# richhiey/YourMT3

Measured on AMD Instinct MI355X. Metric: audio-sec transcribed / wall-sec (RTF), higher is better.
Workload: dtype bf16; 1 GPU; BASELINE configs[1]: MT3 base (T5-small dims, 6+6 layers, d512, 8x64 heads, d_ff 2048, vocab 1536), 2.048 s / 16 kHz / 128-mel segments (256 encoder frames), greedy decode forced to 1024 tokens, seeded random weights; segments_per_gpu=64, global_batch=64, decode_len=1024, frames=256, parallelism=dp1 (segments sharded, token ids all-gathered over RCCL)

## Files before the change

include/ymt3.h:

```cpp
#ifndef YMT3_H
#define YMT3_H

#include <stddef.h>
#include <stdint.h>

#ifdef __cplusplus
extern "C" {
#endif

#define YMT3_ABI_VERSION 3

enum { YMT3_OK = 0, YMT3_ERR_ARG = 1, YMT3_ERR_BLOB = 2, YMT3_ERR_HIP = 3, YMT3_ERR_UNSUPPORTED = 4 };
enum { YMT3_ENC_T5 = 0, YMT3_ENC_PERCEIVER_TF = 1 };
enum { YMT3_FFN_DENSE = 0, YMT3_FFN_MOE = 1 };

typedef struct ymt3_config {
    int32_t sample_rate, segment_samples, n_fft, hop, n_mels;
    float   f_min, f_max, log_floor;
    int32_t d_model, d_ff, n_heads, d_kv, n_enc_layers, n_dec_layers;
    int32_t vocab, rel_buckets, rel_max_distance;
    float   ln_eps;
    int32_t max_decode_len, n_channels, eos_id, pad_id;
    int32_t encoder_type, n_latents;
    int32_t dec_ffn, n_experts, moe_top_k, moe_fp8;
// ... 4 lines not shown
typedef struct ymt3_ctx* ymt3_handle;

int         ymt3_abi_version(void);
const char* ymt3_last_error(void);

int  ymt3_create(const ymt3_config* cfg, const void* blob_host, size_t blob_bytes, int device, ymt3_handle* out);
void ymt3_destroy(ymt3_handle h);

size_t ymt3_device_bytes(ymt3_handle h);

#define YMT3_PCM_S16 0
#define YMT3_PCM_F32 1
int ymt3_ingest_plan(ymt3_handle h, int64_t n_frames, int sample_rate_in, int64_t* n_samples_out, int* n_segments);
int ymt3_ingest(ymt3_handle h, const void* pcm_dev, int pcm_format, int64_t n_frames, int n_channels,
                int sample_rate_in, float* segments_dev, int n_segments, void* stream);

int ymt3_logmel(ymt3_handle h, const float* audio_dev, int B, float* mel_dev, void* stream);

int ymt3_encode(ymt3_handle h, const float* mel_dev, int B, void* enc_dev, void* stream);

int ymt3_decode_greedy(ymt3_handle h, const void* enc_dev, int B, int n_steps, int32_t* tokens_dev,
                       const int32_t* forced_dev, float* logits_dev, void* stream);

int ymt3_decode_prompted(ymt3_handle h, const void* enc_dev, int B, int n_steps, const int32_t* prompt_dev, int n_prompt,
                         int32_t* tokens_dev, const int32_t* forced_dev, float* logits_dev, void* stream);
int ymt3_transcribe_segments_prompted(ymt3_handle h, const float* audio_dev, int B, int n_steps, const int32_t* prompt_dev,
                                      int n_prompt, int32_t* tokens_dev, void* stream);
int ymt3_transcribe_stream_prompted(ymt3_handle h, const float* audio_dev, int n_segments, int n_steps, const int32_t* prompt_dev,
                                    int n_prompt, int32_t* tokens_dev, int slots, int interval, void* stream);

int ymt3_decode_scored(ymt3_handle h, const void* enc_dev, int B, int n_steps, const int32_t* prompt_dev, int n_prompt,
                       int32_t* tokens_dev, float* scores_dev, const int32_t* forced_dev, float* logits_dev, void* stream);
int ymt3_transcribe_segments_scored(ymt3_handle h, const float* audio_dev, int B, int n_steps, const int32_t* prompt_dev,
                                    int n_prompt, int32_t* tokens_dev, float* scores_dev, void* stream);
int ymt3_transcribe_stream_scored(ymt3_handle h, const float* audio_dev, int n_segments, int n_steps, const int32_t* prompt_dev,
                                  int n_prompt, int32_t* tokens_dev, float* scores_dev, int slots, int interval, void* stream);

int ymt3_score_tokens(ymt3_handle h, const void* enc_dev, int B, int n_steps, const int32_t* prompt_dev, int n_prompt,
                      const int32_t* tokens_dev, const int32_t* lengths_dev, float* scores_dev, float* logits_dev, void* stream);
int ymt3_transcribe_segments_score(ymt3_handle h, const float* audio_dev, int B, int n_steps, const int32_t* prompt_dev, int n_prompt,
                                   const int32_t* tokens_dev, const int32_t* lengths_dev, float* scores_dev, void* stream);

typedef struct ymt3_constraint_s* ymt3_constraint;
int  ymt3_constraint_create(ymt3_handle h, int n_states, int vocab, const uint32_t* allowed_bits_host, const int32_t* next_host,
                            ymt3_constraint* out);
void ymt3_constraint_destroy(ymt3_constraint c);
int ymt3_decode_constrained(ymt3_handle h, const void* enc_dev, int B, int n_steps, const int32_t* prompt_dev, int n_prompt,
                            int32_t* tokens_dev, float* scores_dev, const int32_t* forced_dev, float* logits_dev,
                            ymt3_constraint constraint, const int32_t* start_state_dev, void* stream);
int ymt3_transcribe_segments_constrained(ymt3_handle h, const float* audio_dev, int B, int n_steps, const int32_t* prompt_dev,
                                         int n_prompt, int32_t* tokens_dev, float* scores_dev, ymt3_constraint constraint,
                                         const int32_t* start_state_dev, void* stream);
int ymt3_transcribe_stream_constrained(ymt3_handle h, const float* audio_dev, int n_segments, int n_steps, const int32_t* prompt_dev,
                                       int n_prompt, int32_t* tokens_dev, float* scores_dev, int slots, int interval,
                                       ymt3_constraint constraint, const int32_t* start_state_dev, void* stream);

typedef struct ymt3_beam_params { int32_t num_beams, num_return; float length_penalty; } ymt3_beam_params;
int ymt3_decode_beam(ymt3_handle h, const void* enc_dev, int B, int n_steps, const int32_t* prompt_dev, int n_prompt,
                     const ymt3_beam_params* params, int32_t* tokens_dev, float* seq_scores_dev, float* token_scores_dev,
                     ymt3_constraint constraint, const int32_t* start_state_dev, void* stream);
int ymt3_transcribe_segments_beam(ymt3_handle h, const float* audio_dev, int B, int n_steps, const int32_t* prompt_dev, int n_prompt,
                                  const ymt3_beam_params* params, int32_t* tokens_dev, float* seq_scores_dev, float* token_scores_dev,
                                  ymt3_constraint constraint, const int32_t* start_state_dev, void* stream);
int ymt3_transcribe_stream_beam(ymt3_handle h, const float* audio_dev, int n_segments, int n_steps, const int32_t* prompt_dev, int n_prompt,
                                const ymt3_beam_params* params, int32_t* tokens_dev, float* seq_scores_dev, float* token_scores_dev,
                                int slots, int interval, ymt3_constraint constraint, const int32_t* start_state_dev, void* stream);
int ymt3_debug_beam_trace(ymt3_handle h, int32_t* trace_dev, float* run_dev, float* logits_dev, int n_steps, int n_groups);

int ymt3_set_early_stop(ymt3_handle h, int interval);

int ymt3_transcribe_segments(ymt3_handle h, const float* audio_dev, int B, int n_steps,
                             int32_t* tokens_dev, void* stream);

int ymt3_transcribe_stream(ymt3_handle h, const float* audio_dev, int n_segments, int n_steps, int32_t* tokens_dev,
                           int slots, int interval, void* stream);

int ymt3_last_decode_steps(ymt3_handle h);

int ymt3_set_abort_recovery(ymt3_handle h, int mode);
int ymt3_merged_fallbacks(ymt3_handle h);

int ymt3_last_decode_chains(ymt3_handle h);

#define YMT3_PROFILE_CLASSES 16
int ymt3_profile_decode(ymt3_handle h, const void* enc_dev, int B, int n_steps, int stride, int32_t* tokens_dev,
                        float* ms_by_class, int32_t* launches_by_class, void* stream);

int ymt3_debug_step_stamps(ymt3_handle h, int32_t* cls, int32_t* grid, uint64_t* stats, int* n_kernels);
int ymt3_debug_kernel_stamps(ymt3_handle h, int kernel, uint64_t* stamps, int capacity_wgs);

int ymt3_debug_decode_start(ymt3_handle h, int step0);

int ymt3_debug_force_stage_abort(ymt3_handle h);

int ymt3_debug_moe_trace(ymt3_handle h, int32_t* trace_dev, int n_steps, int n_rows);

int ymt3_test_gemm(ymt3_handle h, const void* a_dev, const void* w_dev, float* c_dev, int M, int N, int K, void* stream);

#ifdef __cplusplus
}
#endif
#endif
```

yourmt3_amd/_lib.py:

```python
from __future__ import annotations

import ctypes
import os

from .config import CConfig

_HERE = os.path.dirname(os.path.abspath(__file__))
LIB_PATH = os.environ.get("YMT3_LIB", os.path.join(_HERE, "libymt3_hip.so"))

SYMBOLS = [
    "ymt3_abi_version", "ymt3_last_error", "ymt3_create", "ymt3_destroy", "ymt3_device_bytes",
    "ymt3_logmel", "ymt3_encode", "ymt3_decode_greedy", "ymt3_transcribe_segments", "ymt3_test_gemm", "ymt3_profile_decode", "ymt3_debug_decode_start", "ymt3_debug_force_stage_abort", "ymt3_set_early_stop", "ymt3_last_decode_steps",
    "ymt3_ingest_plan", "ymt3_ingest", "ymt3_transcribe_stream", "ymt3_debug_step_stamps", "ymt3_debug_kernel_stamps",
    "ymt3_set_abort_recovery", "ymt3_merged_fallbacks", "ymt3_debug_moe_trace", "ymt3_last_decode_chains",
    "ymt3_decode_prompted", "ymt3_transcribe_segments_prompted", "ymt3_transcribe_stream_prompted",
    "ymt3_decode_scored", "ymt3_transcribe_segments_scored", "ymt3_transcribe_stream_scored",
    "ymt3_constraint_create", "ymt3_constraint_destroy", "ymt3_decode_constrained", "ymt3_transcribe_segments_constrained",
    "ymt3_transcribe_stream_constrained",
    "ymt3_decode_beam", "ymt3_transcribe_segments_beam", "ymt3_debug_beam_trace", "ymt3_transcribe_stream_beam",
    "ymt3_score_tokens", "ymt3_transcribe_segments_score",
]

_lib = None


class BeamParams(ctypes.Structure):
    _fields_ = [("num_beams", ctypes.c_int32), ("num_return", ctypes.c_int32), ("length_penalty", ctypes.c_float)]


class YMT3Error(RuntimeError):
    pass


def load() -> ctypes.CDLL:
    global _lib
    if _lib is not None:
        return _lib
    if not os.path.exists(LIB_PATH):
        raise YMT3Error(
            f"{LIB_PATH} not found: build it with `python -m yourmt3_amd.build` "
            "(hipcc --offload-arch=gfx950).  There is no CPU fallback for the hot path.")
    import torch
    lib = ctypes.CDLL(LIB_PATH)
    vp, i32, sz = ctypes.c_void_p, ctypes.c_int, ctypes.c_size_t
    lib.ymt3_abi_version.restype = i32
    lib.ymt3_last_error.restype = ctypes.c_char_p
    lib.ymt3_create.argtypes = [ctypes.POINTER(CConfig), vp, sz, i32, ctypes.POINTER(vp)]
    lib.ymt3_create.restype = i32
    lib.ymt3_destroy.argtypes = [vp]
    lib.ymt3_destroy.restype = None
    lib.ymt3_device_bytes.argtypes = [vp]
    lib.ymt3_device_bytes.restype = sz
    lib.ymt3_logmel.argtypes = [vp, vp, i32, vp, vp]
    lib.ymt3_encode.argtypes = [vp, vp, i32, vp, vp]
    lib.ymt3_decode_greedy.argtypes = [vp, vp, i32, i32, vp, vp, vp, vp]
    lib.ymt3_transcribe_segments.argtypes = [vp, vp, i32, i32, vp, vp]
    lib.ymt3_test_gemm.argtypes = [vp, vp, vp, vp, i32, i32, i32, vp]
    lib.ymt3_profile_decode.argtypes = [vp, vp, i32, i32, i32, vp, ctypes.POINTER(ctypes.c_float), ctypes.POINTER(ctypes.c_int32), vp]
    lib.ymt3_profile_decode.restype = i32
    lib.ymt3_debug_decode_start.argtypes = [vp, i32]
    lib.ymt3_debug_decode_start.restype = i32
    lib.ymt3_debug_force_stage_abort.argtypes = [vp]
    lib.ymt3_debug_force_stage_abort.restype = i32
    lib.ymt3_last_decode_steps.argtypes = [vp]
    lib.ymt3_last_decode_steps.restype = i32
    lib.ymt3_set_early_stop.argtypes = [vp, i32]
    lib.ymt3_set_early_stop.restype = i32
    lib.ymt3_ingest_plan.argtypes = [vp, ctypes.c_int64, i32, ctypes.POINTER(ctypes.c_int64), ctypes.POINTER(ctypes.c_int)]
    lib.ymt3_ingest_plan.restype = i32
    lib.ymt3_ingest.argtypes = [vp, vp, i32, ctypes.c_int64, i32, i32, vp, i32, vp]
    lib.ymt3_ingest.restype = i32
    lib.ymt3_transcribe_stream.argtypes = [vp, vp, i32, i32, vp, i32, i32, vp]
    lib.ymt3_transcribe_stream.restype = i32
    lib.ymt3_decode_prompted.argtypes = [vp, vp, i32, i32, vp, i32, vp, vp, vp, vp]
    lib.ymt3_decode_prompted.restype = i32
    lib.ymt3_transcribe_segments_prompted.argtypes = [vp, vp, i32, i32, vp, i32, vp, vp]
    lib.ymt3_transcribe_segments_prompted.restype = i32
    lib.ymt3_transcribe_stream_prompted.argtypes = [vp, vp, i32, i32, vp, i32, vp, i32, i32, vp]
    lib.ymt3_transcribe_stream_prompted.restype = i32
    lib.ymt3_decode_scored.argtypes = [vp, vp, i32, i32, vp, i32, vp, vp, vp, vp, vp]
    lib.ymt3_decode_scored.restype = i32
    lib.ymt3_transcribe_segments_scored.argtypes = [vp, vp, i32, i32, vp, i32, vp, vp, vp]
    lib.ymt3_transcribe_segments_scored.restype = i32
    lib.ymt3_transcribe_stream_scored.argtypes = [vp, vp, i32, i32, vp, i32, vp, vp, i32, i32, vp]
    lib.ymt3_transcribe_stream_scored.restype = i32
    lib.ymt3_constraint_create.argtypes = [vp, i32, i32, vp, vp, ctypes.POINTER(vp)]
    lib.ymt3_constraint_create.restype = i32
    lib.ymt3_constraint_destroy.argtypes = [vp]
    lib.ymt3_constraint_destroy.restype = None
    lib.ymt3_decode_constrained.argtypes = [vp, vp, i32, i32, vp, i32, vp, vp, vp, vp, vp, vp, vp]
    lib.ymt3_decode_constrained.restype = i32
    lib.ymt3_transcribe_segments_constrained.argtypes = [vp, vp, i32, i32, vp, i32, vp, vp, vp, vp, vp]
    lib.ymt3_transcribe_segments_constrained.restype = i32
    lib.ymt3_transcribe_stream_constrained.argtypes = [vp, vp, i32, i32, vp, i32, vp, vp, i32, i32, vp, vp, vp]
    lib.ymt3_transcribe_stream_constrained.restype = i32
    lib.ymt3_debug_step_stamps.argtypes = [vp, vp, vp, vp, ctypes.POINTER(ctypes.c_int)]
    lib.ymt3_debug_step_stamps.restype = i32
    lib.ymt3_debug_kernel_stamps.argtypes = [vp, i32, vp, i32]
    lib.ymt3_debug_kernel_stamps.restype = i32
    lib.ymt3_set_abort_recovery.argtypes = [vp, i32]
    lib.ymt3_set_abort_recovery.restype = i32
    lib.ymt3_merged_fallbacks.argtypes = [vp]
    lib.ymt3_merged_fallbacks.restype = i32
    lib.ymt3_last_decode_chains.argtypes = [vp]
    lib.ymt3_last_decode_chains.restype = i32
    lib.ymt3_debug_moe_trace.argtypes = [vp, vp, i32, i32]
    lib.ymt3_debug_moe_trace.restype = i32
    bp = ctypes.POINTER(BeamParams)
    lib.ymt3_decode_beam.argtypes = [vp, vp, i32, i32, vp, i32, bp, vp, vp, vp, vp, vp, vp]
    lib.ymt3_decode_beam.restype = i32
    lib.ymt3_transcribe_segments_beam.argtypes = [vp, vp, i32, i32, vp, i32, bp, vp, vp, vp, vp, vp, vp]
    lib.ymt3_transcribe_segments_beam.restype = i32
    lib.ymt3_transcribe_stream_beam.argtypes = [vp, vp, i32, i32, vp, i32, bp, vp, vp, vp, i32, i32, vp, vp, vp]
    lib.ymt3_transcribe_stream_beam.restype = i32
    lib.ymt3_debug_beam_trace.argtypes = [vp, vp, vp, vp, i32, i32]
    lib.ymt3_debug_beam_trace.restype = i32
    lib.ymt3_score_tokens.argtypes = [vp, vp, i32, i32, vp, i32, vp, vp, vp, vp, vp]
    lib.ymt3_score_tokens.restype = i32
    lib.ymt3_transcribe_segments_score.argtypes = [vp, vp, i32, i32, vp, i32, vp, vp, vp, vp]
    lib.ymt3_transcribe_segments_score.restype = i32
    for n in ("ymt3_logmel", "ymt3_encode", "ymt3_decode_greedy", "ymt3_transcribe_segments", "ymt3_test_gemm"):
        getattr(lib, n).restype = i32
    if lib.ymt3_abi_version() != 3:
        raise YMT3Error("libymt3_hip.so ABI version mismatch")
    _lib = lib
    return lib


def check(rc: int) -> None:
    if rc != 0:
        raise YMT3Error(f"ymt3 error {rc}: {load().ymt3_last_error().decode(errors='replace')}")
```

yourmt3_amd/csrc/decode.hip:

```cpp
#include <cstdlib>
#include <type_traits>

#include "common.h"
#include "kernels.h"

namespace {

constexpr int DKV = 64;
constexpr int WO_LDS_BYTES = 8 * 64 * 128;
typedef unsigned u32x4 __attribute__((ext_vector_type(4)));

#ifndef YMT3_STAMP_PHASE
#define YMT3_STAMP_PHASE 0
#endif
#define STAMP_IN(a) do { if ((a).stamp && threadIdx.x == 0) (a).stamp[2 * blockIdx.x] = wall_clock64(); } while (0)
#define PAIR_MARK(a, k, v) do { if ((a).stamp && threadIdx.x == 0) (a).stamp[1024 + 8 * blockIdx.x + (k)] = (v); } while (0)
#define STAMP_OUT(a) do { if ((a).stamp && (threadIdx.x & 63) == 0) atomicMax((a).stamp + 2 * blockIdx.x + 1, (unsigned long long)wall_clock64()); } while (0)

template <int MODE, int K, int NT, bool PEND = false>
__global__ __launch_bounds__(512) void dec_gemm_kernel(const bf16_t* __restrict__ pW, const void* __restrict__ pX, const float* __restrict__ pGain,
                                                       float* pSsq, float* pOut, int row0, int R, int N, int ssq_stride, DecGemmArgs a) {
    constexpr bool NORM = (MODE != DG_RESID);
    constexpr int KW = K / 8;
    constexpr int KS = KW / 32;
// ... 111 lines not shown
                }
                __syncthreads();
            }
#pragma unroll
            for (int i = 0; i < NIX; ++i) {
                const int row = i * RPIX + lane / LPRX;
                const float sc = sscale[row];
                *reinterpret_cast<uint2*>(sA + row * PITCH + (lane % LPRX) * 8) =
                    make_uint2(pack_bf16x2(xv[i][0] * sc * gv[0], xv[i][1] * sc * gv[1]),
                               pack_bf16x2(xv[i][2] * sc * gv[2], xv[i][3] * sc * gv[3]));
            }
        } else {
            u32x4 av[NIA];
#pragma unroll
            for (int i = 0; i < NIA; ++i) {
                int mm = m0 + i * RPIW + lane / LPRW;
                mm = mm < m_end ? mm : m_end - 1;
                av[i] = *reinterpret_cast<const u32x4*>(reinterpret_cast<const bf16_t*>(pX) + (size_t)mm * K + wave * KW + (lane % LPRW) * 8);
            }
            __builtin_amdgcn_sched_barrier(0);
            STAMP_IN(a);
#pragma unroll
            for (int i = 0; i < NIW; ++i) {
                const int off = (i * RPIW + lane / LPRW) * PITCH + (lane % LPRW) * 16;
                *reinterpret_cast<u32x4*>(sW + off) = wv[i];
                if (i < NIA) *reinterpret_cast<u32x4*>(sA + off) = av[i];
            }
        }
#pragma unroll
        for (int ks = 0; ks < KS; ++ks) {
            const int off = li * PITCH + (ks * 32 + g * 8) * 2;
            const bf16x8 af = *reinterpret_cast<const bf16x8*>(sA + off);
#pragma unroll
            for (int c = 0; c < NT; ++c) {
                const bf16x8 wf = *reinterpret_cast<const bf16x8*>(sW + c * STRIP + off);
                acc[c] = __builtin_amdgcn_mfma_f32_16x16x32_bf16(wf, af, acc[c], 0, 0, 0);
            }
        }
    }

#if YMT3_STAMP_PHASE == 1
    STAMP_IN(a);
#endif
#pragma unroll
    for (int c = 0; c < NT; ++c)
        *reinterpret_cast<float4*>(red + ((wave * ROWS + li) * COLS + c * 16 + g * 4)) =
            make_float4(acc[c][0], acc[c][1], acc[c][2], acc[c][3]);
    __syncthreads();
#if YMT3_STAMP_PHASE == 2
    STAMP_IN(a);
#endif
    float2 s = make_float2(0.f, 0.f);
    if (epi) {
        s = *reinterpret_cast<const float2*>(red + (mr * COLS + nq));
#pragma unroll
        for (int w = 1; w < 8; ++w) {
            const float2 t = *reinterpret_cast<const float2*>(red + ((w * ROWS + mr) * COLS + nq));
            s.x += t.x; s.y += t.y;
        }
    }

    if constexpr (MODE == DG_RESID) {
        float2 o = make_float2(0.f, 0.f);
        if (live) {
            if (a.part) {
                float2 sp = hp[0];
#pragma unroll
                for (int w = 1; w < 8; ++w) { sp.x += hp[w].x; sp.y += hp[w].y; }
                hold.x += sp.x; hold.y += sp.y;
            }
            o = make_float2(hold.x + s.x, hold.y + s.y);
            *reinterpret_cast<float2*>(pOut + (size_t)m * N + n) = o;
        }
        float q = o.x * o.x + o.y * o.y;
        q = sum8(q);
        if (live && (tid & 7) == 0) pSsq[(size_t)nt_idx * ssq_stride + m] = q;
    } else if constexpr (MODE == DG_NORM_LOGITS) {
        if (live) *reinterpret_cast<float2*>(pOut + (size_t)m * N + n) = s;
    } else if (live) {
        if constexpr (MODE == DG_NORM_BF16_RELU) { s.x = fmaxf(s.x, 0.f); s.y = fmaxf(s.y, 0.f); }
        const uint32_t pk = pack_bf16x2(s.x, s.y);
        if constexpr (MODE == DG_NORM_QKV_CACHE) {
            const int inner = a.H * DKV;
            if (n < inner) {
                *reinterpret_cast<uint32_t*>(a.out_bf16 + (size_t)m * inner + n) = pk;
            } else {
                const int nn = n - inner, kv = nn / inner, hh = (nn % inner) >> 6, dd = nn & 63;
                bf16_t* cache = kv ? a.vcache : a.kcache;
                *reinterpret_cast<uint32_t*>(cache + (((size_t)m * a.H + hh) * a.L + step) * DKV + dd) = pk;
            }
        } else {
            *reinterpret_cast<uint32_t*>(a.out_bf16 + (size_t)m * N + n) = pk;
        }
    }
    STAMP_OUT(a);
}

template <int MODE, int K, int BM, int PF, int NTH>
__global__ __launch_bounds__(NTH) void dec_gemm_mid_kernel(const bf16_t* __restrict__ pW, const void* __restrict__ pX, const float* __restrict__ pGain,
                                                           float* pSsq, float* pOut, int row0, int R, int N, int ssq_stride, DecGemmArgs a) {
    constexpr bool NORM = (MODE != DG_RESID);
    constexpr int BN = 64, BK = 64, MT = BM / 16, PITCH = BK * 2 + 16, NKT = K / BK;
    constexpr int RG = NTH / 256, MTW = MT / RG;
    static_assert(NTH == 256 || NTH == 512, "");
    static_assert(MT % RG == 0, "row tiles split between the two wave groups");
    constexpr int A_STAGE = BM * PITCH, W_STAGE = BN * PITCH;
    __shared__ __attribute__((aligned(16))) char sA[2][A_STAGE];
    __shared__ __attribute__((aligned(16))) char sW[2][W_STAGE];
    __shared__ float sscale[BM];
    __shared__ __attribute__((aligned(16))) float sgain[NORM ? K : 4];
    const int tid = threadIdx.x, lane = tid & 63, wave = tid >> 6, li = lane & 15, g = lane >> 4;
    const int wc = wave & 3, rg = wave >> 2;
    const int n_mt = (R + BM - 1) / BM, n_nt = N / BN;
    int nt_idx, mt_idx;
    if ((n_nt & 7) == 0) {
        const int xcd = blockIdx.x & 7, slot = blockIdx.x >> 3;
        mt_idx = slot % n_mt;
        nt_idx = (slot / n_mt) * 8 + xcd;
    } else {
        mt_idx = blockIdx.x % n_mt;
        nt_idx = blockIdx.x / n_mt;
    }
    const int n0 = nt_idx * BN, m0 = row0 + mt_idx * BM, m_end = row0 + R;

    constexpr int NWV = 512 / NTH, NAB = (BM * 8 + NTH - 1) / NTH, NAF = BM * 16 / NTH;
    static_assert(BM * 16 % NTH == 0, "");
    static_assert(NKT % PF == 0, "the K loop is unrolled by the prefetch depth");
    u32x4 wvr[PF][NWV];
    u32x4 abr[PF][NORM ? 1 : NAB];
    f32x4 afr[PF][NORM ? NAF : 1];
    auto load_regs = [&](int kt, u32x4 (&wv)[NWV], u32x4 (&ab)[NORM ? 1 : NAB], f32x4 (&af)[NORM ? NAF : 1]) {
#pragma unroll
        for (int i = 0; i < NWV; ++i) {
            const int idx = tid + i * NTH, row = idx >> 3, ch = idx & 7;
            wv[i] = *reinterpret_cast<const u32x4*>(pW + (size_t)(n0 + row) * K + kt * BK + ch * 8);
        }
        if constexpr (NORM) {
#pragma unroll
            for (int i = 0; i < NAF; ++i) {
                const int idx = tid + i * NTH, row = idx >> 4, ch = idx & 15;
                int mm = m0 + row;
                mm = mm < m_end ? mm : m_end - 1;
                af[i] = *reinterpret_cast<const f32x4*>(reinterpret_cast<const float*>(pX) + (size_t)mm * K + kt * BK + ch * 4);
            }
        } else {
#pragma unroll
            for (int i = 0; i < NAB; ++i) {
                const int idx = tid + i * NTH, row = idx >> 3, ch = idx & 7;
                int mm = m0 + row;
                mm = mm < m_end ? mm : m_end - 1;
                if (BM * 8 % NTH == 0 || idx < BM * 8)
                    ab[i] = *reinterpret_cast<const u32x4*>(reinterpret_cast<const bf16_t*>(pX) + (size_t)mm * K + kt * BK + ch * 8);
            }
        }
    };
    auto store_lds = [&](int kt, int buf, const u32x4 (&wv)[NWV], const u32x4 (&ab)[NORM ? 1 : NAB], const f32x4 (&af)[NORM ? NAF : 1]) {
#pragma unroll
        for (int i = 0; i < NWV; ++i) {
            const int idx = tid + i * NTH, row = idx >> 3, ch = idx & 7;
            *reinterpret_cast<u32x4*>(sW[buf] + row * PITCH + ch * 16) = wv[i];
        }
        if constexpr (NORM) {
#pragma unroll
            for (int i = 0; i < NAF; ++i) {
                const int idx = tid + i * NTH, row = idx >> 4, ch = idx & 15;
                const float sc = sscale[row];
                const f32x4 gv = *reinterpret_cast<const f32x4*>(sgain + kt * BK + ch * 4);
// ... 454 lines not shown
        }
        if constexpr (OP && SELF) qs[tid] = f2bf(o / L);
        else a.out[((size_t)r * H + h) * DKV + tid] = f2bf(o / L);
    }
    if constexpr (OP && SELF) {
        __syncthreads();
        asm volatile("s_waitcnt vmcnt(0)" ::: "memory");
        const int li = lane & 15, g = lane >> 4;
        const char* strip = wo_lds + wave * 8192;
        f32x4 pa[4];
#pragma unroll
        for (int c = 0; c < 4; ++c) pa[c] = (f32x4){0.f, 0.f, 0.f, 0.f};
#pragma unroll
        for (int ks = 0; ks < 2; ++ks) {
            bf16x8 af = *reinterpret_cast<const bf16x8*>(qs + ks * 32 + g * 8);
            if (li != 0) af = (bf16x8){0, 0, 0, 0, 0, 0, 0, 0};
#pragma unroll
            for (int c = 0; c < 4; ++c) {
                const int row = c * 16 + li;
                const bf16x8 wf = *reinterpret_cast<const bf16x8*>(strip + row * 128 + (((ks * 4 + g) ^ (row & 7)) * 16));
                pa[c] = __builtin_amdgcn_mfma_f32_16x16x32_bf16(wf, af, pa[c], 0, 0, 0);
            }
        }
        if (li == 0) {
            float* dst = a.opart + ((size_t)r * H + h) * 512 + wave * 64 + g * 4;
            if constexpr (PAIR == 1) {
                const __amdgpu_buffer_rsrc_t ro = __builtin_amdgcn_make_buffer_rsrc(a.opart, 0, 0x7fffffff, 0x00020000);
                const int off = (((r * H + h) * 512) + wave * 64 + g * 4) * 4;
#pragma unroll
                for (int c = 0; c < 4; ++c) __builtin_amdgcn_raw_buffer_store_b128(__builtin_bit_cast(u32x4, pa[c]), ro, off + c * 64, 0, 16);
            } else {
#pragma unroll
                for (int c = 0; c < 4; ++c) *reinterpret_cast<float4*>(dst + c * 16) = make_float4(pa[c][0], pa[c][1], pa[c][2], pa[c][3]);
            }
        }
    }
    if constexpr (FUSEQ) {
        if (a.chain_sync && blockIdx.x == 0 && tid < CHAIN_COUNTERS) a.chain_sync[tid * CHAIN_LINE] = 0u;
    }
    if constexpr (PAIR == 1) PAIR_MARK(a, 2, wall_clock64());
    if constexpr (PAIR == 2) pair_leave(ps, r, left_before);
    if constexpr (PAIR != 1) STAMP_OUT(a);
}

template <bool SELF, bool FUSEQ, int NW, bool OP = false>
__global__ __launch_bounds__(64 * NW, 4) void dec_attn_kernel(const bf16_t* __restrict__ pK, const bf16_t* __restrict__ pV, const bf16_t* __restrict__ pQ,
                                                              const float* __restrict__ pF, const void* __restrict__ p4, const void* __restrict__ p5,
                                                              unsigned geom0, unsigned geom1, DecAttnArgs a) {
    attn_body<SELF, FUSEQ, NW, OP, 0>(pK, pV, pQ, pF, p4, p5, geom0, geom1, a, PairSync{});
}

template <int NW>
__global__ __launch_bounds__(64 * NW, 4) void dec_attn_beam_kernel(const bf16_t* __restrict__ pK, const bf16_t* __restrict__ pV, const bf16_t* __restrict__ pQ,
                                                                   const float* __restrict__ pF, const void* __restrict__ p4, const void* __restrict__ p5,
                                                                   unsigned geom0, unsigned geom1, DecAttnArgs a, BeamAttn ba) {
    attn_body<true, false, NW, false, 0, true>(pK, pV, pQ, pF, p4, p5, geom0, geom1, a, PairSync{}, ba);
}

__global__ __launch_bounds__(512, 4) void dec_attn_pair_kernel(const bf16_t* __restrict__ pK, const bf16_t* __restrict__ pV, const bf16_t* __restrict__ pQ,
                                                               const float* __restrict__ pF, const void* __restrict__ p4, const void* __restrict__ p5,
                                                               unsigned geom0, unsigned geom1, DecAttnArgs a, DecAttnArgs b, unsigned gb0, unsigned gb1,
                                                               PairSync ps) {
    attn_body<true, false, 8, true, 1>(pK, pV, pQ, pF, p4, p5, geom0, geom1, a, ps);
    asm volatile("" ::: "memory");
    __builtin_amdgcn_sched_barrier(0);
    attn_body<false, true, 8, true, 2>(b.k, b.v, b.wq, b.x_f32, b.gain, b.ipart, gb0, gb1, b, ps);
}

__device__ __forceinline__ void embed_row(const ArgmaxArgs& a, int r, const bf16_t* e, const bf16_t* c, float* scratch4) {
    const int tid = threadIdx.x;
    float q = 0.f;
    for (int i = tid; i < a.d; i += 256) {
        const float v = bf2f(e[i]) + (c ? bf2f(c[i]) : 0.f);
        a.h[(size_t)r * a.d + i] = v;
        q += v * v;
    }
    q = wave_sum(q);
    __syncthreads();
    if ((tid & 63) == 0) scratch4[tid >> 6] = q;
    __syncthreads();
    if (tid < SSQ_TILES) a.ssq[(size_t)tid * a.ssq_stride + r] = tid == 0 ? (scratch4[0] + scratch4[1]) + (scratch4[2] + scratch4[3]) : 0.f;
}

__global__ __launch_bounds__(256) void argmax_embed_kernel(const float* __restrict__ pLogits, DecodeShared* pShared, int* pFinished, int* pRowPos,
                                                           const long long* __restrict__ pRowOut, const bf16_t* __restrict__ pEmbed, int row0, int V,
                                                           ArgmaxArgs a) {
    __shared__ float sv[4];
    __shared__ int si[4];
    __shared__ int s_feed;
    __shared__ float s_sum[4];
    const int tid = threadIdx.x, lane = tid & 63, wave = tid >> 6;
    const int r = row0 + blockIdx.x;
    DecodeShared* sh = pShared;
    const int t = sh->step, n_steps = sh->n_steps, n_prompt = sh->n_prompt, col = t - sh->step0 - n_prompt;
    const float* row = pLogits + (size_t)r * V;
    int32_t* const tokens_out = sh->tokens_out;
    const int32_t* const forced = sh->forced;
    float* const logits_out = sh->logits_out;
    const int32_t* const prompt = sh->prompt;
    float* const scores_out = sh->scores_out;
    const uint32_t* const c_allowed = sh->c_allowed;
    const int was_finished = pFinished[r];
    const int forced_tok = forced && col >= 0 ? forced[(size_t)r * n_steps + col] : 0;
    const int pos0 = pRowPos ? pRowPos[r] : 0;
    const long long out0 = pRowPos ? pRowOut[r] : 0;

    STAMP_IN(a);
    float bv = -3.4e38f;
    int bi = 0;
    for (int i = tid; i < V; i += 256) {
        const float v = row[i];
        if (v > bv) { bv = v; bi = i; }
    }
    int state = 0;
    const uint32_t* mrow = nullptr;
    if (c_allowed) {
        state = a.row_state[r];
        asm volatile("" : "+v"(state));
        mrow = c_allowed + (size_t)state * sh->c_words;
        bv = -3.4e38f;
        bi = 0x7fffffff;
        for (int i = tid; i < V; i += 256) {
            const float v = row[i];
            if ((mrow[i >> 5] >> (i & 31)) & 1u) {
                if (v > bv) { bv = v; bi = i; }
                else bi = min(bi, i);
            }
        }
    }
#define ARGMAX_TAKE(ctrl, rows, cond)                                                                                      \
    do {                                                                                                                  \
        const float ov = __builtin_bit_cast(float, __builtin_amdgcn_update_dpp(0, __builtin_bit_cast(int, bv), (ctrl), (rows), 0xF, false)); \
        const int oi = __builtin_amdgcn_update_dpp(0, bi, (ctrl), (rows), 0xF, false);                                    \
        if ((cond) && (ov > bv || (ov == bv && oi < bi))) { bv = ov; bi = oi; }                                           \
    } while (0)
    ARGMAX_TAKE(0x128, 0xF, true);
    ARGMAX_TAKE(0x124, 0xF, true);
    ARGMAX_TAKE(0x122, 0xF, true);
    ARGMAX_TAKE(0x121, 0xF, true);
    ARGMAX_TAKE(0x142, 0xA, (lane & 16) != 0);
    ARGMAX_TAKE(0x143, 0xC, lane >= 32);
#undef ARGMAX_TAKE
    if (lane == 63) { sv[wave] = bv; si[wave] = bi; }
    __syncthreads();
    const float row_max = scores_out ? fmaxf(fmaxf(sv[0], sv[1]), fmaxf(sv[2], sv[3])) : 0.f;
    long long score_at = -1;
    int score_id = -1;
    if (tid == 0) { bv = sv[0]; bi = si[0]; }
    if (tid == 0 && pRowPos) {
#pragma unroll
        for (int w = 1; w < 4; ++w)
            if (sv[w] > bv || (sv[w] == bv && si[w] < bi)) { bv = sv[w]; bi = si[w]; }
        bi = min(bi, V - 1);
        int feed = a.pad_id;
        if (!was_finished && pos0 < n_prompt) {
            pRowPos[r] = pos0 + 1;
            feed = prompt[a.row_prompt[r] + pos0];
        } else if (!was_finished) {
            const int p = pos0 - n_prompt;
            tokens_out[out0 + p] = bi;
            if ((a.eos_id >= 0 && bi == a.eos_id) || p + 1 >= n_steps) pFinished[r] = 1;
            else pRowPos[r] = pos0 + 1;
            feed = bi;
            score_at = out0 + p;
            score_id = bi;
            if (mrow) a.row_state[r] = sh->c_next[(size_t)state * V + bi];
        }
        s_feed = feed < 0 ? 0 : (feed >= V ? V - 1 : feed);
    } else if (tid == 0 && col < 0) {
        const int p = prompt[(size_t)r * n_prompt + (t - sh->step0)];
        s_feed = p < 0 ? 0 : (p >= V ? V - 1 : p);
    } else if (tid == 0) {
#pragma unroll
        for (int w = 1; w < 4; ++w)
            if (sv[w] > bv || (sv[w] == bv && si[w] < bi)) { bv = sv[w]; bi = si[w]; }
        int tok = min(bi, V - 1);
        if (a.eos_id >= 0) {
            if (was_finished) tok = a.pad_id;
            else if (tok == a.eos_id) pFinished[r] = 1;
        }
        tokens_out[(size_t)r * n_steps + col] = tok;
        int feed = forced ? forced_tok : tok;
        feed = feed < 0 ? 0 : (feed >= V ? V - 1 : feed);
        s_feed = feed;
        score_at = (long long)r * n_steps + col;
        score_id = !forced && a.eos_id >= 0 && was_finished ? -1 : feed;
        if (mrow && !(a.eos_id >= 0 && was_finished)) a.row_state[r] = sh->c_next[(size_t)state * V + feed];
    }
    __syncthreads();
    const int feed = s_feed;
    const bf16_t* e = pEmbed + (size_t)feed * a.d;
    const bf16_t* c = a.chan_embed ? a.chan_embed + (size_t)(r % a.n_channels) * a.d : nullptr;
    embed_row(a, r, e, c, sv);
    if (logits_out && !pRowPos && col >= 0) {
        float* dst = logits_out + ((size_t)r * n_steps + col) * V;
        for (int i = tid; i < V; i += 256) dst[i] = row[i];
    }
    if (scores_out) {
        float q = 0.f;
        if (mrow) {
            for (int i = tid; i < V; i += 256)
                if ((mrow[i >> 5] >> (i & 31)) & 1u) q += __expf(row[i] - row_max);
        } else {
            for (int i = tid; i < V; i += 256) q += __expf(row[i] - row_max);
        }
        q = wave_sum(q);
        if (lane == 0) s_sum[wave] = q;
    }
    if (a.zero_sync)
        for (int i = blockIdx.x * 256 + tid; i < a.zero_lines; i += gridDim.x * 256) a.zero_sync[(size_t)i * CHAIN_LINE] = 0u;
    __syncthreads();
    if (tid == 0) {
        if (scores_out && score_at >= 0)
            scores_out[score_at] = score_id < 0 ? 0.f
                                 : mrow && !((mrow[score_id >> 5] >> (score_id & 31)) & 1u) ? -__builtin_inff()
                                 : (row[score_id] - row_max) - __logf((s_sum[0] + s_sum[1]) + (s_sum[2] + s_sum[3]));
        if (a.eos_id >= 0) __threadfence();
        bool last;
        if (a.ticket && gridDim.x > 64) {
            const int grp = blockIdx.x >> 5, n_grp = ((int)gridDim.x + 31) >> 5, in_grp = min(32, (int)gridDim.x - 32 * grp);
            last = false;
            if (atomicAdd(a.ticket + (size_t)grp * CHAIN_LINE, 1u) == (unsigned)(in_grp - 1)) {
                a.ticket[(size_t)grp * CHAIN_LINE] = 0u;
                if (a.eos_id >= 0) __threadfence();
                last = atomicAdd(&sh->done_count, 1) == n_grp - 1;
            }
        } else {
            last = atomicAdd(&sh->done_count, 1) == (int)gridDim.x - 1;
        }
        if (last) {
            sh->done_count = 0;
            sh->step = t + 1;
            if (a.eos_id >= 0) {
                int n = 0;
                for (int i = 0; i < (int)gridDim.x; ++i) n += pFinished[row0 + i] ? 0 : 1;
                sh->n_unfinished = n;
            }
        }
    }
    STAMP_OUT(a);
}

__global__ __launch_bounds__(256) void decode_init_kernel(ArgmaxArgs a, int n_chains, int n_steps, int step0, int32_t* tokens_out,
                                                          const int32_t* forced, float* logits_out, const int32_t* prompt, int n_prompt,
                                                          float* scores_out, ConstraintView cv) {
    const int r = blockIdx.x, tid = threadIdx.x;
    const bf16_t* e = a.embed + (size_t)a.pad_id * a.d;
    const bf16_t* c = a.chan_embed ? a.chan_embed + (size_t)(r % a.n_channels) * a.d : nullptr;
    __shared__ float sv[4];
    embed_row(a, r, e, c, sv);
    if (tid == 0) {
        a.finished[r] = 0;
        if (a.row_state) a.row_state[r] = cv.start ? min(max(cv.start[r], 0), cv.n_states - 1) : 0;
    }
    if (r == 0 && tid < n_chains) {
        DecodeShared* sh = a.shared + tid;
        sh->step = step0;
        sh->step0 = step0;
        sh->done_count = 0;
        sh->n_unfinished = a.R;
        sh->n_steps = n_steps;
        sh->tokens_out = tokens_out;
        sh->forced = forced;
        sh->logits_out = logits_out;
        sh->prompt = prompt;
        sh->n_prompt = n_prompt;
        sh->scores_out = scores_out;
        sh->c_allowed = cv.allowed;
        sh->c_next = cv.next;
        sh->c_words = cv.words;
    }
}

__global__ __launch_bounds__(256) void slot_start_kernel(ArgmaxArgs a, int row0, long long first_out, int n_steps, long long* row_out,
                                                         long long first_prompt, int n_prompt, long long* row_prompt, ConstraintView cv) {
    const int r = row0 + blockIdx.x, tid = threadIdx.x;
    const bf16_t* e = a.embed + (size_t)a.pad_id * a.d;
    const bf16_t* c = a.chan_embed ? a.chan_embed + (size_t)(r % a.n_channels) * a.d : nullptr;
    __shared__ float sv[4];
    embed_row(a, r, e, c, sv);
    if (tid == 0) {
        a.finished[r] = 0;
        a.row_pos[r] = 0;
        row_out[r] = first_out + (long long)blockIdx.x * n_steps;
        row_prompt[r] = first_prompt + (long long)blockIdx.x * n_prompt;
        if (a.row_state) a.row_state[r] = cv.start ? min(max(cv.start[blockIdx.x], 0), cv.n_states - 1) : 0;
    }
}

__global__ void slot_retire_kernel(ArgmaxArgs a, int row0, int n_steps, int n_prompt, int32_t* tokens_out, float* scores_out) {
    const int r = row0 + blockIdx.x;
    const long long o = a.row_out[r];
    for (int i = max(a.row_pos[r] + 1 - n_prompt, 0) + threadIdx.x; i < n_steps; i += blockDim.x) {
        tokens_out[o + i] = a.pad_id;
        if (scores_out) scores_out[o + i] = 0.f;
    }
}

__global__ void pad_tail_kernel(int32_t* tokens_out, float* scores_out, int row0, int n_steps, int from, int pad_id) {
    const size_t o = (size_t)(row0 + blockIdx.x) * n_steps;
    for (int i = from + threadIdx.x; i < n_steps; i += blockDim.x) {
        tokens_out[o + i] = pad_id;
        if (scores_out) scores_out[o + i] = 0.f;
    }
}

template <int MODE, int K, int NT, bool PEND = false>
constexpr size_t dg_lds_bytes() {
    return (size_t)(8 * 16 * 16 * NT + 16 + (PEND ? 8 * 16 : 0)) * 4 + (size_t)8 * (1 + NT) * 16 * (K / 8 * 2 + 16);
}

template <int MODE, int K, int NT = 1, bool PEND = false>
int launch_dg(const DecGemmArgs& a, hipStream_t stream) {
    if (a.W == nullptr)
        return hipFuncSetAttribute(reinterpret_cast<const void*>(dec_gemm_kernel<MODE, K, NT, PEND>),
                                   hipFuncAttributeMaxDynamicSharedMemorySize, (int)dg_lds_bytes<MODE, K, NT, PEND>()) == hipSuccess ? 0 : -2;
    if (MODE == DG_RESID && a.N != 16 * SSQ_TILES) return -3;
    if (PEND && (!a.pend_y || (MODE == DG_NORM_QKV_CACHE && !a.h_out))) return -4;
    dec_gemm_kernel<MODE, K, NT, PEND><<<(a.N / (16 * NT)) * ((a.R + 15) / 16), 512, dg_lds_bytes<MODE, K, NT, PEND>(), stream>>>(
        a.W, MODE == DG_RESID ? static_cast<const void*>(a.a_bf16) : static_cast<const void*>(a.x_f32), a.gain, a.ssq, a.out_f32, a.row0, a.R, a.N,
        a.ssq_stride, a);
    return 0;
}

template <int MODE, bool PEND = false>
int launch_dg_wide(const DecGemmArgs& a, hipStream_t stream) {
    static const bool narrow = getenv("YMT3_DEC_GEMM_NARROW") != nullptr;
    const int wgs16 = (a.N / 16) * ((a.R + 15) / 16);
    if (!narrow && a.N % 32 == 0 && wgs16 > 320) return launch_dg<MODE, 512, 2, PEND>(a, stream);
    return launch_dg<MODE, 512, 1, PEND>(a, stream);
}

}

int init_decode_kernels() {
    DecGemmArgs z{};
    int rc = 0;
    rc |= launch_dg<DG_RESID, 512>(z, nullptr);
    rc |= launch_dg<DG_RESID, 1024>(z, nullptr);
    rc |= launch_dg<DG_RESID, 2048>(z, nullptr);
    rc |= launch_dg<DG_NORM_QKV_CACHE, 512>(z, nullptr);
    rc |= launch_dg<DG_NORM_BF16, 512>(z, nullptr);
    rc |= launch_dg<DG_NORM_BF16_RELU, 512>(z, nullptr);
    rc |= launch_dg<DG_NORM_LOGITS, 512>(z, nullptr);
    rc |= launch_dg<DG_NORM_QKV_CACHE, 512, 2>(z, nullptr);
    rc |= launch_dg<DG_NORM_BF16, 512, 2>(z, nullptr);
    rc |= launch_dg<DG_NORM_BF16_RELU, 512, 2>(z, nullptr);
    rc |= launch_dg<DG_NORM_LOGITS, 512, 2>(z, nullptr);
    rc |= launch_dg<DG_NORM_QKV_CACHE, 512, 1, true>(z, nullptr);
    rc |= launch_dg<DG_NORM_QKV_CACHE, 512, 2, true>(z, nullptr);
    rc |= launch_dg<DG_NORM_LOGITS, 512, 1, true>(z, nullptr);
    rc |= launch_dg<DG_NORM_LOGITS, 512, 2, true>(z, nullptr);
    if (hipFuncSetAttribute(reinterpret_cast<const void*>(dec_attn_pair_kernel), hipFuncAttributeMaxDynamicSharedMemorySize, WO_LDS_BYTES) != hipSuccess) rc |= -2;
    if (hipFuncSetAttribute(reinterpret_cast<const void*>(dec_attn_kernel<true, false, 8, true>), hipFuncAttributeMaxDynamicSharedMemorySize,
                            WO_LDS_BYTES) != hipSuccess) rc |= -2;
    return rc;
}

template <int MODE, int K, int BM>
int launch_dg_mid(const DecGemmArgs& a, hipStream_t stream) {
    if (MODE == DG_RESID && a.N != 16 * SSQ_TILES) return -3;
    constexpr int PF = 4;
    constexpr int NTH = 256;
    dec_gemm_mid_kernel<MODE, K, BM, PF, NTH><<<(a.N / 64) * ((a.R + BM - 1) / BM), NTH, 0, stream>>>(
        a.W, MODE == DG_RESID ? static_cast<const void*>(a.a_bf16) : static_cast<const void*>(a.x_f32), a.gain, a.ssq, a.out_f32, a.row0, a.R, a.N,
        a.ssq_stride, a);
    return 0;
}

static int launch_dec_gemm_mid(int mode, const DecGemmArgs& a, hipStream_t stream) {
    if (a.N % 64 || a.part) return -1;
    switch (mode) {
        case DG_RESID:
            if (a.K == 512) return launch_dg_mid<DG_RESID, 512, 32>(a, stream);
            if (a.K == 2048) return launch_dg_mid<DG_RESID, 2048, 32>(a, stream);
            return -1;
        case DG_NORM_QKV_CACHE: return a.K == 512 ? launch_dg_mid<DG_NORM_QKV_CACHE, 512, 64>(a, stream) : -1;
        case DG_NORM_BF16: return a.K == 512 ? launch_dg_mid<DG_NORM_BF16, 512, 32>(a, stream) : -1;
        case DG_NORM_BF16_RELU: return a.K == 512 ? launch_dg_mid<DG_NORM_BF16_RELU, 512, 64>(a, stream) : -1;
        case DG_NORM_LOGITS: return a.K == 512 ? launch_dg_mid<DG_NORM_LOGITS, 512, 64>(a, stream) : -1;
        default: return -1;
    }
}

int launch_dec_gemm(int mode, const DecGemmArgs& a, hipStream_t stream) {
    if (a.R <= 0) return 0;
    if (a.N % 16) return -1;
    const int mid_rows = a.mid_rows >= 0 ? a.mid_rows : DEC_GEMM_MID_ROWS;
    if (mid_rows > 0 && a.R >= mid_rows && a.N % 64 == 0 && !a.part && !a.pend_y && (a.K == 512 || (a.K == 2048 && mode == DG_RESID)))
        return launch_dec_gemm_mid(mode, a, stream);
    if (mode == DG_RESID) {
        if (a.K == 512) return launch_dg<DG_RESID, 512>(a, stream);
        if (a.K == 2048) return launch_dg<DG_RESID, 2048>(a, stream);
        if (a.K == 1024) return launch_dg<DG_RESID, 1024>(a, stream);
        return -1;
    }
    if (a.K != 512) return -1;
    if (a.pend_y) {
        if (mode == DG_NORM_QKV_CACHE) return launch_dg_wide<DG_NORM_QKV_CACHE, true>(a, stream);
        if (mode == DG_NORM_LOGITS) return launch_dg_wide<DG_NORM_LOGITS, true>(a, stream);
        return -1;
    }
    switch (mode) {
        case DG_NORM_QKV_CACHE: return launch_dg_wide<DG_NORM_QKV_CACHE>(a, stream);
        case DG_NORM_BF16: return launch_dg_wide<DG_NORM_BF16>(a, stream);
        case DG_NORM_BF16_RELU: return launch_dg_wide<DG_NORM_BF16_RELU>(a, stream);
        case DG_NORM_LOGITS: return launch_dg_wide<DG_NORM_LOGITS>(a, stream);
        default: return -1;
    }
}

int launch_dec_attention(bool self_attn, const DecAttnArgs& a, hipStream_t stream) {
    if (a.R <= 0) return 0;
    const bool many = a.force_many || a.R * a.H > 2048;
    if (a.chain_sync && (self_attn || !a.wq)) return -1;
    if ((a.wo || a.ipart) && (many || a.H != 8 || (a.wo && !a.opart) || (a.ipart && !a.wq))) return -1;
    if (a.row0 < 0 || a.row0 > 0xffff || a.rows_per_kv < 1 || a.rows_per_kv > 0xff || a.H < 1 || a.H > 0xff || a.slab_keys < 1 || a.slab_keys > 0xfffff ||
        a.n_keys_const < 0 || a.n_keys_const > 0xfff || (self_attn && a.bias_stride != a.slab_keys))
        return -1;
    const unsigned g0 = (unsigned)a.row0 | (unsigned)a.rows_per_kv << 16 | (unsigned)a.H << 24, g1 = (unsigned)a.slab_keys | (unsigned)a.n_keys_const << 20;
    const int grid = a.R * a.H;
#define ATTN(S, F, W, O, THREADS, LDS, PQ, PF, P4, P5) dec_attn_kernel<S, F, W, O><<<grid, THREADS, LDS, stream>>>(a.k, a.v, PQ, PF, P4, P5, g0, g1, a)
    if (self_attn) {
        if (a.wo) ATTN(true, false, 8, true, 512, WO_LDS_BYTES, a.q, a.bias, a.shared, a.row_pos);
        else if (many) ATTN(true, false, 2, false, 128, 0, a.q, a.bias, a.shared, a.row_pos);
        else ATTN(true, false, 8, false, 512, 0, a.q, a.bias, a.shared, a.row_pos);
    } else if (a.wq) {
        if (a.ipart) ATTN(false, true, 8, true, 512, 0, a.wq, a.x_f32, a.gain, a.ipart);
        else ATTN(false, true, 8, false, 512, 0, a.wq, a.x_f32, a.gain, a.ssq);
    } else {
        if (many) ATTN(false, false, 2, false, 128, 0, a.q, nullptr, nullptr, nullptr);
        else ATTN(false, false, 8, false, 512, 0, a.q, nullptr, nullptr, nullptr);
    }
#undef ATTN
    return 0;
}

int launch_dec_attention_beam(const DecAttnArgs& a, const BeamAttn& ba, hipStream_t stream) {
    if (a.R <= 0) return 0;
    if (!ba.anc || ba.W < 1 || ba.W > BEAM_MAX || a.R % ba.W || a.row0 % ba.W || ba.anc_pitch % 16 || ba.anc_pitch <= a.slab_keys || ba.anc_pitch > 48 * 1024 ||
        a.row0 + a.R > ba.anc_rows || a.wo || a.ipart || a.wq || a.chain_sync || a.rows_per_kv != 1)
        return -1;
    if (a.row0 < 0 || a.row0 > 0xffff || a.H < 1 || a.H > 0xff || a.slab_keys < 1 || a.slab_keys > 0xfffff || a.bias_stride != a.slab_keys) return -1;
    const bool many = a.force_many || a.R * a.H > 2048;
    const unsigned g0 = (unsigned)a.row0 | 1u << 16 | (unsigned)a.H << 24, g1 = (unsigned)a.slab_keys;
    const int grid = a.R * a.H;
    if (many) dec_attn_beam_kernel<2><<<grid, 128, ba.anc_pitch, stream>>>(a.k, a.v, a.q, a.bias, a.shared, a.row_pos, g0, g1, a, ba);
    else dec_attn_beam_kernel<8><<<grid, 512, ba.anc_pitch, stream>>>(a.k, a.v, a.q, a.bias, a.shared, a.row_pos, g0, g1, a, ba);
    return 0;
}

bool dec_attention_pair_fits(int n_cus) {
    int n = 0;
    if (hipOccupancyMaxActiveBlocksPerMultiprocessor(&n, dec_attn_pair_kernel, 512, WO_LDS_BYTES) != hipSuccess) return false;
    return (long long)n * n_cus >= 512;
}

int launch_dec_attention_pair(const DecAttnArgs& a, const DecAttnArgs& b, unsigned* pair_rows, unsigned* abort_word, unsigned* host_abort,
                              hipStream_t stream) {
    if (a.R <= 0) return 0;
    if (a.R > 16 * CHAIN_TILES_MAX || a.R != b.R || a.row0 != b.row0 || a.H != 8 || b.H != 8 || !a.wo || !a.opart || !b.wq || b.ipart != a.opart || !pair_rows || !abort_word ||
        a.rows_per_kv != 1 || b.rows_per_kv < 1 || b.rows_per_kv > 0xff || a.row0 < 0 || a.row0 > 0xffff || a.slab_keys < 1 || a.slab_keys > 0xfffff ||
        b.slab_keys < 1 || b.slab_keys > 0xfffff || b.n_keys_const < 1 || b.n_keys_const > 0xfff || a.bias_stride != a.slab_keys)
        return -1;
    const unsigned g0 = (unsigned)a.row0 | 1u << 16 | 8u << 24, g1 = (unsigned)a.slab_keys;
    const unsigned h0 = (unsigned)b.row0 | (unsigned)b.rows_per_kv << 16 | 8u << 24, h1 = (unsigned)b.slab_keys | (unsigned)b.n_keys_const << 20;
    dec_attn_pair_kernel<<<a.R * 8, 512, WO_LDS_BYTES, stream>>>(a.k, a.v, a.q, a.bias, a.shared, a.row_pos, g0, g1, a, b, h0, h1,
                                                                 PairSync{pair_rows, abort_word, host_abort});
    return 0;
}

int launch_argmax_embed(const ArgmaxArgs& a, hipStream_t stream) {
    if (a.R <= 0) return 0;
    argmax_embed_kernel<<<a.R, 256, 0, stream>>>(a.logits, a.shared, a.finished, a.row_pos, a.row_out, a.embed, a.row0, a.V, a);
    return 0;
}

int launch_decode_init(const ArgmaxArgs& a, int n_chains, int n_steps, int step0, int32_t* tokens_out, const int32_t* forced,
                       float* logits_out, const int32_t* prompt, int n_prompt, float* scores_out, const ConstraintView& cv,
                       hipStream_t stream) {
    if (a.R <= 0) return 0;
    if (n_prompt < 0 || (n_prompt > 0 && !prompt)) return -1;
    if (cv.allowed && (!cv.next || !a.row_state || cv.n_states < 1 || cv.words * 32 < a.V)) return -1;
    decode_init_kernel<<<a.R, 256, 0, stream>>>(a, n_chains, n_steps, step0, tokens_out, forced, logits_out, prompt, n_prompt, scores_out, cv);
    return 0;
}

int launch_slot_start(const ArgmaxArgs& a, int row0, long long first_out, int n_steps, long long* row_out, long long first_prompt,
                      int n_prompt, long long* row_prompt, const ConstraintView& cv, hipStream_t stream) {
    if (!a.row_pos || !row_out || !row_prompt || a.n_channels <= 0) return -1;
    if (cv.start && cv.n_states < 1) return -1;
    slot_start_kernel<<<a.n_channels, 256, 0, stream>>>(a, row0, first_out, n_steps, row_out, first_prompt, n_prompt, row_prompt, cv);
    return 0;
}

int launch_slot_retire(const ArgmaxArgs& a, int row0, int n_rows, int n_steps, int n_prompt, int32_t* tokens_out, float* scores_out,
                       hipStream_t stream) {
    if (!a.row_pos || !a.row_out || n_rows <= 0) return -1;
    slot_retire_kernel<<<n_rows, 256, 0, stream>>>(a, row0, n_steps, n_prompt, tokens_out, scores_out);
    return 0;
}

int launch_pad_tail(int32_t* tokens_out, float* scores_out, int row0, int R, int n_steps, int from, int pad_id, hipStream_t stream) {
    if (R <= 0 || from >= n_steps) return 0;
    pad_tail_kernel<<<R, 256, 0, stream>>>(tokens_out, scores_out, row0, n_steps, from, pad_id);
    return 0;
}
```

yourmt3_amd/csrc/kernels.h:

```cpp
#pragma once
#include <hip/hip_runtime.h>
#include <stdint.h>
#include "common.h"

struct FrontendTables {
    const float* window;
    const float2* tw;
    const float2* untw;
    const int* mel_start;
    const int* mel_len;
    const int* mel_off;
    const float* mel_w;
    int n_fft, hop, n_mels, n_samples, n_frames, n_mel_w;
    float log_floor;
};
int launch_logmel(const FrontendTables& t, const float* audio, float* mel, int B, hipStream_t stream);

struct IngestArgs {
    const void* pcm;
    const float* taps;
    float* out;
    long long n_in, n_out, n_total, r;
    int up, down, J, Jp, n_channels, s16, window;
};
int launch_ingest(const IngestArgs& a, hipStream_t stream);

enum GemmEpilogue {
    EPI_F32 = 0,
    EPI_BF16 = 1,
    EPI_BF16_RELU = 2,
    EPI_RESID = 3,
    EPI_KV_HEADMAJOR = 4,
};
struct GemmArgs {
    const bf16_t* A; const bf16_t* W; void* out; const float* bias;
    int M, N, K, lda, ldw, ldc;
    int T, H, n_seg;
};
int launch_gemm(int epilogue, const GemmArgs& a, hipStream_t stream);
int init_gemm_kernels();

int launch_rmsnorm(const float* x, const float* gain, bf16_t* out, int M, int d, float eps, hipStream_t stream);
int launch_f32_to_bf16(const float* x, bf16_t* out, size_t n, hipStream_t stream);
int launch_broadcast_bf16(const bf16_t* src, float* out, int B, size_t n, hipStream_t stream);

int init_enc_attn_kernels();
int launch_enc_attention_qkv(const bf16_t* q, int ldq, const bf16_t* k, const bf16_t* v, int ldkv, const float* bias_off,
                             bf16_t* out, int B, int T, int H, hipStream_t stream);
int launch_enc_attention(const bf16_t* qkv, const float* bias_off, bf16_t* out, int B, int T, int H, hipStream_t stream);

struct SeqAttnArgs {
    const bf16_t* q; const bf16_t* k; const bf16_t* v; bf16_t* out;
    const float* bias_off;
    int n_seq, H, Tq, Tk, inner_n;
    long long q_outer, q_inner, q_step, kv_outer, kv_inner, kv_step, o_outer, o_inner, o_step;
};
int launch_seq_attention(const SeqAttnArgs& a, hipStream_t stream);
int launch_spec_embed(const float* mel, const float* w, const bf16_t* pos, const float* gain, bf16_t* out, long long n_rows, int F, int d,
                      float eps, hipStream_t stream);

struct DecodeShared {
    int step;
    int done_count;
    int n_steps;
    int step0;
    int n_unfinished;
    int n_prompt;
    int32_t* tokens_out;
    const int32_t* forced;
    float* logits_out;
    const int32_t* prompt;
    float* scores_out;
    const uint32_t* c_allowed;
    const int32_t* c_next;
    int c_words;
};

struct ConstraintView {
    const uint32_t* allowed;
    const int32_t* next;
    int words, n_states;
    const int32_t* start;
};

constexpr int SSQ_TILES = 32;

struct DecGemmArgs {
    const float* x_f32;
    const float* gain;
    const bf16_t* a_bf16;
    const bf16_t* W;
    int row0, R, N, K;
    float eps;
    bf16_t* out_bf16;
    float* out_f32;
    bf16_t* kcache;
    bf16_t* vcache;
    int H, L;
    const DecodeShared* shared;
    const int* row_pos;
    unsigned long long* stamp;
    float* ssq;
    int ssq_stride;
    const float* part;
    const float* pend_y;
    float* h_out;
    int mid_rows;
};
constexpr int DEC_GEMM_MID_ROWS = 512;
struct ChainArgs {
    const bf16_t *w0, *w1, *w2, *w3;
    const bf16_t* attn;
    const float* part;
    float* h;
    float* ssq; int ssq_stride;
    const float *gain1, *gain3;
    bf16_t* dff;
    int d_ff;
    int mode3, N3;
    bf16_t* out_q; bf16_t* kcache; bf16_t* vcache;
    float* logits;
    int H, L;
    const DecodeShared* shared; const int* row_pos;
    int row0, R;
    float eps;
    unsigned* sync;
    unsigned* host_abort;
    unsigned long long* stamp;
    unsigned* sync_abort;
    int nsub;
};
constexpr int CHAIN_LINE = 32;
constexpr int CHAIN_TILES_MAX = 16;
constexpr int CHAIN_COUNTERS = 3 * CHAIN_TILES_MAX * 8;
constexpr int CHAIN_ABORT_WORD = CHAIN_COUNTERS * CHAIN_LINE;
constexpr int CHAIN_SYNC_WORDS = (CHAIN_COUNTERS + 1) * CHAIN_LINE;
int init_chain_kernels();
bool dec_chain_fits(int n_cus);
bool dec_attention_pair_fits(int n_cus);
int launch_dec_chain(const ChainArgs& c, hipStream_t stream);
int launch_chain_poison(const unsigned* sync, int32_t* tokens, float* scores, long long n, hipStream_t stream);

struct StepLayer {
    const bf16_t *wo, *wq_c, *wo_c, *wi, *wo2, *w3;
    const float *ln2, *ln3, *gain3;
    const bf16_t *kself, *vself;
    const bf16_t *kcross, *vcross;
    bf16_t *knext, *vnext;
    int N3, last;
};
struct StepArgs {
    int n_layers, R, T, L, ssq_stride;
    float eps;
    int tiles_free, pad_;
    bf16_t* q; bf16_t* attn; float* opart; float* h; float* ssq; bf16_t* dff; float* logits;
    const float* bias;
    const DecodeShared* shared; const int* row_pos;
    unsigned* sync;
    unsigned* pair_rows;
    unsigned* abort_word; unsigned* host_abort;
    unsigned long long* stamp;
    StepLayer layer[8];
};
constexpr int STEP_SYNC_LINES_PER_LAYER = CHAIN_COUNTERS + 32 + 32;
constexpr int STEP_SYNC_LINES = 9 * STEP_SYNC_LINES_PER_LAYER;
int init_step_kernel();
bool dec_step_fits(int n_cus);
int launch_dec_step(const StepArgs& s, hipStream_t stream);

enum DecGemmMode { DG_NORM_QKV_CACHE = 0, DG_NORM_BF16 = 1, DG_NORM_BF16_RELU = 2, DG_NORM_LOGITS = 3, DG_RESID = 4 };
int init_decode_kernels();
int launch_dec_gemm(int mode, const DecGemmArgs& a, hipStream_t stream);

struct DecAttnArgs {
    const bf16_t* q;
    const bf16_t* k;
    const bf16_t* v;
    bf16_t* out;
    const float* bias;
    const DecodeShared* shared;
    const int* row_pos;
    unsigned long long* stamp;
    int n_keys_const;
    int slab_keys;
    int rows_per_kv;
    int row0, R, H, bias_stride;
    const bf16_t* wq;
    const float* x_f32;
    const float* gain;
    const float* ssq; int ssq_stride;
    float eps;
    const bf16_t* wo;
    float* opart;
    const float* ipart;
    unsigned* chain_sync;
    int force_many;
};
int launch_dec_attention(bool self_attn, const DecAttnArgs& a, hipStream_t stream);
int launch_dec_attention_pair(const DecAttnArgs& self_args, const DecAttnArgs& cross_args, unsigned* pair_rows, unsigned* abort_word,
                              unsigned* host_abort, hipStream_t stream);

struct McCrossArgs {
    const float* x_f32;
    const float* gain;
    const float* ssq; int ssq_stride;
    const bf16_t* wq;
    const bf16_t* k;
    const bf16_t* v;
    bf16_t* out;
    int row0, n_seg, n_channels, H, T;
    float eps;
};
int init_mc_cross_kernels();
int launch_mc_cross_attention(const McCrossArgs& a, hipStream_t stream);

struct ArgmaxArgs {
    const float* logits;
    float* h;
    const bf16_t* embed;
    const bf16_t* chan_embed;
    DecodeShared* shared;
    int* finished;
    float* ssq;
    int ssq_stride;
    int row0, R, V, d, n_channels, eos_id, pad_id;
    int* row_pos;
    const long long* row_out;
    unsigned long long* stamp;
    unsigned* ticket;
    unsigned* zero_sync;
    int zero_lines;
    const long long* row_prompt;
    int* row_state;
};
int launch_argmax_embed(const ArgmaxArgs& a, hipStream_t stream);
int launch_pad_tail(int32_t* tokens_out, float* scores_out, int row0, int R, int n_steps, int from, int pad_id, hipStream_t stream);
int launch_slot_start(const ArgmaxArgs& a, int row0, long long first_out, int n_steps, long long* row_out, long long first_prompt,
                      int n_prompt, long long* row_prompt, const ConstraintView& cv, hipStream_t stream);
int launch_slot_retire(const ArgmaxArgs& a, int row0, int n_rows, int n_steps, int n_prompt, int32_t* tokens_out, float* scores_out,
                       hipStream_t stream);
int launch_decode_init(const ArgmaxArgs& a, int n_chains, int n_steps, int step0, int32_t* tokens_out, const int32_t* forced,
                       float* logits_out, const int32_t* prompt, int n_prompt, float* scores_out, const ConstraintView& cv,
                       hipStream_t stream);

constexpr int BEAM_MAX = 8;
struct BeamAttn {
    const uint8_t* anc;
    int anc_rows, anc_pitch, W;
};
int launch_dec_attention_beam(const DecAttnArgs& a, const BeamAttn& ba, hipStream_t stream);

struct BeamShared {
    float alpha;
    int32_t* tokens_out;
    float* seq_out;
    float* tok_out;
    int32_t* trace;
    float* trace_run;
    float* trace_logits;
    int trace_steps, trace_groups;
};
struct BeamArgs {
    const float* logits;
    float* h;
    const bf16_t* embed; const bf16_t* chan_embed;
    DecodeShared* shared; BeamShared* beam;
    int* finished;
    float* ssq; int ssq_stride;
    int R, V, d, n_channels, eos_id, pad_id, W;
    int* row_state;
    uint8_t* anc; int anc_rows, anc_pitch;
    int32_t* fed_tok; float* fed_lp; int fed_pitch;
    float* run;
    float* fin_score; int* fin_len; int* fin_store; int32_t* fin_tok; float* fin_lp;
    int* n_fin;
    uint8_t* slot_anc;
    unsigned long long* stamp;
    int* row_pos;
    long long* row_out;
    long long* row_prompt;
};
int launch_beam_select(const BeamArgs& a, hipStream_t stream);
int launch_beam_init(const BeamArgs& a, int n_steps, const int32_t* prompt, int n_prompt, const ConstraintView& cv, const BeamShared& params,
                     hipStream_t stream);
int launch_beam_finalize(const BeamArgs& a, int N, hipStream_t stream);
int launch_beam_slot_start(const BeamArgs& a, int row0, long long first_group, int n_prompt, const ConstraintView& cv, hipStream_t stream);
int launch_beam_slot_finalize(const BeamArgs& a, int row0, int N, hipStream_t stream);

struct SeqEmbedArgs {
    float* h;
    const bf16_t* embed;
    const bf16_t* chan_embed;
    const int32_t* prompt;
    const int32_t* tokens;
    int row0, n_rows, L, n_prompt, n_steps, V, d, n_channels, pad_id;
};
int launch_seq_embed(const SeqEmbedArgs& a, hipStream_t stream);
struct SeqAttnDecArgs {
    const bf16_t* q; const bf16_t* k; const bf16_t* v; bf16_t* out;
    const float* bias;
    long long q_seq, kv_seq, o_seq;
    int ldq, ldkv, ldo, kv_head;
    int row0, n_rows, L, n_keys, rows_per_kv, H, bias_stride;
};
int launch_dec_seq_attention(bool causal, const SeqAttnDecArgs& a, hipStream_t stream);
struct SeqLmHeadArgs {
    const bf16_t* xn;
    const bf16_t* W;
    const int32_t* tokens;
    const int32_t* lengths;
    float* scores;
    float* logits;
    int M, L, n_prompt, n_steps, V, d, row0;
};
int launch_seq_lm_head_score(const SeqLmHeadArgs& a, hipStream_t stream);

struct MoeArgs {
    float* h;
// ... 39 lines not shown
```

yourmt3_amd/csrc/runtime.hip:

```cpp
#include <hip/hip_runtime.h>

#include <cmath>
#include <cstdarg>
#include <cstdio>
#include <cstdlib>
#include <algorithm>
#include <cstring>
#include <map>
#include <atomic>
#include <string>
#include <thread>
#include <vector>

#include "../../include/ymt3.h"
#include "common.h"
#include "kernels.h"

static thread_local char g_err[512] = "";
void ymt3_set_error(const char* fmt, ...) {
    va_list ap;
    va_start(ap, fmt);
    vsnprintf(g_err, sizeof(g_err), fmt, ap);
    va_end(ap);
}
// ... 4 lines not shown
    } while (0)
#define LAUNCH(expr)                                                             \
    do {                                                                         \
        int _rc = (expr);                                                        \
        if (_rc != 0) FAIL(YMT3_ERR_UNSUPPORTED, "%s rejected its shape (rc=%d)", #expr, _rc); \
    } while (0)

struct Tensor {
    void* dev = nullptr;
    uint32_t dtype = 0, ndim = 0, shape[4] = {1, 1, 1, 1};
    size_t nbytes = 0;
};

struct StepGraph {
    hipGraph_t graph = nullptr;
    hipGraphExec_t exec = nullptr;
    bool merged = false;
};

struct ymt3_ctx {
    ymt3_config cfg{};
    int device = 0;
    int T = 0, inner = 0, maxB = 0, maxR = 0;
    char* blob_dev = nullptr;
    size_t blob_bytes = 0;
    std::map<std::string, Tensor> tensors;
    std::vector<void*> allocs;
    size_t dev_bytes = 0;
    FrontendTables fe{};
    float* mel = nullptr;
    bf16_t* mel_bf = nullptr;
    float* h_enc = nullptr;
    bf16_t *xn = nullptr, *qkv = nullptr, *attn = nullptr, *ff = nullptr, *enc_out = nullptr;
    size_t act_rows = 0;
    bf16_t *p_xs = nullptr, *p_kvs = nullptr;
    float* p_z = nullptr;
    bf16_t *p_zn = nullptr, *p_qkv = nullptr, *p_att = nullptr, *p_ff = nullptr;
    bf16_t* wkv_all = nullptr;
    bf16_t* ckv = nullptr;
    bf16_t *kcache = nullptr, *vcache = nullptr;
    float* h_dec = nullptr;
    float* h_dec2 = nullptr;
    bf16_t *dq = nullptr, *dattn = nullptr, *dff = nullptr;
    float* logits = nullptr;
    float* ssq = nullptr;
    float* opart = nullptr;
    MoeArgs moe{};
    int* finished = nullptr;
    int* row_pos = nullptr;
    long long* row_out = nullptr;
    long long* row_prompt = nullptr;
    int* row_state = nullptr;
    int* host_rows = nullptr;
    bool slot_mode = false;
    DecodeShared* shared = nullptr;
    hipStream_t cap_stream = nullptr;
    int n_chains = 1;
    bool auto_chains = true;
    int last_chains = 1;
    bool chain_threads = true;
    hipStream_t chain_stream[8] = {};
    hipEvent_t fork_ev = nullptr, join_ev[8] = {};
    std::map<long, StepGraph> step_graphs;
    bool use_graph = true;
    int graph_steps = 16;
    bool fuse_q = true;
    bool moe_fold_combine = true;
    bool fold_o = true;
    bool gemm_chain = true;
    unsigned* chain_sync = nullptr;
    unsigned* chain_host_abort = nullptr;
    bool step_merged = false;
    bool forced_abort = false;
    int abort_recovery = 1;
    int fallback_count = 0;
    int mid_rows = -1;
    bool force_2wave = false;
    bool attn_pair = true;
    unsigned* pair_rows = nullptr;
    bool step_kernel = false;
    bool moe_chain = false;
    int merged_max_rows = 64;
    bool step_tiles_free = false;
    unsigned* ticket = nullptr;
    unsigned* step_sync = nullptr;
    bool prof_on = false;
    size_t prof_span_idx = 0;
    bool prof_span_open = false;
    int last_steps = 0;
    int early_stop_interval = 0;
    int* host_flag = nullptr;
    bool debug_hooks = false;
    int prof_step0 = 0;
    int32_t* moe_trace = nullptr;
    int moe_trace_steps = 0, moe_trace_rows = 0;
    int beam_W = 0;
    BeamArgs beam{};
    BeamShared* beam_shared = nullptr;
    BeamShared beam_trace{};
    std::vector<hipEvent_t> prof_ev;
    std::vector<int> prof_cls;
    unsigned long long* stamp_buf = nullptr;
    int stamp_n = 0, stamp_cls[64] = {}, stamp_grid[64] = {};
    struct Resampler { float* taps = nullptr; int up = 1, down = 1, J = 1, Jp = 4, window = 0; long long r = 0; };
    std::map<std::pair<int, int>, Resampler> resamplers;
};

constexpr int STAMP_NODES = 64, STAMP_WGS = 8192;
static unsigned long long* next_stamp(ymt3_ctx* c, int cls, int grid) {
    if (!c->stamp_buf || c->stamp_n >= STAMP_NODES || grid > STAMP_WGS) return nullptr;
    const int i = c->stamp_n++;
    c->stamp_cls[i] = cls;
    c->stamp_grid[i] = grid;
    return c->stamp_buf + (size_t)i * STAMP_WGS * 2;
}

enum { PC_QKV = 0, PC_SELF_ATTN, PC_SELF_O, PC_CROSS_Q, PC_CROSS_ATTN, PC_CROSS_O, PC_FFN_WI, PC_FFN_WO, PC_LM_HEAD, PC_ARGMAX, PC_SPAN, PC_CHAIN, PC_ATTN_PAIR, PC_STEP, PC_COUNT };

struct ProfScope {
    ymt3_ctx* c; hipStream_t s; bool on;
    ProfScope(ymt3_ctx* c_, int cls, hipStream_t s_) : c(c_), s(s_), on(c_->prof_on) {
        if (!on) return;
        hipEvent_t a, b;
        if (hipEventCreate(&a) != hipSuccess || hipEventCreate(&b) != hipSuccess) { on = false; return; }
        c->prof_ev.push_back(a); c->prof_ev.push_back(b); c->prof_cls.push_back(cls);
        (void)hipEventRecord(a, s);
    }
    ~ProfScope() { if (on) (void)hipEventRecord(c->prof_ev.back(), s); }
};
#define PLAUNCH(cls, expr) do { ProfScope _ps(h, cls, s); LAUNCH(expr); } while (0)

static int dev_alloc(ymt3_ctx* c, void** p, size_t bytes) {
    HIP_TRY(hipMalloc(p, bytes ? bytes : 16));
    c->allocs.push_back(*p);
    c->dev_bytes += bytes;
    return 0;
}

template <typename T>
static int get(ymt3_ctx* c, const std::string& name, uint32_t dtype, T** out, size_t min_elems = 0) {
    auto it = c->tensors.find(name);
    if (it == c->tensors.end()) FAIL(YMT3_ERR_BLOB, "weight blob has no tensor '%s'", name.c_str());
    if (it->second.dtype != dtype) FAIL(YMT3_ERR_BLOB, "tensor '%s' has dtype %u, expected %u", name.c_str(), it->second.dtype, dtype);
    const size_t esz = dtype == 1 ? 2 : (dtype == 3 ? 1 : 4);
    if (it->second.nbytes < min_elems * esz)
        FAIL(YMT3_ERR_BLOB, "tensor '%s' holds %zu bytes, expected at least %zu", name.c_str(), it->second.nbytes, min_elems * esz);
    *out = reinterpret_cast<T*>(it->second.dev);
    return 0;
}
#define GET(...)                     \
    do {                             \
        int _rc = get(__VA_ARGS__);  \
        if (_rc) return _rc;         \
    } while (0)

#pragma pack(push, 1)
struct BlobEntry {
    char name[48];
    uint32_t dtype, ndim, shape[4];
    uint64_t offset, nbytes;
};
#pragma pack(pop)
static_assert(sizeof(BlobEntry) == 88, "blob entry layout");

static int parse_blob(ymt3_ctx* c, const void* blob, size_t nbytes) {
    const char* b = static_cast<const char*>(blob);
    if (nbytes < 16 || memcmp(b, "YMT3BLOB", 8) != 0) FAIL(YMT3_ERR_BLOB, "bad weight blob magic");
    uint32_t ver, n;
    memcpy(&ver, b + 8, 4);
    memcpy(&n, b + 12, 4);
    if (ver != 1) FAIL(YMT3_ERR_BLOB, "unsupported blob version %u", ver);
    if (16 + (size_t)n * sizeof(BlobEntry) > nbytes) FAIL(YMT3_ERR_BLOB, "truncated blob header");
    HIP_TRY(hipMalloc(reinterpret_cast<void**>(&c->blob_dev), nbytes));
    c->allocs.push_back(c->blob_dev);
    c->dev_bytes += nbytes;
    c->blob_bytes = nbytes;
    HIP_TRY(hipMemcpy(c->blob_dev, blob, nbytes, hipMemcpyHostToDevice));
    for (uint32_t i = 0; i < n; ++i) {
        BlobEntry e;
        memcpy(&e, b + 16 + (size_t)i * sizeof(BlobEntry), sizeof(e));
        const size_t header_end = 16 + (size_t)n * sizeof(BlobEntry);
        if (e.offset % 16 || e.offset < header_end || e.offset > nbytes || e.nbytes > nbytes - e.offset)
            FAIL(YMT3_ERR_BLOB, "tensor %u out of bounds / misaligned", i);
        e.name[47] = 0;
        Tensor t;
        t.dev = c->blob_dev + e.offset;
        t.dtype = e.dtype;
        t.ndim = e.ndim;
        memcpy(t.shape, e.shape, sizeof(t.shape));
        t.nbytes = e.nbytes;
        c->tensors[e.name] = t;
    }
    return 0;
}

extern "C" int ymt3_abi_version(void) { return YMT3_ABI_VERSION; }
extern "C" const char* ymt3_last_error(void) { return g_err; }

extern "C" void ymt3_destroy(ymt3_handle h) {
    if (!h) return;
    (void)hipSetDevice(h->device);
    for (auto& kv : h->step_graphs) {
        if (kv.second.exec) (void)hipGraphExecDestroy(kv.second.exec);
        if (kv.second.graph) (void)hipGraphDestroy(kv.second.graph);
    }
    if (h->cap_stream) (void)hipStreamDestroy(h->cap_stream);
    if (h->host_flag) (void)hipHostFree(h->host_flag);
    if (h->chain_host_abort) (void)hipHostFree(h->chain_host_abort);
    if (h->host_rows) (void)hipHostFree(h->host_rows);
    for (int i = 0; i < 8; ++i) {
        if (h->chain_stream[i]) (void)hipStreamDestroy(h->chain_stream[i]);
        if (h->join_ev[i]) (void)hipEventDestroy(h->join_ev[i]);
    }
    if (h->fork_ev) (void)hipEventDestroy(h->fork_ev);
    for (void* p : h->allocs) (void)hipFree(p);
    delete h;
}

extern "C" size_t ymt3_device_bytes(ymt3_handle h) { return h ? h->dev_bytes : 0; }

static int create_impl(ymt3_ctx* c, const ymt3_config* cfg, const void* blob, size_t nbytes) {
    const ymt3_config& k = c->cfg;
    if (k.d_kv != 64) FAIL(YMT3_ERR_UNSUPPORTED, "d_kv must be 64 (got %d)", k.d_kv);
    if (k.d_model != 16 * SSQ_TILES) FAIL(YMT3_ERR_UNSUPPORTED, "d_model must be 512 (got %d)", k.d_model);
    if (k.n_heads * k.d_kv != 512) FAIL(YMT3_ERR_UNSUPPORTED, "n_heads*d_kv must be 512");
    if (k.encoder_type != YMT3_ENC_T5 && k.encoder_type != YMT3_ENC_PERCEIVER_TF) FAIL(YMT3_ERR_UNSUPPORTED, "unknown encoder_type %d", k.encoder_type);
    if (k.dec_ffn == YMT3_FFN_MOE && (k.moe_top_k != 2 || k.n_experts < 2 || k.n_experts > 16 || k.d_ff != 2048))
        FAIL(YMT3_ERR_UNSUPPORTED, "MoE FFN needs top_k = 2, 2..16 experts, d_ff = 2048");
    if (k.max_batch <= 0 || k.n_channels <= 0 || k.max_decode_len <= 0) FAIL(YMT3_ERR_ARG, "bad max_batch / n_channels / max_decode_len");
    if (k.hop <= 0 || k.sample_rate <= 0 || k.segment_samples <= 0 || k.n_fft <= 0 || k.n_mels <= 0 || k.vocab <= 0 || k.d_ff <= 0 ||
        k.n_enc_layers < 0 || k.n_dec_layers <= 0 || k.n_enc_layers > 64 || k.n_dec_layers > 64 || k.n_channels > 64 ||
        k.max_decode_len > 65536 || (long long)k.max_batch * k.n_channels > 65536)
        FAIL(YMT3_ERR_ARG, "a size field of the config is zero, negative or absurd");
    c->T = 1 + k.segment_samples / k.hop;
    c->inner = k.n_heads * k.d_kv;
    c->maxB = k.max_batch;
    c->maxR = k.max_batch * k.n_channels;
    if (c->T % 64) FAIL(YMT3_ERR_UNSUPPORTED, "n_frames must be a multiple of 64 (got %d)", c->T);
    if (k.segment_samples <= k.n_fft / 2) FAIL(YMT3_ERR_UNSUPPORTED, "segment_samples must exceed n_fft/2 (reflect padding)");
    if (k.pad_id < 0 || k.pad_id >= k.vocab || k.eos_id >= k.vocab) FAIL(YMT3_ERR_ARG, "pad_id / eos_id outside the vocabulary");
    if (k.vocab % 16 || k.d_ff % 128) FAIL(YMT3_ERR_UNSUPPORTED, "vocab %% 16 and d_ff %% 128 must be 0");
    if (k.n_fft != 2048 && k.n_fft != 512) FAIL(YMT3_ERR_UNSUPPORTED, "n_fft must be 2048 or 512 (got %d)", k.n_fft);
    if (k.n_mels % 64) FAIL(YMT3_ERR_UNSUPPORTED, "n_mels must be a multiple of 64 (got %d)", k.n_mels);
    if (k.hop > 256 || k.hop % 2)
        FAIL(YMT3_ERR_UNSUPPORTED, "hop must be even and at most 256 (got %d): the log-mel kernel stages 8 frames in LDS and reads sample pairs", k.hop);
    if (k.encoder_type == YMT3_ENC_T5 && c->T != 64 && c->T != 128 && c->T != 256 && c->T != 512)
        FAIL(YMT3_ERR_UNSUPPORTED, "n_frames must be 64, 128, 256 or 512 for the T5 encoder's self-attention (got %d)", c->T);
    if (k.encoder_type == YMT3_ENC_PERCEIVER_TF && c->T != 64 && c->T != 128 && c->T != 256)
        FAIL(YMT3_ERR_UNSUPPORTED, "n_frames must be 64, 128 or 256 for the Perceiver-TF temporal attention (got %d)", c->T);
    if (k.dec_ffn == YMT3_FFN_DENSE && k.d_ff != 512 && k.d_ff != 1024 && k.d_ff != 2048)
        FAIL(YMT3_ERR_UNSUPPORTED, "a dense d_ff must be 512, 1024 or 2048 (got %d): the decoder's FFN-out kernel is instantiated at those K", k.d_ff);
    if (k.dec_ffn != YMT3_FFN_DENSE && k.dec_ffn != YMT3_FFN_MOE) FAIL(YMT3_ERR_UNSUPPORTED, "unknown dec_ffn %d", k.dec_ffn);

    HIP_TRY(hipSetDevice(c->device));
    int rc = parse_blob(c, blob, nbytes);
    if (rc) return rc;
    if (init_gemm_kernels() || init_enc_attn_kernels() || init_decode_kernels() || init_moe_kernels() || init_mc_cross_kernels()) FAIL(YMT3_ERR_HIP, "hipFuncSetAttribute(max dynamic LDS) failed");

    const int nfft = k.n_fft;
    FrontendTables& fe = c->fe;
    GET(c, "fe.window", 0u, const_cast<float**>(&fe.window), (size_t)nfft);
    GET(c, "fe.tw", 0u, reinterpret_cast<float**>(const_cast<float2**>(&fe.tw)), (size_t)nfft);
    GET(c, "fe.untw", 0u, reinterpret_cast<float**>(const_cast<float2**>(&fe.untw)), (size_t)nfft + 2);
    GET(c, "fe.mel_start", 2u, const_cast<int**>(&fe.mel_start), (size_t)k.n_mels);
    GET(c, "fe.mel_len", 2u, const_cast<int**>(&fe.mel_len), (size_t)k.n_mels);
    GET(c, "fe.mel_off", 2u, const_cast<int**>(&fe.mel_off), (size_t)k.n_mels);
    GET(c, "fe.mel_w", 0u, const_cast<float**>(&fe.mel_w), 1);
    fe.n_mel_w = (int)(c->tensors["fe.mel_w"].nbytes / 4);
    fe.n_fft = nfft; fe.hop = k.hop; fe.n_mels = k.n_mels; fe.n_samples = k.segment_samples;
    fe.n_frames = c->T; fe.log_floor = k.log_floor;
    if (fe.n_mel_w > 2304) FAIL(YMT3_ERR_UNSUPPORTED, "fe.mel_w holds %d filterbank weights; the log-mel kernel stages at most 2304", fe.n_mel_w);

    const size_t BT = (size_t)c->maxB * c->T, d = k.d_model, R = c->maxR;
    if (dev_alloc(c, (void**)&c->mel, BT * k.n_mels * 4)) return YMT3_ERR_HIP;
    if (dev_alloc(c, (void**)&c->mel_bf, BT * k.n_mels * 2)) return YMT3_ERR_HIP;
    const size_t AR = c->act_rows = std::max(BT, (size_t)k.max_decode_len);
    if (dev_alloc(c, (void**)&c->h_enc, AR * d * 4)) return YMT3_ERR_HIP;
    if (dev_alloc(c, (void**)&c->xn, AR * d * 2)) return YMT3_ERR_HIP;
    if (dev_alloc(c, (void**)&c->qkv, AR * 3 * c->inner * 2)) return YMT3_ERR_HIP;
    if (dev_alloc(c, (void**)&c->attn, AR * c->inner * 2)) return YMT3_ERR_HIP;
    if (dev_alloc(c, (void**)&c->ff, AR * k.d_ff * 2)) return YMT3_ERR_HIP;
    if (dev_alloc(c, (void**)&c->enc_out, BT * d * 2)) return YMT3_ERR_HIP;
    if (k.encoder_type == YMT3_ENC_PERCEIVER_TF) {
        const int D = k.ptf_d, K = k.n_latents;
        if (D <= 0 || D % 64 || D > 256) FAIL(YMT3_ERR_UNSUPPORTED, "ptf_d must be 64, 128, 192 or 256 (got %d)", D);
        if (K < 16 || K > 64 || K % 16) FAIL(YMT3_ERR_UNSUPPORTED, "n_latents must be 16, 32, 48 or 64 latents per frame (got %d)", K);
        if (k.ptf_blocks < 1 || k.ptf_blocks > 16 || k.ptf_dff <= 0 || k.ptf_dff % 128) FAIL(YMT3_ERR_UNSUPPORTED, "ptf_blocks must be 1..16 and ptf_dff a multiple of 128");
        if (D % 128 || (3 * D) % 128) FAIL(YMT3_ERR_UNSUPPORTED, "ptf_d must be a multiple of 128 (GEMM column tiles)");
        if (c->T > 256 || (k.n_mels != 64 && k.n_mels != 128 && k.n_mels != 256)) FAIL(YMT3_ERR_UNSUPPORTED, "the Perceiver-TF encoder needs n_frames <= 256 and n_mels in {64, 128, 256}");
        if (K != 32 && K != 64) FAIL(YMT3_ERR_UNSUPPORTED, "n_latents must be 32 or 64 (latent self-attention key tiles)");
        const size_t N1 = (size_t)c->maxB * c->T * k.n_mels, N2 = (size_t)c->maxB * c->T * K;
        if (N1 > 0x7fffffffULL / 2) FAIL(YMT3_ERR_UNSUPPORTED, "max_batch too large for the Perceiver-TF encoder workspace");
        if (dev_alloc(c, (void**)&c->p_xs, N1 * D * 2) || dev_alloc(c, (void**)&c->p_kvs, N1 * 2 * D * 2) || dev_alloc(c, (void**)&c->p_z, N2 * D * 4) ||
            dev_alloc(c, (void**)&c->p_zn, N2 * D * 2) || dev_alloc(c, (void**)&c->p_qkv, N2 * 3 * D * 2) || dev_alloc(c, (void**)&c->p_att, N2 * D * 2) ||
            dev_alloc(c, (void**)&c->p_ff, N2 * k.ptf_dff * 2))
            return YMT3_ERR_HIP;
        std::vector<std::string> names = {"spec_w", "spec_pos", "ln_x", "latents", "bias_off", "ln_out", "out_w"};
        for (int b = 0; b < k.ptf_blocks; ++b) {
            const std::string p = std::to_string(b) + ".";
            for (const char* n : {"s.ln_q", "s.wq", "s.wkv", "s.wo", "l.ln1", "l.wqkv", "l.wo", "t.ln1", "t.wqkv", "t.wo"}) names.push_back(p + n);
            for (const char* sub : {"s.", "l.", "t."})
                for (const char* n : {"ln_ff", "wi", "wo2"}) names.push_back(p + sub + n);
// ... 45 lines not shown
            HIP_TRY(hipMemset(c->step_sync, 0, (size_t)STEP_SYNC_LINES * CHAIN_LINE * sizeof(unsigned)));
        }
        if (c->gemm_chain || c->attn_pair || c->moe_chain) {
            if (dev_alloc(c, (void**)&c->chain_sync, CHAIN_SYNC_WORDS * sizeof(unsigned))) return YMT3_ERR_HIP;
            HIP_TRY(hipMemset(c->chain_sync, 0, CHAIN_SYNC_WORDS * sizeof(unsigned)));
            HIP_TRY(hipHostMalloc(reinterpret_cast<void**>(&c->chain_host_abort), sizeof(unsigned), hipHostMallocDefault));
            *c->chain_host_abort = 0u;
            if (dev_alloc(c, (void**)&c->pair_rows, (size_t)16 * CHAIN_TILES_MAX * 2 * CHAIN_LINE * sizeof(unsigned))) return YMT3_ERR_HIP;
            HIP_TRY(hipMemset(c->pair_rows, 0, (size_t)16 * CHAIN_TILES_MAX * 2 * CHAIN_LINE * sizeof(unsigned)));
        }
    }
    if (k.dec_ffn == YMT3_FFN_MOE) {
        MoeArgs& m = c->moe;
        const size_t P = 2 * R;
        if (R > 1536) FAIL(YMT3_ERR_UNSUPPORTED, "the MoE FFN holds its pair list in LDS: at most 1536 decoder rows (got %zu)", R);
        if (dev_alloc(c, (void**)&m.xn, R * d * 2) || dev_alloc(c, (void**)&m.sel, P * 4) || dev_alloc(c, (void**)&m.gate, P * 4) ||
            dev_alloc(c, (void**)&m.hidden, P * k.d_ff * 2) || dev_alloc(c, (void**)&m.y, P * d * 4))
            return YMT3_ERR_HIP;
        m.E = k.n_experts; m.top_k = k.moe_top_k; m.d_model = d; m.d_ff = k.d_ff; m.eps = k.ln_eps;
    }
    {
        BeamArgs& b = c->beam;
        b.anc_rows = (int)R;
        b.anc_pitch = (k.max_decode_len + 1 + 15) / 16 * 16;
        b.fed_pitch = k.max_decode_len + 1;
        if (dev_alloc(c, (void**)&b.anc, (size_t)2 * R * b.anc_pitch) || dev_alloc(c, (void**)&b.slot_anc, R * b.anc_pitch) ||
            dev_alloc(c, (void**)&b.fed_tok, R * b.fed_pitch * 4) || dev_alloc(c, (void**)&b.fed_lp, R * b.fed_pitch * 4) ||
            dev_alloc(c, (void**)&b.run, R * 4) || dev_alloc(c, (void**)&b.fin_score, R * 4) || dev_alloc(c, (void**)&b.fin_len, R * 4) ||
            dev_alloc(c, (void**)&b.fin_store, R * 4) || dev_alloc(c, (void**)&b.fin_tok, R * 4) || dev_alloc(c, (void**)&b.fin_lp, R * 4) ||
            dev_alloc(c, (void**)&b.n_fin, R * 4) || dev_alloc(c, (void**)&c->beam_shared, sizeof(BeamShared)))
            return YMT3_ERR_HIP;
        HIP_TRY(hipMemset(b.anc, 0, (size_t)2 * R * b.anc_pitch));
        HIP_TRY(hipMemset(b.slot_anc, 0, R * b.anc_pitch));
        HIP_TRY(hipMemset(b.fed_tok, 0, R * b.fed_pitch * 4));
        HIP_TRY(hipMemset(b.fed_lp, 0, R * b.fed_pitch * 4));
        HIP_TRY(hipMemset(c->beam_shared, 0, sizeof(BeamShared)));
    }
    if (dev_alloc(c, (void**)&c->shared, 8 * sizeof(DecodeShared))) return YMT3_ERR_HIP;
    HIP_TRY(hipMemset(c->shared, 0, 8 * sizeof(DecodeShared)));
    if (getenv("YMT3_STAMP")) {
        if (dev_alloc(c, (void**)&c->stamp_buf, (size_t)STAMP_NODES * STAMP_WGS * 2 * sizeof(unsigned long long))) return YMT3_ERR_HIP;
        HIP_TRY(hipMemset(c->stamp_buf, 0, (size_t)STAMP_NODES * STAMP_WGS * 2 * sizeof(unsigned long long)));
    }
    HIP_TRY(hipStreamCreateWithFlags(&c->cap_stream, hipStreamNonBlocking));
    const char* dh = getenv("YMT3_DEBUG_HOOKS");
    c->debug_hooks = dh && dh[0] == '1';
    const char* ng = getenv("YMT3_NO_GRAPH");
    c->use_graph = !(ng && ng[0] == '1');
    if (const char* gs = getenv("YMT3_GRAPH_STEPS")) { const int v = atoi(gs); if (v >= 1 && v <= 64) c->graph_steps = v; }
    const char* nf = getenv("YMT3_NO_FUSEQ");
    c->fuse_q = !(nf && nf[0] == '1');
    const char* mcl = getenv("YMT3_MOE_COMBINE_LAUNCH");
    c->moe_fold_combine = !(mcl && mcl[0] == '1');
    const char* nfo = getenv("YMT3_NO_FOLD_O");
    c->fold_o = !(nfo && nfo[0] == '1');
    if (const char* mr = getenv("YMT3_DEC_GEMM_MID_ROWS")) c->mid_rows = atoi(mr) < 0 ? -1 : atoi(mr);
    const char* f2 = getenv("YMT3_SELF_ATTN_2WAVE");
    c->force_2wave = f2 && f2[0] == '1';
    if (const char* mm = getenv("YMT3_MERGED_MAX_ROWS")) { const int v = atoi(mm); if (v >= 16 && v <= 16 * CHAIN_TILES_MAX) c->merged_max_rows = v; }
    { const char* tf = getenv("YMT3_STEP_TILES_FREE"); c->step_tiles_free = tf && tf[0] == '1'; }
    if (const char* ar = getenv("YMT3_ABORT_RECOVERY")) c->abort_recovery = ar[0] == '0' ? 0 : 1;
    const char* nc = getenv("YMT3_CHAINS");
    if (nc && atoi(nc) >= 1) { c->n_chains = atoi(nc) > 8 ? 8 : atoi(nc); c->auto_chains = false; }
    const char* ct = getenv("YMT3_CHAIN_THREADS");
    c->chain_threads = !(ct && ct[0] == '0');
    for (int i = 0; i < std::max(c->n_chains, 2); ++i) {
        HIP_TRY(hipStreamCreateWithFlags(&c->chain_stream[i], hipStreamNonBlocking));
        HIP_TRY(hipEventCreateWithFlags(&c->join_ev[i], hipEventDisableTiming));
    }
    HIP_TRY(hipEventCreateWithFlags(&c->fork_ev, hipEventDisableTiming));

    const char* enc_names[] = {"ln1", "wqkv", "wo", "ln2", "wi", "wo2"};
    for (int l = 0; l < k.n_enc_layers; ++l)
        for (const char* n : enc_names)
            if (!c->tensors.count("enc." + std::to_string(l) + "." + n)) FAIL(YMT3_ERR_BLOB, "missing enc.%d.%s", l, n);
    const bool fp8_experts = k.dec_ffn == YMT3_FFN_MOE && k.moe_fp8;
    std::vector<const char*> dec_names = {"ln1", "wqkv", "wo", "ln2", "wq_c", "wo_c", "ln3"};
    if (fp8_experts) { dec_names.push_back("wi_q8"); dec_names.push_back("wo2_q8"); dec_names.push_back("wi_s"); dec_names.push_back("wo2_s"); }
    else { dec_names.push_back("wi"); dec_names.push_back("wo2"); }
    if (k.dec_ffn == YMT3_FFN_MOE) dec_names.push_back("router");
    for (int l = 0; l < nd; ++l)
        for (const char* n : dec_names)
            if (!c->tensors.count("dec." + std::to_string(l) + "." + n)) FAIL(YMT3_ERR_BLOB, "missing dec.%d.%s", l, n);
    HIP_TRY(hipDeviceSynchronize());
    return YMT3_OK;
}

extern "C" int ymt3_create(const ymt3_config* cfg, const void* blob, size_t nbytes, int device, ymt3_handle* out) {
    if (!cfg || !blob || !out) FAIL(YMT3_ERR_ARG, "null argument to ymt3_create");
    int ndev = 0;
    if (hipGetDeviceCount(&ndev) != hipSuccess || ndev <= 0) FAIL(YMT3_ERR_HIP, "no HIP device visible: the HIP path cannot run (there is no CPU fallback)");
    if (device < 0 || device >= ndev) FAIL(YMT3_ERR_ARG, "device %d out of range (%d visible)", device, ndev);
    ymt3_ctx* c = new ymt3_ctx();
    c->cfg = *cfg;
    c->device = device;
    int rc = create_impl(c, cfg, blob, nbytes);
    if (rc != YMT3_OK) {
        ymt3_destroy(c);
        return rc;
    }
    *out = c;
    return YMT3_OK;
}

static int merged_fallback(ymt3_ctx* h) {
    h->gemm_chain = h->attn_pair = h->step_kernel = h->moe_chain = false;
    ++h->fallback_count;
    h->forced_abort = false;
    for (auto& kv : h->step_graphs) {
        if (kv.second.exec) (void)hipGraphExecDestroy(kv.second.exec);
        if (kv.second.graph) (void)hipGraphDestroy(kv.second.graph);
    }
    h->step_graphs.clear();
    if (h->chain_sync) HIP_TRY(hipMemset(h->chain_sync, 0, CHAIN_SYNC_WORDS * sizeof(unsigned)));
    if (h->pair_rows) HIP_TRY(hipMemset(h->pair_rows, 0, (size_t)16 * CHAIN_TILES_MAX * 2 * CHAIN_LINE * sizeof(unsigned)));
    if (h->step_sync) HIP_TRY(hipMemset(h->step_sync, 0, (size_t)STEP_SYNC_LINES * CHAIN_LINE * sizeof(unsigned)));
    HIP_TRY(hipDeviceSynchronize());
    if (h->chain_host_abort) *h->chain_host_abort = 0u;
    return YMT3_OK;
}

static int check_call(ymt3_handle h, int B) {
    if (!h) FAIL(YMT3_ERR_ARG, "null handle");
    if (B < 0 || B > h->maxB) FAIL(YMT3_ERR_ARG, "B=%d outside [0, max_batch=%d]", B, h->maxB);
    HIP_TRY(hipSetDevice(h->device));
    if (h->chain_host_abort && *static_cast<volatile unsigned*>(h->chain_host_abort)) {
        HIP_TRY(hipDeviceSynchronize());
        int rc = merged_fallback(h);
        if (rc) return rc;
    }
    return 0;
}

struct ymt3_constraint_s {
    ymt3_ctx* owner;
    int device, n_states, vocab, words;
    uint32_t* allowed = nullptr;
    int32_t* next = nullptr;
};

extern "C" void ymt3_constraint_destroy(ymt3_constraint c) {
    if (!c) return;
    (void)hipSetDevice(c->device);
    if (c->allowed) (void)hipFree(c->allowed);
    if (c->next) (void)hipFree(c->next);
    delete c;
}

extern "C" int ymt3_constraint_create(ymt3_handle h, int n_states, int vocab, const uint32_t* allowed_bits_host, const int32_t* next_host,
                                      ymt3_constraint* out) {
    if (!out) FAIL(YMT3_ERR_ARG, "null output pointer");
    *out = nullptr;
    if (!h) FAIL(YMT3_ERR_ARG, "null handle");
    if (!allowed_bits_host || !next_host) FAIL(YMT3_ERR_ARG, "null automaton table");
    if (vocab != h->cfg.vocab) FAIL(YMT3_ERR_ARG, "constraint vocab=%d != the model's vocab=%d", vocab, h->cfg.vocab);
    if (n_states < 1 || n_states > 1024) FAIL(YMT3_ERR_ARG, "n_states=%d outside [1, 1024]", n_states);
    const int words = (vocab + 31) / 32;
    for (int st = 0; st < n_states; ++st) {
        bool any = false;
        for (int i = 0; i < vocab && !any; ++i) any = (allowed_bits_host[(size_t)st * words + i / 32] >> (i % 32)) & 1u;
        if (!any) FAIL(YMT3_ERR_ARG, "state %d allows no token", st);
        for (int i = 0; i < vocab; ++i) {
            const int32_t nx = next_host[(size_t)st * vocab + i];
            if (nx < 0 || nx >= n_states) FAIL(YMT3_ERR_ARG, "next[%d][%d]=%d outside [0, %d)", st, i, nx, n_states);
        }
    }
// ... 103 lines not shown
        if ((rc = gemm(EPI_BF16, h->p_zn, w, h->p_qkv, N2, 3 * D, D))) return rc;
        {
            SeqAttnArgs a{};
            a.q = h->p_qkv; a.k = h->p_qkv + D; a.v = h->p_qkv + 2 * D; a.out = h->p_att; a.bias_off = tbias;
            a.n_seq = B * K; a.H = Hs; a.Tq = T; a.Tk = T; a.inner_n = K;
            a.q_outer = a.kv_outer = (long long)T * K * 3 * D; a.q_inner = a.kv_inner = 3 * D; a.q_step = a.kv_step = (long long)K * 3 * D;
            a.o_outer = (long long)T * K * D; a.o_inner = D; a.o_step = (long long)K * D;
            LAUNCH(launch_seq_attention(a, s));
        }
        GET(h, p + "t.wo", 1u, &w, (size_t)D * D);
        if ((rc = gemm(EPI_RESID, h->p_att, w, h->p_z, N2, D, D))) return rc;
        if ((rc = ffn(p + "t."))) return rc;
    }
    GET(h, "ptf.ln_out", 0u, &f, (size_t)D);
    LAUNCH(launch_rmsnorm(h->p_z, f, h->p_zn, N2, D, k.ln_eps, s));
    GET(h, "ptf.out_w", 1u, &w, (size_t)d * K * D);
    int rc = gemm(EPI_F32, h->p_zn, w, h->h_enc, B * T, d, K * D);
    if (rc) return rc;
    GET(h, "enc.ln_f", 0u, &f, (size_t)d);
    LAUNCH(launch_rmsnorm(h->h_enc, f, enc_out, B * T, d, k.ln_eps, s));
    HIP_TRY(hipGetLastError());
    return YMT3_OK;
}

static int encode_impl(ymt3_handle h, const float* mel, int B, bf16_t* enc_out, hipStream_t s) {
    const ymt3_config& k = h->cfg;
    if (k.encoder_type == YMT3_ENC_PERCEIVER_TF) return encode_ptf(h, mel, B, enc_out, s);
    const int M = B * h->T, d = k.d_model, inner = h->inner;
    LAUNCH(launch_f32_to_bf16(mel, h->mel_bf, (size_t)M * k.n_mels, s));
    bf16_t* w;
    float* f;
    {
        float* bias;
        GET(h, "in_proj.w", 1u, &w, (size_t)d * k.n_mels);
        GET(h, "in_proj.b", 0u, &bias, (size_t)d);
        GemmArgs g{h->mel_bf, w, h->h_enc, bias, M, d, k.n_mels, k.n_mels, k.n_mels, d, 0, 0, 0};
        LAUNCH(launch_gemm(EPI_F32, g, s));
    }
    const float* bias_off;
    GET(h, "enc.bias_off", 0u, const_cast<float**>(&bias_off), (size_t)k.n_heads * (2 * h->T - 1));
    for (int l = 0; l < k.n_enc_layers; ++l) {
        const std::string p = "enc." + std::to_string(l) + ".";
        GET(h, p + "ln1", 0u, &f, (size_t)d);
        LAUNCH(launch_rmsnorm(h->h_enc, f, h->xn, M, d, k.ln_eps, s));
        GET(h, p + "wqkv", 1u, &w, (size_t)3 * inner * d);
        { GemmArgs g{h->xn, w, h->qkv, nullptr, M, 3 * inner, d, d, d, 3 * inner, 0, 0, 0}; LAUNCH(launch_gemm(EPI_BF16, g, s)); }
        LAUNCH(launch_enc_attention(h->qkv, bias_off, h->attn, B, h->T, k.n_heads, s));
        GET(h, p + "wo", 1u, &w, (size_t)d * inner);
        { GemmArgs g{h->attn, w, h->h_enc, nullptr, M, d, inner, inner, inner, d, 0, 0, 0}; LAUNCH(launch_gemm(EPI_RESID, g, s)); }
        GET(h, p + "ln2", 0u, &f, (size_t)d);
        LAUNCH(launch_rmsnorm(h->h_enc, f, h->xn, M, d, k.ln_eps, s));
        GET(h, p + "wi", 1u, &w, (size_t)k.d_ff * d);
        { GemmArgs g{h->xn, w, h->ff, nullptr, M, k.d_ff, d, d, d, k.d_ff, 0, 0, 0}; LAUNCH(launch_gemm(EPI_BF16_RELU, g, s)); }
        GET(h, p + "wo2", 1u, &w, (size_t)d * k.d_ff);
        { GemmArgs g{h->ff, w, h->h_enc, nullptr, M, d, k.d_ff, k.d_ff, k.d_ff, d, 0, 0, 0}; LAUNCH(launch_gemm(EPI_RESID, g, s)); }
    }
    GET(h, "enc.ln_f", 0u, &f, (size_t)d);
    LAUNCH(launch_rmsnorm(h->h_enc, f, enc_out, M, d, k.ln_eps, s));
    HIP_TRY(hipGetLastError());
    return YMT3_OK;
}

extern "C" int ymt3_encode(ymt3_handle h, const float* mel_dev, int B, void* enc_dev, void* stream) {
    int rc = check_call(h, B);
    if (rc) return rc;
    if (B == 0) return YMT3_OK;
    if (!mel_dev || !enc_dev) FAIL(YMT3_ERR_ARG, "null buffer");
    return encode_impl(h, mel_dev, B, static_cast<bf16_t*>(enc_dev), (hipStream_t)stream);
}

static int beam_args(ymt3_handle h, int R, int W, DecodeShared* shared, BeamArgs* out) {
    const ymt3_config& k = h->cfg;
    const int d = k.d_model;
    BeamArgs b = h->beam;
    b.logits = h->logits; b.h = h->h_dec; b.shared = shared; b.beam = h->beam_shared; b.finished = h->finished; b.ssq = h->ssq; b.ssq_stride = h->maxR;
    b.R = R; b.V = k.vocab; b.d = d; b.n_channels = k.n_channels; b.eos_id = k.eos_id; b.pad_id = k.pad_id; b.W = W; b.row_state = h->row_state;
    if (h->slot_mode) { b.row_pos = h->row_pos; b.row_out = h->row_out; b.row_prompt = h->row_prompt; }
    GET(h, "dec.embed", 1u, const_cast<bf16_t**>(&b.embed), (size_t)k.vocab * d);
    if (k.n_channels > 1) GET(h, "dec.chan_embed", 1u, const_cast<bf16_t**>(&b.chan_embed), (size_t)k.n_channels * d);
    *out = b;
    return 0;
}

static int launch_step(ymt3_handle h, int B, int row0, int R, DecodeShared* shared, hipStream_t s, bool solo = true) {
    const ymt3_config& k = h->cfg;
    const int d = k.d_model, inner = h->inner, H = k.n_heads, L = k.max_decode_len;
    const size_t layer_cache = (size_t)h->maxR * H * L * 64;
    const size_t slab = (size_t)B * H * h->T * 64;
    const float* bias_dist;
    GET(h, "dec.bias_dist", 0u, const_cast<float**>(&bias_dist), (size_t)H * L);
    bf16_t* w;
    float* f;
    struct LayerW { float *ln1, *ln2, *ln3; bf16_t *wqkv, *wo, *wq_c, *wo_c, *wi, *wo2, *router; uint8_t *wi_q8, *wo_q8; float *wi_s, *wo_s; };
    std::vector<LayerW> LW(k.n_dec_layers);
    for (int l = 0; l < k.n_dec_layers; ++l) {
        const std::string p = "dec." + std::to_string(l) + ".";
        GET(h, p + "ln1", 0u, &LW[l].ln1, (size_t)d);
        GET(h, p + "ln2", 0u, &LW[l].ln2, (size_t)d);
        GET(h, p + "ln3", 0u, &LW[l].ln3, (size_t)d);
        GET(h, p + "wqkv", 1u, &LW[l].wqkv, (size_t)3 * inner * d);
        GET(h, p + "wo", 1u, &LW[l].wo, (size_t)d * inner);
        GET(h, p + "wq_c", 1u, &LW[l].wq_c, (size_t)inner * d);
        GET(h, p + "wo_c", 1u, &LW[l].wo_c, (size_t)d * inner);
        const size_t ne = k.dec_ffn == YMT3_FFN_MOE ? (size_t)k.n_experts : 1;
        LW[l].wi = LW[l].wo2 = nullptr; LW[l].wi_q8 = LW[l].wo_q8 = nullptr; LW[l].wi_s = LW[l].wo_s = nullptr;
        if (k.dec_ffn == YMT3_FFN_MOE && k.moe_fp8) {
            GET(h, p + "wi_q8", 3u, &LW[l].wi_q8, ne * k.d_ff * d);
            GET(h, p + "wo2_q8", 3u, &LW[l].wo_q8, ne * d * k.d_ff);
            GET(h, p + "wi_s", 0u, &LW[l].wi_s, ne);
            GET(h, p + "wo2_s", 0u, &LW[l].wo_s, ne);
        } else {
            GET(h, p + "wi", 1u, &LW[l].wi, ne * k.d_ff * d);
            GET(h, p + "wo2", 1u, &LW[l].wo2, ne * d * k.d_ff);
        }
        LW[l].router = nullptr;
        if (k.dec_ffn == YMT3_FFN_MOE) GET(h, p + "router", 1u, &LW[l].router, (size_t)k.n_experts * d);
    }
    bf16_t* lm_head;
    GET(h, "dec.lm_head", 1u, &lm_head, (size_t)k.vocab * d);
    (void)w;
    h->stamp_n = 0;
    const int mtiles = (R + 15) / 16;
    const bool fold_combine = k.dec_ffn == YMT3_FFN_MOE && h->moe_fold_combine && R < (h->mid_rows > 0 ? h->mid_rows : (h->mid_rows < 0 ? DEC_GEMM_MID_ROWS : 1 << 30));
    float* hcur = h->h_dec;
    const float* pend = nullptr;
    const int bW = h->beam_W, rows_kv = k.n_channels * (bW > 0 ? bW : 1);
    const bool mc = h->fuse_q && rows_kv >= 2 && rows_kv <= 16 && (h->T == 128 || h->T == 256 || h->T == 512) &&
                    row0 % rows_kv == 0 && R % rows_kv == 0;
    const bool merged_rows = solo && k.n_channels == 1 && row0 == 0 && R <= h->merged_max_rows && h->attn_pair && h->pair_rows;
    const bool fold = bW == 0 && h->fold_o && h->fuse_q && !mc && !h->force_2wave && H == 8 && d == 512 && ((R <= 96 && solo) || merged_rows);
    const bool merged_regime = fold && solo && k.n_channels == 1 && R <= h->merged_max_rows && row0 == 0;
    const bool chain = h->gemm_chain && h->chain_sync && merged_regime && k.dec_ffn != YMT3_FFN_MOE && inner == 512 && k.d_ff == 2048 &&
                       k.vocab % 32 == 0 && k.vocab / 32 >= 32 && k.vocab / 32 <= 64;
    const bool pair_ok = h->attn_pair && h->pair_rows && merged_regime;
    const bool moe_chain = h->moe_chain && h->chain_sync && pair_ok && fold_combine && k.dec_ffn == YMT3_FFN_MOE && k.n_experts == 8 && inner == 512 && k.d_ff == 2048 &&
                           k.vocab % 32 == 0 && k.vocab / 32 >= 32 && k.vocab / 32 <= 64 && h->h_dec2;
    const bool stepk = h->step_kernel && h->step_sync && chain && pair_ok && R <= 64 && k.n_dec_layers <= 8 && h->T <= 0xfff;
    h->step_merged = chain || pair_ok || moe_chain;
    bool qkv_done = false, lm_done = false;
    for (int l = 0; l < k.n_dec_layers; ++l) {
        const LayerW& W = LW[l];
        DecGemmArgs a{};
        a.row0 = row0; a.R = R; a.eps = k.ln_eps; a.H = H; a.L = L; a.shared = shared; a.ssq = h->ssq; a.ssq_stride = h->maxR;
        a.row_pos = h->slot_mode ? h->row_pos : nullptr;
        a.mid_rows = h->mid_rows;
        a.x_f32 = hcur; a.gain = W.ln1; a.W = W.wqkv; a.N = 3 * inner; a.K = d; a.out_bf16 = h->dq;
        if (pend) {
            a.pend_y = pend;
            a.h_out = hcur == h->h_dec ? h->h_dec2 : h->h_dec;
        }
        a.kcache = h->kcache + l * layer_cache; a.vcache = h->vcache + l * layer_cache;
        if (!qkv_done) {
            a.stamp = next_stamp(h, PC_QKV, a.N / 16 * mtiles);
            PLAUNCH(PC_QKV, launch_dec_gemm(DG_NORM_QKV_CACHE, a, s));
        }
        qkv_done = false;
        if (pend) { hcur = a.h_out; pend = nullptr; a.pend_y = nullptr; a.h_out = nullptr; }
        if (stepk) {
            StepArgs sa{};
            sa.n_layers = k.n_dec_layers; sa.R = R; sa.T = h->T; sa.L = L; sa.ssq_stride = h->maxR; sa.eps = k.ln_eps;
            sa.tiles_free = h->step_tiles_free ? 1 : 0;
            sa.q = h->dq; sa.attn = h->dattn; sa.opart = h->opart; sa.h = hcur; sa.ssq = h->ssq; sa.dff = h->dff; sa.logits = h->logits;
            sa.bias = bias_dist; sa.shared = shared; sa.row_pos = a.row_pos;
            sa.sync = h->step_sync; sa.pair_rows = h->pair_rows; sa.abort_word = h->chain_sync + CHAIN_ABORT_WORD; sa.host_abort = h->chain_host_abort;
            const float* ln_f;
            GET(h, "dec.ln_f", 0u, const_cast<float**>(&ln_f), (size_t)d);
            for (int j = 0; j < k.n_dec_layers; ++j) {
                const bool last = j + 1 == k.n_dec_layers;
                StepLayer& SL = sa.layer[j];
                SL.wo = LW[j].wo; SL.wq_c = LW[j].wq_c; SL.wo_c = LW[j].wo_c; SL.wi = LW[j].wi; SL.wo2 = LW[j].wo2;
                SL.w3 = last ? lm_head : LW[j + 1].wqkv;
                SL.ln2 = LW[j].ln2; SL.ln3 = LW[j].ln3; SL.gain3 = last ? ln_f : LW[j + 1].ln1;
                SL.kself = h->kcache + (size_t)j * layer_cache; SL.vself = h->vcache + (size_t)j * layer_cache;
                SL.kcross = h->ckv + (size_t)(2 * j) * slab; SL.vcross = h->ckv + (size_t)(2 * j + 1) * slab;
                SL.knext = last ? nullptr : h->kcache + (size_t)(j + 1) * layer_cache; SL.vnext = last ? nullptr : h->vcache + (size_t)(j + 1) * layer_cache;
                SL.N3 = last ? k.vocab : 3 * inner; SL.last = last ? 1 : 0;
            }
            sa.stamp = next_stamp(h, PC_STEP, ((R + 15) / 16) * 128);
            PLAUNCH(PC_STEP, launch_dec_step(sa, s));
            lm_done = true;
            break;
        }
        DecAttnArgs t{};
        t.q = h->dq; t.k = a.kcache; t.v = a.vcache; t.out = h->dattn; t.bias = bias_dist; t.shared = shared; t.row0 = row0;
        t.n_keys_const = 0; t.slab_keys = L; t.rows_per_kv = 1; t.R = R; t.H = H; t.bias_stride = L;
        t.row_pos = a.row_pos; t.force_many = h->force_2wave ? 1 : 0;
        if (fold) { t.wo = W.wo; t.opart = h->opart; }
        const bool pair = pair_ok && fold;
        DecAttnArgs ts = t;
        if (bW > 0) {
            const BeamAttn ba{h->beam.anc, h->beam.anc_rows, h->beam.anc_pitch, bW};
            t.stamp = next_stamp(h, PC_SELF_ATTN, R * H);
            PLAUNCH(PC_SELF_ATTN, launch_dec_attention_beam(t, ba, s));
        } else if (!pair) {
            t.stamp = next_stamp(h, PC_SELF_ATTN, R * H);
            PLAUNCH(PC_SELF_ATTN, launch_dec_attention(true, t, s));
        }
        t.wo = nullptr; t.opart = nullptr;
        a.a_bf16 = h->dattn; a.W = W.wo; a.N = d; a.K = inner; a.out_f32 = hcur;
        if (!fold) {
            a.stamp = next_stamp(h, PC_SELF_O, a.N / 16 * mtiles);
            PLAUNCH(PC_SELF_O, launch_dec_gemm(DG_RESID, a, s));
        }
        t.k = h->ckv + (size_t)(2 * l) * slab; t.v = h->ckv + (size_t)(2 * l + 1) * slab; t.bias = nullptr;
        t.n_keys_const = h->T; t.slab_keys = h->T; t.rows_per_kv = rows_kv;
        if (fold) t.ipart = h->opart;
        if (mc) {
            McCrossArgs mcx{};
            mcx.x_f32 = hcur; mcx.gain = W.ln2; mcx.ssq = h->ssq; mcx.ssq_stride = h->maxR; mcx.eps = k.ln_eps;
            mcx.wq = W.wq_c; mcx.k = t.k + (size_t)(row0 / rows_kv) * H * h->T * 64; mcx.v = t.v + (size_t)(row0 / rows_kv) * H * h->T * 64;
            mcx.out = h->dattn; mcx.row0 = row0; mcx.n_seg = R / rows_kv; mcx.n_channels = rows_kv; mcx.H = H; mcx.T = h->T;
            PLAUNCH(PC_CROSS_ATTN, launch_mc_cross_attention(mcx, s));
        } else if (h->fuse_q) {
            t.wq = W.wq_c; t.x_f32 = hcur; t.gain = W.ln2; t.ssq = h->ssq; t.ssq_stride = h->maxR; t.eps = k.ln_eps;
        } else {
            a.gain = W.ln2; a.W = W.wq_c; a.N = inner; a.K = d; a.out_bf16 = h->dq;
            a.stamp = next_stamp(h, PC_CROSS_Q, a.N / 16 * mtiles);
            PLAUNCH(PC_CROSS_Q, launch_dec_gemm(DG_NORM_BF16, a, s));
        }
        if (pair) {
            if (chain || moe_chain) t.chain_sync = h->chain_sync;
            ts.stamp = t.stamp = next_stamp(h, PC_ATTN_PAIR, R * H);
            PLAUNCH(PC_ATTN_PAIR, launch_dec_attention_pair(ts, t, h->pair_rows, h->chain_sync + CHAIN_ABORT_WORD, h->chain_host_abort, s));
        } else if (!mc) {
            if (chain) t.chain_sync = h->chain_sync;
            t.stamp = next_stamp(h, PC_CROSS_ATTN, R * H);
            PLAUNCH(PC_CROSS_ATTN, launch_dec_attention(false, t, s));
        }
        if (chain) {
            const bool last = l + 1 == k.n_dec_layers;
            ChainArgs cg{};
            cg.w0 = W.wo_c; cg.w1 = W.wi; cg.w2 = W.wo2; cg.w3 = last ? lm_head : LW[l + 1].wqkv;
            cg.attn = h->dattn; cg.part = h->opart; cg.h = hcur; cg.ssq = h->ssq; cg.ssq_stride = h->maxR;
            cg.gain1 = W.ln3;
            if (last) GET(h, "dec.ln_f", 0u, const_cast<float**>(&cg.gain3), (size_t)d);
// ... 2 lines not shown
            cg.mode3 = last ? DG_NORM_LOGITS : DG_NORM_QKV_CACHE; cg.N3 = last ? k.vocab : 3 * inner;
            cg.out_q = h->dq; cg.kcache = h->kcache + (size_t)(l + 1) * layer_cache; cg.vcache = h->vcache + (size_t)(l + 1) * layer_cache;
            cg.logits = h->logits; cg.H = H; cg.L = L; cg.shared = shared; cg.row_pos = a.row_pos; cg.row0 = row0; cg.R = R; cg.eps = k.ln_eps;
            cg.sync = h->chain_sync; cg.host_abort = h->chain_host_abort;
            { static const int nsub_env = [] { const char* e = getenv("YMT3_CHAIN_NSUB"); return e ? (int)strtol(e, nullptr, 16) : 0; }(); cg.nsub = nsub_env; }
            cg.stamp = next_stamp(h, PC_CHAIN, 256);
            PLAUNCH(PC_CHAIN, launch_dec_chain(cg, s));
            if (last) lm_done = true; else qkv_done = true;
            continue;
        }
        if (moe_chain) {
            const bool last = l + 1 == k.n_dec_layers;
            MoeChainArgs mc2{};
            mc2.wo_c = W.wo_c; mc2.w3 = last ? lm_head : LW[l + 1].wqkv;
            if (k.moe_fp8) { mc2.wi = W.wi_q8; mc2.wo = W.wo_q8; mc2.wi_s = W.wi_s; mc2.wo_s = W.wo_s; }
            else { mc2.wi = W.wi; mc2.wo = W.wo2; }
            mc2.attn = h->dattn; mc2.h = hcur; mc2.part = h->opart; mc2.ssq = h->ssq; mc2.ssq_stride = h->maxR;
            mc2.gain_r = W.ln3; mc2.router = W.router; mc2.xn = h->moe.xn; mc2.sel = h->moe.sel; mc2.gate = h->moe.gate; mc2.hidden = h->moe.hidden; mc2.y = h->moe.y;
            if (last) GET(h, "dec.ln_f", 0u, const_cast<float**>(&mc2.gain3), (size_t)d);
            else mc2.gain3 = LW[l + 1].ln1;
            mc2.mode3 = last ? DG_NORM_LOGITS : DG_NORM_QKV_CACHE; mc2.N3 = last ? k.vocab : 3 * inner;
            mc2.h_out = last ? nullptr : (hcur == h->h_dec ? h->h_dec2 : h->h_dec);
            mc2.out_q = h->dq; mc2.kcache = h->kcache + (size_t)(l + 1) * layer_cache; mc2.vcache = h->vcache + (size_t)(l + 1) * layer_cache;
            mc2.logits = h->logits; mc2.H = H; mc2.L = L; mc2.shared = shared; mc2.row_pos = a.row_pos;
            mc2.R = R; mc2.E = k.n_experts; mc2.fp8 = k.moe_fp8; mc2.eps = k.ln_eps;
            mc2.sync = h->chain_sync; mc2.host_abort = h->chain_host_abort;
            mc2.sel_trace = h->slot_mode ? nullptr : h->moe_trace; mc2.layer = l; mc2.n_layers = k.n_dec_layers;
            mc2.trace_rows = h->moe_trace_rows; mc2.trace_steps = h->moe_trace_steps;
            mc2.stamp = next_stamp(h, PC_CHAIN, 256);
            PLAUNCH(PC_CHAIN, launch_moe_chain(mc2, s));
            if (last) lm_done = true;
            else { qkv_done = true; hcur = mc2.h_out; }
            continue;
        }
        a.a_bf16 = h->dattn; a.W = W.wo_c; a.N = d; a.K = inner;
        a.part = fold ? h->opart : nullptr;
        a.stamp = next_stamp(h, PC_CROSS_O, a.N / 16 * mtiles);
        PLAUNCH(PC_CROSS_O, launch_dec_gemm(DG_RESID, a, s));
        a.part = nullptr;
        if (k.dec_ffn == YMT3_FFN_MOE) {
            MoeArgs mo = h->moe;
            mo.h = hcur; mo.gain = W.ln3; mo.ssq = h->ssq; mo.ssq_stride = h->maxR;
            mo.router = W.router; mo.wi = W.wi; mo.wo = W.wo2; mo.row0 = row0; mo.R = R;
            mo.wi_q8 = W.wi_q8; mo.wo_q8 = W.wo_q8; mo.wi_s = W.wi_s; mo.wo_s = W.wo_s; mo.fp8 = k.moe_fp8;
            mo.sel_trace = h->slot_mode ? nullptr : h->moe_trace; mo.shared = shared; mo.layer = l; mo.n_layers = k.n_dec_layers;
            mo.trace_rows = h->moe_trace_rows; mo.trace_steps = h->moe_trace_steps;
            { ProfScope _ps(h, PC_FFN_WI, s); LAUNCH(launch_moe_stage(0, mo, s)); LAUNCH(launch_moe_stage(1, mo, s)); }
            { ProfScope _ps(h, PC_FFN_WO, s); LAUNCH(launch_moe_stage(2, mo, s)); if (!fold_combine) LAUNCH(launch_moe_stage(3, mo, s)); }
            if (fold_combine) pend = mo.y;
        } else {
            a.gain = W.ln3; a.W = W.wi; a.N = k.d_ff; a.K = d; a.out_bf16 = h->dff;
            a.stamp = next_stamp(h, PC_FFN_WI, a.N / 16 * mtiles);
            PLAUNCH(PC_FFN_WI, launch_dec_gemm(DG_NORM_BF16_RELU, a, s));
            a.a_bf16 = h->dff; a.W = W.wo2; a.N = d; a.K = k.d_ff;
            a.stamp = next_stamp(h, PC_FFN_WO, a.N / 16 * mtiles);
            PLAUNCH(PC_FFN_WO, launch_dec_gemm(DG_RESID, a, s));
        }
    }
    DecGemmArgs a{};
    a.row0 = row0; a.R = R; a.eps = k.ln_eps; a.H = H; a.L = L; a.shared = shared; a.ssq = h->ssq; a.ssq_stride = h->maxR;
    a.mid_rows = h->mid_rows;
    GET(h, "dec.ln_f", 0u, &f, (size_t)d);
    a.x_f32 = hcur; a.gain = f; a.W = lm_head; a.N = k.vocab; a.K = d; a.out_f32 = h->logits;
    a.pend_y = pend;
    if (!lm_done) {
        a.stamp = next_stamp(h, PC_LM_HEAD, a.N / 16 * mtiles);
        PLAUNCH(PC_LM_HEAD, launch_dec_gemm(DG_NORM_LOGITS, a, s));
    }
    if (bW > 0) {
        BeamArgs b{};
        int rcb = beam_args(h, R, bW, shared, &b);
        if (rcb) return rcb;
        b.stamp = next_stamp(h, PC_ARGMAX, R / bW);
        PLAUNCH(PC_ARGMAX, launch_beam_select(b, s));
        return YMT3_OK;
    }
    ArgmaxArgs g{};
    g.logits = h->logits; g.h = h->h_dec; g.shared = shared; g.finished = h->finished; g.ssq = h->ssq; g.ssq_stride = h->maxR; g.row0 = row0;
    g.R = R; g.V = k.vocab; g.d = d; g.n_channels = k.n_channels; g.eos_id = k.eos_id; g.pad_id = k.pad_id;
    GET(h, "dec.embed", 1u, const_cast<bf16_t**>(&g.embed), (size_t)k.vocab * d);
    if (k.n_channels > 1) GET(h, "dec.chan_embed", 1u, const_cast<bf16_t**>(&g.chan_embed), (size_t)k.n_channels * d);
    if (h->slot_mode) { g.row_pos = h->row_pos; g.row_out = h->row_out; g.row_prompt = h->row_prompt; }
    g.row_state = h->row_state;
    if (solo) g.ticket = h->ticket;
    if (stepk) { g.zero_sync = h->step_sync; g.zero_lines = k.n_dec_layers * STEP_SYNC_LINES_PER_LAYER; }
    g.stamp = next_stamp(h, PC_ARGMAX, R);
    PLAUNCH(PC_ARGMAX, launch_argmax_embed(g, s));
    return YMT3_OK;
}

static int decode_run(ymt3_handle h, const bf16_t* enc, int B, int n_steps, const int32_t* prompt, int n_prompt, int32_t* tokens,
                      float* scores, const int32_t* forced, float* logits_out, const ConstraintView& cv, hipStream_t s, int prof_stride,
                      int step0);

static int decode_impl(ymt3_handle h, const bf16_t* enc, int B, int n_steps, const int32_t* prompt, int n_prompt, int32_t* tokens,
                       float* scores, const int32_t* forced, float* logits_out, const ConstraintView& cv, hipStream_t s,
                       int prof_stride = 0) {
    const int step0 = h->prof_step0;
    h->prof_step0 = 0;
    if (n_prompt < 0) FAIL(YMT3_ERR_ARG, "n_prompt=%d < 0", n_prompt);
    if (n_prompt > 0 && !prompt) FAIL(YMT3_ERR_ARG, "n_prompt=%d with a null prompt", n_prompt);
    if (n_prompt > 0 && step0 > 0) FAIL(YMT3_ERR_ARG, "ymt3_debug_decode_start does not combine with a prompt (n_prompt=%d)", n_prompt);
    return decode_run(h, enc, B, n_steps, prompt, n_prompt, tokens, scores, forced, logits_out, cv, s, prof_stride, step0);
}

static int decode_run(ymt3_handle h, const bf16_t* enc, int B, int n_steps, const int32_t* prompt, int n_prompt, int32_t* tokens,
                      float* scores, const int32_t* forced, float* logits_out, const ConstraintView& cv, hipStream_t s, int prof_stride,
                      int step0) {
    const ymt3_config& k = h->cfg;
    bool merged = false;
    if (n_steps <= 0 || step0 + n_prompt + n_steps > k.max_decode_len)
        FAIL(YMT3_ERR_ARG, "n_steps=%d outside [1, max_decode_len - n_prompt=%d]", n_steps, k.max_decode_len - step0 - n_prompt);
    const int n_total = n_prompt + n_steps;
    const int d = k.d_model, R = B * k.n_channels;
    GemmArgs g{enc, h->wkv_all, h->ckv, nullptr, B * h->T, k.n_dec_layers * 2 * h->inner, d, d, d, 0, h->T, k.n_heads, B};
    LAUNCH(launch_gemm(EPI_KV_HEADMAJOR, g, s));

    ArgmaxArgs a{};
    a.h = h->h_dec; a.shared = h->shared; a.finished = h->finished; a.ssq = h->ssq; a.ssq_stride = h->maxR;
    a.R = R; a.V = k.vocab; a.d = d; a.n_channels = k.n_channels; a.eos_id = k.eos_id; a.pad_id = k.pad_id;
    GET(h, "dec.embed", 1u, const_cast<bf16_t**>(&a.embed), (size_t)k.vocab * d);
    if (k.n_channels > 1) GET(h, "dec.chan_embed", 1u, const_cast<bf16_t**>(&a.chan_embed), (size_t)k.n_channels * d);
    int n_chains = (!h->use_graph || prof_stride > 0 || k.dec_ffn == YMT3_FFN_MOE) ? 1 : h->n_chains;
    if (h->auto_chains && n_chains == 1 && h->use_graph && prof_stride == 0 && k.dec_ffn != YMT3_FFN_MOE && k.n_channels == 1 && R >= 168 && R <= 256 &&
        !(h->early_stop_interval > 0 && k.eos_id >= 0 && !forced))
        n_chains = 2;
    if (n_chains > R) n_chains = R;
    h->last_chains = n_chains;
    if (h->step_kernel && h->step_sync) HIP_TRY(hipMemsetAsync(h->step_sync, 0, (size_t)STEP_SYNC_LINES * CHAIN_LINE * sizeof(unsigned), s));
    a.row_state = h->row_state;
    LAUNCH(launch_decode_init(a, n_chains, n_steps, step0, tokens, forced, logits_out, prompt, n_prompt, scores, cv, s));
    h->last_steps = n_total;
    int row0[9];
    row0[0] = 0;
    for (int c = 0; c < n_chains; ++c) row0[c + 1] = row0[c] + R / n_chains + (c < R % n_chains ? 1 : 0);

    if (!h->use_graph || prof_stride > 0) {
        for (int t = 0; t < n_total; ++t) {
            const bool sampled = prof_stride > 0 && (t % prof_stride) == prof_stride / 2;
            const bool span_begin = prof_stride > 1 && (t % prof_stride) == prof_stride / 2 + 1 && t + prof_stride - 1 <= n_total;
            const bool span_end = prof_stride > 1 && t >= prof_stride && (t % prof_stride) == prof_stride / 2 && !h->prof_ev.empty() && h->prof_span_open;
            if (span_end) { (void)hipEventRecord(h->prof_ev[h->prof_span_idx], s); h->prof_span_open = false; }
            if (span_begin) {
                hipEvent_t ea, eb;
                if (hipEventCreate(&ea) == hipSuccess && hipEventCreate(&eb) == hipSuccess) {
                    h->prof_ev.push_back(ea); h->prof_ev.push_back(eb); h->prof_cls.push_back(PC_SPAN);
                    h->prof_span_idx = h->prof_ev.size() - 1; h->prof_span_open = true;
                    (void)hipEventRecord(ea, s);
                }
            }
            h->prof_on = sampled;
            int rc = launch_step(h, B, 0, R, h->shared, s);
            h->prof_on = false;
            if (rc) return rc;
            merged = merged || h->step_merged;
        }
        if (h->prof_span_open) {
            (void)hipEventRecord(h->prof_ev[h->prof_span_idx], s);
            h->prof_cls[h->prof_span_idx / 2] = -1;
            h->prof_span_open = false;
        }
    } else {
        hipGraphExec_t exec[8];
        for (int c = 0; c < n_chains; ++c) {
            StepGraph& sg = h->step_graphs[((long)B * 16 + n_chains) * 16 + c];
            if (!sg.exec) {
                HIP_TRY(hipStreamBeginCapture(h->cap_stream, hipStreamCaptureModeThreadLocal));
                int rc = launch_step(h, B, row0[c], row0[c + 1] - row0[c], h->shared + c, h->cap_stream, n_chains == 1);
                hipError_t e = hipStreamEndCapture(h->cap_stream, &sg.graph);
                if (rc) return rc;
                if (e != hipSuccess) FAIL(YMT3_ERR_HIP, "hipStreamEndCapture: %s", hipGetErrorString(e));
                HIP_TRY(hipGraphInstantiate(&sg.exec, sg.graph, nullptr, nullptr, 0));
                sg.merged = h->step_merged;
            }
            exec[c] = sg.exec;
            merged = merged || sg.merged;
        }
        if (n_chains == 1 && h->early_stop_interval > 0 && k.eos_id >= 0 && !forced) {
            for (int i = 0; i < n_prompt; ++i) HIP_TRY(hipGraphLaunch(exec[0], s));
            int t = 0;
            while (t < n_steps) {
                const int chunk = std::min(h->early_stop_interval, n_steps - t);
                for (int i = 0; i < chunk; ++i) HIP_TRY(hipGraphLaunch(exec[0], s));
                t += chunk;
                if (t >= n_steps) break;
                HIP_TRY(hipMemcpyAsync(h->host_flag, &h->shared->n_unfinished, sizeof(int), hipMemcpyDeviceToHost, s));
                HIP_TRY(hipStreamSynchronize(s));
                if (*h->host_flag == 0) break;
            }
            h->last_steps = n_prompt + t;
            LAUNCH(launch_pad_tail(tokens, scores, 0, R, n_steps, t, k.pad_id, s));
        } else if (n_chains == 1) {
            const int G = h->graph_steps;
            int t = 0;
            if (G > 1 && n_total >= G) {
                StepGraph& mg = h->step_graphs[(((long)B * 16 + 1) * 16) | (1L << 40) | ((long)G << 32)];
                if (!mg.exec) {
                    HIP_TRY(hipStreamBeginCapture(h->cap_stream, hipStreamCaptureModeThreadLocal));
                    int rc = 0;
                    for (int i = 0; i < G && !rc; ++i) rc = launch_step(h, B, 0, R, h->shared, h->cap_stream);
                    hipError_t e = hipStreamEndCapture(h->cap_stream, &mg.graph);
                    if (rc) return rc;
                    if (e != hipSuccess) FAIL(YMT3_ERR_HIP, "hipStreamEndCapture: %s", hipGetErrorString(e));
                    HIP_TRY(hipGraphInstantiate(&mg.exec, mg.graph, nullptr, nullptr, 0));
                    mg.merged = h->step_merged;
                }
                merged = merged || mg.merged;
                for (; t + G <= n_total; t += G) HIP_TRY(hipGraphLaunch(mg.exec, s));
            }
            for (; t < n_total; ++t) HIP_TRY(hipGraphLaunch(exec[0], s));
        } else {
// ... 191 lines not shown
            SeqAttnDecArgs ca{};
            ca.q = h->qkv; ca.k = h->ckv + (size_t)(2 * l) * slab; ca.v = h->ckv + (size_t)(2 * l + 1) * slab; ca.out = h->attn;
            ca.q_seq = ca.o_seq = (long long)L * inner; ca.kv_seq = (long long)H * T * 64;
            ca.ldq = ca.ldo = inner; ca.ldkv = 64; ca.kv_head = T * 64;
            ca.row0 = row0; ca.n_rows = nr; ca.L = L; ca.n_keys = T; ca.rows_per_kv = k.n_channels; ca.H = H;
            LAUNCH(launch_dec_seq_attention(false, ca, s));
            GET(h, p + "wo_c", 1u, &w, (size_t)d * inner);
            { GemmArgs q{h->attn, w, h->h_enc, nullptr, M, d, inner, inner, inner, d, 0, 0, 0}; LAUNCH(launch_gemm(EPI_RESID, q, s)); }
            GET(h, p + "ln3", 0u, &f, (size_t)d);
            LAUNCH(launch_rmsnorm(h->h_enc, f, h->xn, M, d, k.ln_eps, s));
            GET(h, p + "wi", 1u, &w, (size_t)k.d_ff * d);
            { GemmArgs q{h->xn, w, h->ff, nullptr, M, k.d_ff, d, d, d, k.d_ff, 0, 0, 0}; LAUNCH(launch_gemm(EPI_BF16_RELU, q, s)); }
            GET(h, p + "wo2", 1u, &w, (size_t)d * k.d_ff);
            { GemmArgs q{h->ff, w, h->h_enc, nullptr, M, d, k.d_ff, k.d_ff, k.d_ff, d, 0, 0, 0}; LAUNCH(launch_gemm(EPI_RESID, q, s)); }
        }
        LAUNCH(launch_rmsnorm(h->h_enc, ln_f, h->xn, M, d, k.ln_eps, s));
        SeqLmHeadArgs lm{};
        lm.xn = h->xn; lm.W = lm_head; lm.tokens = tokens; lm.lengths = lengths; lm.scores = scores; lm.logits = logits_out;
        lm.M = M; lm.L = L; lm.n_prompt = n_prompt; lm.n_steps = n_steps; lm.V = k.vocab; lm.d = d; lm.row0 = row0;
        LAUNCH(launch_seq_lm_head_score(lm, s));
    }
    HIP_TRY(hipGetLastError());
    return YMT3_OK;
}

extern "C" int ymt3_score_tokens(ymt3_handle h, const void* enc_dev, int B, int n_steps, const int32_t* prompt_dev, int n_prompt,
                                 const int32_t* tokens_dev, const int32_t* lengths_dev, float* scores_dev, float* logits_dev, void* stream) {
    int rc = check_call(h, B);
    if (rc) return rc;
    rc = score_check(h, n_steps, prompt_dev, n_prompt, tokens_dev, scores_dev);
    if (rc) return rc;
    if (B == 0) return YMT3_OK;
    if (!enc_dev) FAIL(YMT3_ERR_ARG, "null buffer");
    return score_impl(h, static_cast<const bf16_t*>(enc_dev), B, n_steps, prompt_dev, n_prompt, tokens_dev, lengths_dev, scores_dev, logits_dev,
                      (hipStream_t)stream);
}

extern "C" int ymt3_transcribe_segments_score(ymt3_handle h, const float* audio_dev, int B, int n_steps, const int32_t* prompt_dev, int n_prompt,
                                              const int32_t* tokens_dev, const int32_t* lengths_dev, float* scores_dev, void* stream) {
    int rc = check_call(h, B);
    if (rc) return rc;
    rc = score_check(h, n_steps, prompt_dev, n_prompt, tokens_dev, scores_dev);
    if (rc) return rc;
    if (B == 0) return YMT3_OK;
    if (!audio_dev) FAIL(YMT3_ERR_ARG, "null buffer");
    hipStream_t s = (hipStream_t)stream;
    LAUNCH(launch_logmel(h->fe, audio_dev, h->mel, B, s));
    rc = encode_impl(h, h->mel, B, h->enc_out, s);
    if (rc) return rc;
    return score_impl(h, h->enc_out, B, n_steps, prompt_dev, n_prompt, tokens_dev, lengths_dev, scores_dev, nullptr, s);
}

static int beam_check(ymt3_handle h, int B, int n_steps, const int32_t* prompt, int n_prompt, const ymt3_beam_params* p, const int32_t* tokens) {
    const ymt3_config& k = h->cfg;
    if (!p) FAIL(YMT3_ERR_ARG, "null beam parameters");
    if (p->num_beams < 1 || p->num_beams > BEAM_MAX) FAIL(YMT3_ERR_ARG, "num_beams=%d outside [1, %d]", p->num_beams, BEAM_MAX);
    if (p->num_return < 1 || p->num_return > p->num_beams) FAIL(YMT3_ERR_ARG, "num_return=%d outside [1, num_beams=%d]", p->num_return, p->num_beams);
    if (!(p->length_penalty >= 0.f) || p->length_penalty > 3.0e38f) FAIL(YMT3_ERR_ARG, "length_penalty=%g must be finite and >= 0", (double)p->length_penalty);
    if ((long long)B * k.n_channels * p->num_beams > h->maxR)
        FAIL(YMT3_ERR_ARG, "B * n_channels * num_beams = %lld rows exceed the max_batch * n_channels = %d rows the handle was created for",
             (long long)B * k.n_channels * p->num_beams, h->maxR);
    if (k.n_channels * p->num_beams > 255) FAIL(YMT3_ERR_ARG, "n_channels * num_beams = %d exceeds 255 rows per segment", k.n_channels * p->num_beams);
    if (h->beam.anc_pitch > 48 * 1024) FAIL(YMT3_ERR_ARG, "beam search needs max_decode_len < %d (the staged ancestry table)", 48 * 1024 - 16);
    if (n_prompt < 0 || (n_prompt > 0 && !prompt)) FAIL(YMT3_ERR_ARG, "n_prompt=%d with prompt %s", n_prompt, prompt ? "set" : "null");
    if (n_steps <= 0 || n_prompt + n_steps > k.max_decode_len)
        FAIL(YMT3_ERR_ARG, "n_steps=%d outside [1, max_decode_len - n_prompt=%d]", n_steps, k.max_decode_len - n_prompt);
    if (h->prof_step0) FAIL(YMT3_ERR_ARG, "ymt3_debug_decode_start is pending: it does not combine with beams");
    if (B > 0 && !tokens) FAIL(YMT3_ERR_ARG, "null buffer");
    return 0;
}

static int decode_beam_impl(ymt3_handle h, const bf16_t* enc, int B, int n_steps, const int32_t* prompt, int n_prompt, const ymt3_beam_params* p,
                            int32_t* tokens, float* seq_scores, float* token_scores, const ConstraintView& cv, hipStream_t s) {
    const ymt3_config& k = h->cfg;
    const int W = p->num_beams, d = k.d_model, R = B * k.n_channels * W, n_total = n_prompt + n_steps;
    GemmArgs g{enc, h->wkv_all, h->ckv, nullptr, B * h->T, k.n_dec_layers * 2 * h->inner, d, d, d, 0, h->T, k.n_heads, B};
    LAUNCH(launch_gemm(EPI_KV_HEADMAJOR, g, s));
    BeamArgs b{};
    int rcb = beam_args(h, R, W, h->shared, &b);
    if (rcb) return rcb;
    BeamShared params = h->beam_trace;
    params.alpha = p->length_penalty; params.tokens_out = tokens; params.seq_out = seq_scores; params.tok_out = token_scores;
    h->last_chains = 1;
    LAUNCH(launch_beam_init(b, n_steps, prompt, n_prompt, cv, params, s));
    h->last_steps = n_total;
    struct BeamGuard { ymt3_ctx* c; ~BeamGuard() { c->beam_W = 0; } } guard{h};
    h->beam_W = W;
    auto graph_of = [&](int G, hipGraphExec_t* out) -> int {
        StepGraph& sg = h->step_graphs[(((long)B * 16 + 14) * 16 + W) | (1L << 41) | ((long)G << 32)];
        if (!sg.exec) {
            HIP_TRY(hipStreamBeginCapture(h->cap_stream, hipStreamCaptureModeThreadLocal));
            int rc = 0;
            for (int i = 0; i < G && !rc; ++i) rc = launch_step(h, B, 0, R, h->shared, h->cap_stream);
            hipError_t e = hipStreamEndCapture(h->cap_stream, &sg.graph);
            if (rc) return rc;
            if (e != hipSuccess) FAIL(YMT3_ERR_HIP, "hipStreamEndCapture: %s", hipGetErrorString(e));
            HIP_TRY(hipGraphInstantiate(&sg.exec, sg.graph, nullptr, nullptr, 0));
        }
        *out = sg.exec;
        return 0;
    };
    if (!h->use_graph) {
        for (int t = 0; t < n_total; ++t) { int rc = launch_step(h, B, 0, R, h->shared, s); if (rc) return rc; }
    } else if (h->early_stop_interval > 0) {
        hipGraphExec_t one;
        int rc = graph_of(1, &one);
        if (rc) return rc;
        for (int i = 0; i < n_prompt; ++i) HIP_TRY(hipGraphLaunch(one, s));
        int t = 0;
        while (t < n_steps) {
            const int chunk = std::min(h->early_stop_interval, n_steps - t);
            for (int i = 0; i < chunk; ++i) HIP_TRY(hipGraphLaunch(one, s));
            t += chunk;
            if (t >= n_steps) break;
            HIP_TRY(hipMemcpyAsync(h->host_flag, &h->shared->n_unfinished, sizeof(int), hipMemcpyDeviceToHost, s));
            HIP_TRY(hipStreamSynchronize(s));
            if (*h->host_flag == 0) break;
        }
        h->last_steps = n_prompt + t;
    } else {
        const int G = h->graph_steps;
        int t = 0;
        if (G > 1 && n_total >= G) {
            hipGraphExec_t many;
            int rc = graph_of(G, &many);
            if (rc) return rc;
            for (; t + G <= n_total; t += G) HIP_TRY(hipGraphLaunch(many, s));
        }
        if (t < n_total) {
            hipGraphExec_t one;
            int rc = graph_of(1, &one);
            if (rc) return rc;
            for (; t < n_total; ++t) HIP_TRY(hipGraphLaunch(one, s));
        }
    }
    LAUNCH(launch_beam_finalize(b, p->num_return, s));
    HIP_TRY(hipGetLastError());
    return YMT3_OK;
}

extern "C" int ymt3_decode_beam(ymt3_handle h, const void* enc_dev, int B, int n_steps, const int32_t* prompt_dev, int n_prompt,
                                const ymt3_beam_params* params, int32_t* tokens_dev, float* seq_scores_dev, float* token_scores_dev,
                                ymt3_constraint constraint, const int32_t* start_state_dev, void* stream) {
    int rc = check_call(h, B);
    if (rc) return rc;
    ConstraintView cv{};
    rc = constraint_view(h, constraint, start_state_dev, &cv);
    if (rc) return rc;
    rc = beam_check(h, B, n_steps, prompt_dev, n_prompt, params, tokens_dev);
    if (rc) return rc;
    if (B == 0) return YMT3_OK;
    if (!enc_dev) FAIL(YMT3_ERR_ARG, "null buffer");
    return decode_beam_impl(h, static_cast<const bf16_t*>(enc_dev), B, n_steps, prompt_dev, n_prompt, params, tokens_dev, seq_scores_dev,
                            token_scores_dev, cv, (hipStream_t)stream);
}

extern "C" int ymt3_transcribe_segments_beam(ymt3_handle h, const float* audio_dev, int B, int n_steps, const int32_t* prompt_dev, int n_prompt,
                                             const ymt3_beam_params* params, int32_t* tokens_dev, float* seq_scores_dev,
                                             float* token_scores_dev, ymt3_constraint constraint, const int32_t* start_state_dev, void* stream) {
    int rc = check_call(h, B);
    if (rc) return rc;
    ConstraintView cv{};
    rc = constraint_view(h, constraint, start_state_dev, &cv);
    if (rc) return rc;
    rc = beam_check(h, B, n_steps, prompt_dev, n_prompt, params, tokens_dev);
    if (rc) return rc;
// ... 56 lines not shown
            LAUNCH(launch_gemm(EPI_KV_HEADMAJOR, g, s));
            rce = start(slot, first_seg + i);
            if (rce) return rce;
            slot_seg[(size_t)slot] = first_seg + i;
        }
        return YMT3_OK;
    };
    for (int i = 0; i < slots; ++i) free_slots.push_back(i);
    rc = admit(0, slots);
    if (rc) return rc;
    int next = slots, live = slots;
    const long max_rounds = ((long)n_segments / slots + 2) * ((n_total + interval - 1) / interval + 1);
    h->last_steps = 0;
    for (long round = 0; live > 0; ++round) {
        h->last_steps += interval;
        if (round > max_rounds) FAIL(YMT3_ERR_HIP, "slot scheduler made no progress (%d live, %d admitted of %d)", live, next, n_segments);
        for (int i = 0; i < interval; i += exec ? per_graph : 1) {
            if (exec) HIP_TRY(hipGraphLaunch(exec, s));
            else { int rcs = launch_step(h, slots, 0, R, h->shared, s); if (rcs) return rcs; }
        }
        HIP_TRY(hipMemcpyAsync(h->host_rows, h->finished, (size_t)R * sizeof(int), hipMemcpyDeviceToHost, s));
        HIP_TRY(hipStreamSynchronize(s));
        if (watch_abort) {
            if (h->forced_abort && h->chain_host_abort) *h->chain_host_abort = 1u;
            if (h->chain_host_abort && *static_cast<volatile unsigned*>(h->chain_host_abort)) return restart();
        }
        free_slots.clear();
        for (int slot = 0; slot < slots; ++slot) {
            if (slot_seg[(size_t)slot] < 0) continue;
            bool all = true;
            for (int c = 0; c < rows; ++c) all = all && h->host_rows[slot * rows + c] != 0;
            if (!all) continue;
            rc = retire(slot);
            if (rc) return rc;
            slot_seg[(size_t)slot] = -1;
            --live;
            free_slots.push_back(slot);
        }
        const int nb = std::min((int)free_slots.size(), n_segments - next);
        if (nb > 0) {
            rc = admit(next, nb);
            if (rc) return rc;
            next += nb;
            live += nb;
        }
    }
    HIP_TRY(hipGetLastError());
    return YMT3_OK;
}

extern "C" int ymt3_transcribe_stream_constrained(ymt3_handle h, const float* audio_dev, int n_segments, int n_steps,
                                                  const int32_t* prompt_dev, int n_prompt, int32_t* tokens_dev, float* scores_dev, int slots,
                                                  int interval, ymt3_constraint constraint, const int32_t* start_state_dev, void* stream) {
    int rc = check_call(h, 0);
    if (rc) return rc;
    ConstraintView cv{};
    rc = constraint_view(h, constraint, start_state_dev, &cv);
    if (rc) return rc;
    if (n_segments < 0) FAIL(YMT3_ERR_ARG, "n_segments=%d", n_segments);
    if (n_segments == 0) return YMT3_OK;
    if (!audio_dev || !tokens_dev) FAIL(YMT3_ERR_ARG, "null buffer");
    const ymt3_config& k = h->cfg;
    if (n_prompt < 0 || (n_prompt > 0 && !prompt_dev)) FAIL(YMT3_ERR_ARG, "n_prompt=%d with prompt %s", n_prompt, prompt_dev ? "set" : "null");
    if (n_steps <= 0 || n_prompt + n_steps > k.max_decode_len)
        FAIL(YMT3_ERR_ARG, "n_steps=%d outside [1, max_decode_len - n_prompt=%d]", n_steps, k.max_decode_len - n_prompt);
    if (interval < 0) FAIL(YMT3_ERR_ARG, "interval=%d", interval);
    if (h->prof_step0) FAIL(YMT3_ERR_UNSUPPORTED, "ymt3_debug_decode_start is pending: it applies to lock-step decode calls only");
    if (interval == 0) interval = 8;
    if (slots <= 0 || slots > h->maxB) slots = h->maxB;
    if (slots > n_segments) slots = n_segments;
    hipStream_t s = (hipStream_t)stream;
    if (!h->host_rows) HIP_TRY(hipHostMalloc(reinterpret_cast<void**>(&h->host_rows), (size_t)h->maxR * sizeof(int), hipHostMallocDefault));
    const int K = k.n_channels, R = slots * K, d = k.d_model;

    ArgmaxArgs a{};
    a.h = h->h_dec; a.shared = h->shared; a.finished = h->finished; a.ssq = h->ssq; a.ssq_stride = h->maxR;
    a.R = R; a.V = k.vocab; a.d = d; a.n_channels = K; a.eos_id = k.eos_id; a.pad_id = k.pad_id;
    a.row_pos = h->row_pos; a.row_out = h->row_out; a.row_prompt = h->row_prompt; a.row_state = h->row_state;
    GET(h, "dec.embed", 1u, const_cast<bf16_t**>(&a.embed), (size_t)k.vocab * d);
    if (K > 1) GET(h, "dec.chan_embed", 1u, const_cast<bf16_t**>(&a.chan_embed), (size_t)K * d);

    struct ModeGuard { ymt3_ctx* c; ~ModeGuard() { c->slot_mode = false; } } guard{h};
    h->slot_mode = true;
    if (h->step_kernel && h->step_sync) HIP_TRY(hipMemsetAsync(h->step_sync, 0, (size_t)STEP_SYNC_LINES * CHAIN_LINE * sizeof(unsigned), s));
    ConstraintView cv_init = cv;
    cv_init.start = nullptr;
    LAUNCH(launch_decode_init(a, 1, n_steps, 0, tokens_dev, nullptr, nullptr, prompt_dev, n_prompt, scores_dev, cv_init, s));
    HIP_TRY(hipMemsetD32Async(reinterpret_cast<hipDeviceptr_t>(h->finished), 1, (size_t)R, s));
    HIP_TRY(hipMemsetAsync(h->row_pos, 0, (size_t)R * sizeof(int), s));
    HIP_TRY(hipMemsetAsync(h->row_out, 0, (size_t)R * sizeof(long long), s));
    HIP_TRY(hipMemsetAsync(h->row_prompt, 0, (size_t)R * sizeof(long long), s));

    const long key = ((long)slots * 16 + 15) * 16;
    auto start = [&](int slot, int seg) -> int {
        ConstraintView cv_seg = cv;
        if (cv.start) cv_seg.start = cv.start + (size_t)seg * K;
        LAUNCH(launch_slot_start(a, slot * K, (long long)seg * K * n_steps, n_steps, h->row_out, (long long)seg * K * n_prompt, n_prompt,
                                 h->row_prompt, cv_seg, s));
        return YMT3_OK;
    };
    auto retire = [&](int slot) -> int {
        LAUNCH(launch_slot_retire(a, slot * K, K, n_steps, n_prompt, tokens_dev, scores_dev, s));
        return YMT3_OK;
    };
    auto restart = [&]() -> int {
        int rcf = merged_fallback(h);
        if (rcf) return rcf;
        return ymt3_transcribe_stream_constrained(h, audio_dev, n_segments, n_steps, prompt_dev, n_prompt, tokens_dev, scores_dev, slots, interval,
                                                  constraint, start_state_dev, stream);
    };
    return run_slot_queue(h, audio_dev, n_segments, slots, K, interval, n_prompt + n_steps, key, true, start, retire, restart, s);
}

extern "C" int ymt3_transcribe_stream_scored(ymt3_handle h, const float* audio_dev, int n_segments, int n_steps, const int32_t* prompt_dev,
                                             int n_prompt, int32_t* tokens_dev, float* scores_dev, int slots, int interval, void* stream) {
    return ymt3_transcribe_stream_constrained(h, audio_dev, n_segments, n_steps, prompt_dev, n_prompt, tokens_dev, scores_dev, slots, interval,
                                              nullptr, nullptr, stream);
}

extern "C" int ymt3_transcribe_stream_prompted(ymt3_handle h, const float* audio_dev, int n_segments, int n_steps, const int32_t* prompt_dev,
                                               int n_prompt, int32_t* tokens_dev, int slots, int interval, void* stream) {
    return ymt3_transcribe_stream_scored(h, audio_dev, n_segments, n_steps, prompt_dev, n_prompt, tokens_dev, nullptr, slots, interval, stream);
}

extern "C" int ymt3_transcribe_stream(ymt3_handle h, const float* audio_dev, int n_segments, int n_steps, int32_t* tokens_dev,
                                      int slots, int interval, void* stream) {
    return ymt3_transcribe_stream_prompted(h, audio_dev, n_segments, n_steps, nullptr, 0, tokens_dev, slots, interval, stream);
}

extern "C" int ymt3_transcribe_stream_beam(ymt3_handle h, const float* audio_dev, int n_segments, int n_steps, const int32_t* prompt_dev,
                                           int n_prompt, const ymt3_beam_params* params, int32_t* tokens_dev, float* seq_scores_dev,
                                           float* token_scores_dev, int slots, int interval, ymt3_constraint constraint,
                                           const int32_t* start_state_dev, void* stream) {
    int rc = check_call(h, 0);
    if (rc) return rc;
    ConstraintView cv{};
    rc = constraint_view(h, constraint, start_state_dev, &cv);
    if (rc) return rc;
    if (n_segments < 0) FAIL(YMT3_ERR_ARG, "n_segments=%d", n_segments);
    rc = beam_check(h, 0, n_steps, prompt_dev, n_prompt, params, tokens_dev);
    if (rc) return rc;
    if (interval < 0) FAIL(YMT3_ERR_ARG, "interval=%d", interval);
    const ymt3_config& k = h->cfg;
    const int W = params->num_beams, K = k.n_channels;
    if (h->maxB / W < 1) FAIL(YMT3_ERR_ARG, "num_beams=%d exceeds max_batch=%d: not one slot of n_channels * num_beams rows fits", W, h->maxB);
    if (n_segments == 0) return YMT3_OK;
    if (!audio_dev || !tokens_dev) FAIL(YMT3_ERR_ARG, "null buffer");
    if (interval == 0) interval = 8;
    if (slots <= 0 || slots > h->maxB / W) slots = h->maxB / W;
    if (slots > n_segments) slots = n_segments;
    hipStream_t s = (hipStream_t)stream;
    if (!h->host_rows) HIP_TRY(hipHostMalloc(reinterpret_cast<void**>(&h->host_rows), (size_t)h->maxR * sizeof(int), hipHostMallocDefault));
    const int rows = K * W, R = slots * rows;

    struct ModeGuard { ymt3_ctx* c; ~ModeGuard() { c->slot_mode = false; c->beam_W = 0; } } guard{h};
    h->slot_mode = true;
    h->beam_W = W;
    BeamArgs b{};
    rc = beam_args(h, R, W, h->shared, &b);
    if (rc) return rc;
    BeamShared bp = h->beam_trace;
    bp.alpha = params->length_penalty; bp.tokens_out = tokens_dev; bp.seq_out = seq_scores_dev; bp.tok_out = token_scores_dev;
    h->last_chains = 1;
    ConstraintView cv_init = cv;
    cv_init.start = nullptr;
    LAUNCH(launch_beam_init(b, n_steps, prompt_dev, n_prompt, cv_init, bp, s));
    HIP_TRY(hipMemsetD32Async(reinterpret_cast<hipDeviceptr_t>(h->finished), 1, (size_t)R, s));
    HIP_TRY(hipMemsetAsync(h->row_pos, 0, (size_t)R * sizeof(int), s));
    HIP_TRY(hipMemsetAsync(h->row_out, 0, (size_t)R * sizeof(long long), s));
    HIP_TRY(hipMemsetAsync(h->row_prompt, 0, (size_t)R * sizeof(long long), s));

    const long key = (((long)slots * 16 + 13) * 16 + W) | (1L << 42);
    const int N = params->num_return;
    auto start = [&](int slot, int seg) -> int {
        ConstraintView cv_seg = cv;
        if (cv.start) cv_seg.start = cv.start + (size_t)seg * K;
        LAUNCH(launch_beam_slot_start(b, slot * rows, (long long)seg * K, n_prompt, cv_seg, s));
        return YMT3_OK;
    };
    auto retire = [&](int slot) -> int {
        LAUNCH(launch_beam_slot_finalize(b, slot * rows, N, s));
        return YMT3_OK;
    };
    auto restart = []() -> int { return YMT3_OK; };
    return run_slot_queue(h, audio_dev, n_segments, slots, rows, interval, n_prompt + n_steps, key, false, start, retire, restart, s);
}

extern "C" int ymt3_test_gemm(ymt3_handle h, const void* a_dev, const void* w_dev, float* c_dev, int M, int N, int K, void* stream) {
    int rc = check_call(h, 0);
    if (rc) return rc;
    GemmArgs g{static_cast<const bf16_t*>(a_dev), static_cast<const bf16_t*>(w_dev), c_dev, nullptr, M, N, K, K, K, N, 0, 0, 0};
    LAUNCH(launch_gemm(EPI_F32, g, (hipStream_t)stream));
    HIP_TRY(hipGetLastError());
    return YMT3_OK;
}

extern "C" int ymt3_profile_decode(ymt3_handle h, const void* enc_dev, int B, int n_steps, int stride, int32_t* tokens_dev,
                                   float* ms_by_class, int32_t* launches_by_class, void* stream) {
    int rc = check_call(h, B);
    if (rc) return rc;
    if (!enc_dev || !tokens_dev || !ms_by_class || !launches_by_class || stride <= 0 || B == 0) FAIL(YMT3_ERR_ARG, "bad argument");
    hipStream_t s = (hipStream_t)stream;
    h->prof_ev.clear();
    h->prof_cls.clear();
    rc = decode_impl(h, static_cast<const bf16_t*>(enc_dev), B, n_steps, nullptr, 0, tokens_dev, nullptr, nullptr, nullptr, ConstraintView{}, s,
                     stride);
    hipError_t e = hipStreamSynchronize(s);
    for (int i = 0; i < YMT3_PROFILE_CLASSES; ++i) { ms_by_class[i] = 0.f; launches_by_class[i] = 0; }
    for (size_t i = 0; i < h->prof_cls.size(); ++i) {
        float ms = 0.f;
        if (rc == 0 && e == hipSuccess && h->prof_cls[i] >= 0 &&
            hipEventElapsedTime(&ms, h->prof_ev[2 * i], h->prof_ev[2 * i + 1]) == hipSuccess) {
            ms_by_class[h->prof_cls[i]] += ms;
            launches_by_class[h->prof_cls[i]] += 1;
        }
        (void)hipEventDestroy(h->prof_ev[2 * i]);
        (void)hipEventDestroy(h->prof_ev[2 * i + 1]);
    }
    h->prof_ev.clear();
    h->prof_cls.clear();
    if (rc) return rc;
    if (e != hipSuccess) FAIL(YMT3_ERR_HIP, "hipStreamSynchronize: %s", hipGetErrorString(e));
    return YMT3_OK;
}
static_assert(PC_COUNT <= YMT3_PROFILE_CLASSES, "profile class table");

extern "C" int ymt3_debug_step_stamps(ymt3_handle h, int32_t* cls, int32_t* grid, uint64_t* stats, int* n_kernels) {
    if (!h || !cls || !grid || !stats || !n_kernels) FAIL(YMT3_ERR_ARG, "null argument");
    if (!h->stamp_buf) FAIL(YMT3_ERR_UNSUPPORTED, "stamps are recorded only by a handle created with YMT3_STAMP=1 in the environment");
    HIP_TRY(hipSetDevice(h->device));
    HIP_TRY(hipDeviceSynchronize());
    std::vector<unsigned long long> host((size_t)STAMP_WGS * 2);
    *n_kernels = h->stamp_n;
    for (int i = 0; i < h->stamp_n; ++i) {
        const int gsz = h->stamp_grid[i];
        HIP_TRY(hipMemcpy(host.data(), h->stamp_buf + (size_t)i * STAMP_WGS * 2, (size_t)gsz * 2 * sizeof(unsigned long long), hipMemcpyDeviceToHost));
        unsigned long long in_min = ~0ull, in_max = 0, out_min = ~0ull, out_max = 0;
        for (int w = 0; w < gsz; ++w) {
            if (host[2 * w] == 0) continue;
            in_min = std::min(in_min, host[2 * w]); in_max = std::max(in_max, host[2 * w]);
            out_min = std::min(out_min, host[2 * w + 1]); out_max = std::max(out_max, host[2 * w + 1]);
        }
        cls[i] = h->stamp_cls[i]; grid[i] = gsz;
        stats[4 * i] = in_min; stats[4 * i + 1] = in_max; stats[4 * i + 2] = out_min; stats[4 * i + 3] = out_max;
    }
    return YMT3_OK;
// ... 177 lines not shown
```

yourmt3_amd/model.py:

```python
from __future__ import annotations

import ctypes
import weakref
from typing import Dict, List, Optional

import numpy as np
import torch

from . import _lib
from .config import YMT3Config, to_c
from .constraint import TokenAutomaton
from .tables import derived_tables
from .weights import make_weights, pack_blob


def _ptr(t: Optional[torch.Tensor]):
    return ctypes.c_void_p(t.data_ptr()) if t is not None else None


class DecodeConstraint:

    def __init__(self, model: "YourMT3", automaton: TokenAutomaton):
        self.automaton = automaton
        self.n_states = automaton.n_states
# ... 80 lines not shown
        elif t.dim() == 2:
            if t.shape[0] != B:
                raise ValueError(f"task_tokens (B, P) needs B = {B} rows, got {tuple(t.shape)}")
            t = t[:, None, :].expand(B, K, t.shape[1])
        elif t.dim() == 3:
            if tuple(t.shape[:2]) != (B, K):
                raise ValueError(f"task_tokens (B, K, P) must be ({B}, {K}, P), got {tuple(t.shape)}")
        else:
            raise ValueError(f"task_tokens must be (P,), (B, P) or (B, K, P), got {tuple(t.shape)}")
        P = int(t.shape[-1])
        if t.numel() and (int(t.min()) < 0 or int(t.max()) >= cfg.vocab):
            raise ValueError(f"task_tokens ids must lie in [0, {cfg.vocab})")
        if P + n_steps > cfg.max_decode_len:
            raise ValueError(f"{P} prompt + {n_steps} emitted steps exceed max_decode_len {cfg.max_decode_len}")
        return t.to(self.device, torch.int32).contiguous()

    BEAM_MAX = 8

    def _beam_params(self, B: int, num_beams, num_return_sequences, length_penalty) -> Optional["_lib.BeamParams"]:
        W, N = int(num_beams), int(num_return_sequences)
        if W != num_beams or N != num_return_sequences:
            raise ValueError("num_beams and num_return_sequences must be integers")
        alpha = float(length_penalty)
        if not 1 <= W <= self.BEAM_MAX:
            raise ValueError(f"num_beams={W} outside [1, {self.BEAM_MAX}]")
        if not 1 <= N <= W:
            raise ValueError(f"num_return_sequences={N} outside [1, num_beams={W}]")
        if not (alpha >= 0.0) or alpha == float("inf"):
            raise ValueError(f"length_penalty={alpha} must be finite and >= 0")
        if W == 1 and N == 1:
            return None
        if B * W > self.max_batch:
            raise ValueError(f"{B} segments x num_beams={W} need max_batch >= {B * W}, the model was created with max_batch={self.max_batch}")
        if self.cfg.n_channels * W > 255:
            raise ValueError(f"n_channels * num_beams = {self.cfg.n_channels * W} exceeds 255 rows per segment")
        return _lib.BeamParams(W, N, alpha)

    def beam_trace(self, n_steps: int, n_groups: int, num_beams: int, logits: bool = False):
        W = int(num_beams)
        tr = torch.full((n_steps, n_groups, W, 2), -1, device=self.device, dtype=torch.int32)
        run = torch.full((n_steps, n_groups, W), float("nan"), device=self.device, dtype=torch.float32)
        lg = torch.full((n_steps, n_groups, W, self.cfg.vocab), float("nan"), device=self.device, dtype=torch.float32) if logits else None
        _lib.check(self._lib.ymt3_debug_beam_trace(self._handle, _ptr(tr), _ptr(run), _ptr(lg), n_steps, n_groups))
        self._beam_trace = (tr, run, lg)
        return self._beam_trace

    def compile_constraint(self, automaton: TokenAutomaton) -> DecodeConstraint:
        if automaton.vocab != self.cfg.vocab:
            raise ValueError(f"automaton vocab {automaton.vocab} != the model's {self.cfg.vocab}")
        c = DecodeConstraint(self, automaton)
        self._constraints.add(c)
        return c

    def _start_states(self, constraint: Optional[DecodeConstraint], start_states, B: int) -> Optional[torch.Tensor]:
        if constraint is None:
            if start_states is not None:
                raise ValueError("start_states without a constraint")
            return None
        if start_states is None:
            return None
        K = self.cfg.n_channels
        t = torch.as_tensor(start_states)
        if t.dtype.is_floating_point or t.dtype == torch.bool or t.dtype.is_complex:
            raise ValueError(f"start_states must be integer states, got {t.dtype}")
        if t.dim() == 1 and t.shape[0] == K:
            t = t[None, :].expand(B, K)
        elif not (t.dim() == 2 and tuple(t.shape) == (B, K)):
            raise ValueError(f"start_states must be ({K},) or ({B}, {K}), got {tuple(t.shape)}")
        if t.numel() and (int(t.min()) < 0 or int(t.max()) >= constraint.n_states):
            raise ValueError(f"start states must lie in [0, {constraint.n_states})")
        return t.to(self.device, torch.int32).contiguous()

    @property
    def last_decode_steps(self) -> int:
        return int(self._lib.ymt3_last_decode_steps(self._handle))

    @property
    def merged_fallbacks(self) -> int:
        return int(self._lib.ymt3_merged_fallbacks(self._handle))

    @property
    def last_decode_chains(self) -> int:
        return int(self._lib.ymt3_last_decode_chains(self._handle))

    def set_abort_recovery(self, mode: int) -> None:
        _lib.check(self._lib.ymt3_set_abort_recovery(self._handle, int(mode)))

    def set_early_stop(self, interval: int) -> None:
        _lib.check(self._lib.ymt3_set_early_stop(self._handle, int(interval)))

    def ingest(self, pcm: torch.Tensor, sample_rate: int) -> torch.Tensor:
        if pcm.dim() == 1:
            pcm = pcm[:, None]
        if pcm.dim() != 2:
            raise ValueError("pcm must be (n_frames, n_channels)")
        if pcm.dtype == torch.int16:
            fmt = 0
        elif pcm.dtype == torch.float32:
            fmt = 1
        else:
            raise ValueError("pcm must be int16 or float32")
        pcm = pcm.to(self.device).contiguous()
        n_frames, n_ch = int(pcm.shape[0]), int(pcm.shape[1])
        n_out, n_seg = ctypes.c_int64(0), ctypes.c_int(0)
        _lib.check(self._lib.ymt3_ingest_plan(self._handle, n_frames, int(sample_rate), ctypes.byref(n_out), ctypes.byref(n_seg)))
        segs = torch.empty(n_seg.value, 1, self.cfg.segment_samples, device=self.device, dtype=torch.float32)
        _lib.check(self._lib.ymt3_ingest(self._handle, _ptr(pcm) if n_frames else None, fmt, n_frames, n_ch, int(sample_rate),
                                         _ptr(segs), n_seg.value, self._stream()))
        self.last_ingest_samples = int(n_out.value)
        return segs

    def logmel(self, audio: torch.Tensor) -> torch.Tensor:
        a = self._audio2d(audio)
        B = a.shape[0]
        mel = torch.empty(B, self.cfg.n_frames, self.cfg.n_mels, device=self.device, dtype=torch.float32)
        _lib.check(self._lib.ymt3_logmel(self._handle, _ptr(a), B, _ptr(mel), self._stream()))
        return mel

    def encode(self, mel: torch.Tensor) -> torch.Tensor:
        mel = mel.to(self.device, torch.float32).contiguous()
        B = mel.shape[0]
        enc = torch.empty(B, self.cfg.n_frames, self.cfg.d_model, device=self.device, dtype=torch.bfloat16)
        _lib.check(self._lib.ymt3_encode(self._handle, _ptr(mel), B, _ptr(enc), self._stream()))
        return enc

    def decode(self, enc: torch.Tensor, n_steps: Optional[int] = None, forced: Optional[torch.Tensor] = None,
               return_logits: bool = False, prompt=None, return_scores: bool = False, constraint: Optional[DecodeConstraint] = None,
               start_states=None, num_beams: int = 1, num_return_sequences: int = 1, length_penalty: float = 1.0, _force_beam: bool = False):
        cfg = self.cfg
        enc = enc.to(self.device, torch.bfloat16).contiguous()
        B = enc.shape[0]
        bp = self._beam_params(B, num_beams, num_return_sequences, length_penalty)
        if bp is None and _force_beam:
            bp = _lib.BeamParams(1, 1, float(length_penalty))
        p = self._prompt(prompt, B, int(n_steps or 1))
        n_steps = int(n_steps or cfg.max_decode_len - (p.shape[-1] if p is not None else 0))
        if bp is not None:
            if forced is not None or return_logits:
                raise ValueError("forced ids and return_logits do not combine with beam search")
            N = bp.num_return
            tokens = torch.empty(B, cfg.n_channels, N, n_steps, device=self.device, dtype=torch.int32)
            ts = torch.empty(B, cfg.n_channels, N, n_steps, device=self.device, dtype=torch.float32) if return_scores else None
            ss = torch.empty(B, cfg.n_channels, N, device=self.device, dtype=torch.float32) if return_scores else None
            st = self._start_states(constraint, start_states, B)
            _lib.check(self._lib.ymt3_decode_beam(self._handle, _ptr(enc), B, n_steps, _ptr(p), 0 if p is None else int(p.shape[-1]),
                                                  ctypes.byref(bp), _ptr(tokens), _ptr(ss), _ptr(ts),
                                                  constraint.ptr if constraint is not None else None, _ptr(st), self._stream()))
            return (tokens, ts, ss) if return_scores else tokens
        tokens = torch.empty(B, cfg.n_channels, n_steps, device=self.device, dtype=torch.int32)
        f = forced.to(self.device, torch.int32).contiguous() if forced is not None else None
        if f is not None and tuple(f.shape) != (B, cfg.n_channels, n_steps):
            raise ValueError("forced must be (B, n_channels, n_steps)")
        lg = torch.empty(B, cfg.n_channels, n_steps, cfg.vocab, device=self.device, dtype=torch.float32) if return_logits else None
        sc = torch.empty(B, cfg.n_channels, n_steps, device=self.device, dtype=torch.float32) if return_scores else None
        st = self._start_states(constraint, start_states, B)
        if constraint is not None:
            _lib.check(self._lib.ymt3_decode_constrained(self._handle, _ptr(enc), B, n_steps, _ptr(p), 0 if p is None else int(p.shape[-1]),
                                                         _ptr(tokens), _ptr(sc), _ptr(f), _ptr(lg), constraint.ptr, _ptr(st),
                                                         self._stream()))
        elif sc is not None:
            _lib.check(self._lib.ymt3_decode_scored(self._handle, _ptr(enc), B, n_steps, _ptr(p), 0 if p is None else int(p.shape[-1]),
                                                    _ptr(tokens), _ptr(sc), _ptr(f), _ptr(lg), self._stream()))
        elif p is None:
            _lib.check(self._lib.ymt3_decode_greedy(self._handle, _ptr(enc), B, n_steps, _ptr(tokens), _ptr(f), _ptr(lg), self._stream()))
        else:
            _lib.check(self._lib.ymt3_decode_prompted(self._handle, _ptr(enc), B, n_steps, _ptr(p), int(p.shape[-1]), _ptr(tokens), _ptr(f),
# ... 225 lines not shown
```

Measured before the change: 556.6 audio_s/wall_s.

## Precompute layer-0 decoder QKV per vocab token and gather it in argmax kernel

Layer 0's RMSNorm+QKV projection depends only on the fed token (single channel), so it is precomputed once at model creation into a vocab x 1536 bf16 table. The argmax/embed and init kernels then copy the table row for the chosen token straight into the layer-0 Q buffer and K/V caches, and the per-step layer-0 QKV GEMM is skipped. This removes one GEMM launch and its weight reads from every decode step, at the cost of about 4.7 MB of device memory, extra setup work, and a gather in the argmax kernel. It is disabled for beam, profiling, multi-channel, step-kernel, or large-row modes.

```diff
diff --git a/include/ymt3.h b/include/ymt3.h
--- a/include/ymt3.h
+++ b/include/ymt3.h
@@ -110,6 +110,8 @@
 
 int ymt3_last_decode_chains(ymt3_handle h);
 
+int ymt3_qkv0_table_active(ymt3_handle h);
+
 #define YMT3_PROFILE_CLASSES 16
 int ymt3_profile_decode(ymt3_handle h, const void* enc_dev, int B, int n_steps, int stride, int32_t* tokens_dev,
                         float* ms_by_class, int32_t* launches_by_class, void* stream);
diff --git a/yourmt3_amd/_lib.py b/yourmt3_amd/_lib.py
--- a/yourmt3_amd/_lib.py
+++ b/yourmt3_amd/_lib.py
@@ -19,6 +19,7 @@
     "ymt3_transcribe_stream_constrained",
     "ymt3_decode_beam", "ymt3_transcribe_segments_beam", "ymt3_debug_beam_trace", "ymt3_transcribe_stream_beam",
     "ymt3_score_tokens", "ymt3_transcribe_segments_score",
+    "ymt3_qkv0_table_active",
 ]
 
 _lib = None
@@ -104,6 +105,8 @@
     lib.ymt3_merged_fallbacks.restype = i32
     lib.ymt3_last_decode_chains.argtypes = [vp]
     lib.ymt3_last_decode_chains.restype = i32
+    lib.ymt3_qkv0_table_active.argtypes = [vp]
+    lib.ymt3_qkv0_table_active.restype = i32
     lib.ymt3_debug_moe_trace.argtypes = [vp, vp, i32, i32]
     lib.ymt3_debug_moe_trace.restype = i32
     bp = ctypes.POINTER(BeamParams)
diff --git a/yourmt3_amd/csrc/decode.hip b/yourmt3_amd/csrc/decode.hip
--- a/yourmt3_amd/csrc/decode.hip
+++ b/yourmt3_amd/csrc/decode.hip
@@ -217,7 +217,9 @@
         const uint32_t pk = pack_bf16x2(s.x, s.y);
         if constexpr (MODE == DG_NORM_QKV_CACHE) {
             const int inner = a.H * DKV;
-            if (n < inner) {
+            if (a.table) {
+                *reinterpret_cast<uint32_t*>(a.table + (size_t)m * N + n) = pk;
+            } else if (n < inner) {
                 *reinterpret_cast<uint32_t*>(a.out_bf16 + (size_t)m * inner + n) = pk;
             } else {
                 const int nn = n - inner, kv = nn / inner, hh = (nn % inner) >> 6, dd = nn & 63;
@@ -838,12 +840,44 @@
     if (tid < SSQ_TILES) a.ssq[(size_t)tid * a.ssq_stride + r] = tid == 0 ? (scratch4[0] + scratch4[1]) + (scratch4[2] + scratch4[3]) : 0.f;
 }
 
+struct Qkv0Lane {
+    const bf16_t* src;
+    bf16_t* dst;
+    int pos_stride, L;
+};
+__device__ __forceinline__ Qkv0Lane qkv0_lane(const ArgmaxArgs& a, int r) {
+    Qkv0Lane q{nullptr, nullptr, 0, 0};
+    if (a.qkv0 && threadIdx.x < QKV0_COLS / 8) {
+        constexpr int inner = QKV0_COLS / 3, H = inner / DKV;
+        const int n = threadIdx.x * 8, nn = n - inner;
+        q.src = a.qkv0 + n;
+        q.L = a.L;
+        if (n < inner) {
+            q.dst = a.q0 + (size_t)r * inner + n;
+        } else {
+            q.dst = (nn / inner ? a.vcache0 : a.kcache0) + ((size_t)r * H + ((nn % inner) >> 6)) * a.L * DKV + (nn & 63);
+            q.pos_stride = DKV;
+        }
+    }
+    asm volatile("" : "+v"(q.src), "+v"(q.dst), "+v"(q.pos_stride), "+v"(q.L));
+    return q;
+}
+__device__ __forceinline__ u32x4 qkv0_load(const Qkv0Lane& q, int feed) {
+    u32x4 v = {0u, 0u, 0u, 0u};
+    if (q.src) v = *reinterpret_cast<const u32x4*>(q.src + (size_t)feed * QKV0_COLS);
+    return v;
+}
+__device__ __forceinline__ void qkv0_store(const Qkv0Lane& q, int pos, const u32x4& v) {
+    if (q.src && (pos < q.L || q.pos_stride == 0)) *reinterpret_cast<u32x4*>(q.dst + (size_t)pos * q.pos_stride) = v;
+}
+
 __global__ __launch_bounds__(256) void argmax_embed_kernel(const float* __restrict__ pLogits, DecodeShared* pShared, int* pFinished, int* pRowPos,
                                                            const long long* __restrict__ pRowOut, const bf16_t* __restrict__ pEmbed, int row0, int V,
                                                            ArgmaxArgs a) {
     __shared__ float sv[4];
     __shared__ int si[4];
     __shared__ int s_feed;
+    __shared__ int s_pos;
     __shared__ float s_sum[4];
     const int tid = threadIdx.x, lane = tid & 63, wave = tid >> 6;
     const int r = row0 + blockIdx.x;
@@ -860,6 +894,7 @@
     const int forced_tok = forced && col >= 0 ? forced[(size_t)r * n_steps + col] : 0;
     const int pos0 = pRowPos ? pRowPos[r] : 0;
     const long long out0 = pRowPos ? pRowOut[r] : 0;
+    const Qkv0Lane ql = qkv0_lane(a, r);
 
     STAMP_IN(a);
     float bv = -3.4e38f;
@@ -908,21 +943,22 @@
         for (int w = 1; w < 4; ++w)
             if (sv[w] > bv || (sv[w] == bv && si[w] < bi)) { bv = sv[w]; bi = si[w]; }
         bi = min(bi, V - 1);
-        int feed = a.pad_id;
+        int feed = a.pad_id, pos1 = pos0;
         if (!was_finished && pos0 < n_prompt) {
-            pRowPos[r] = pos0 + 1;
+            pRowPos[r] = pos1 = pos0 + 1;
             feed = prompt[a.row_prompt[r] + pos0];
         } else if (!was_finished) {
             const int p = pos0 - n_prompt;
             tokens_out[out0 + p] = bi;
             if ((a.eos_id >= 0 && bi == a.eos_id) || p + 1 >= n_steps) pFinished[r] = 1;
-            else pRowPos[r] = pos0 + 1;
+            else pRowPos[r] = pos1 = pos0 + 1;
             feed = bi;
             score_at = out0 + p;
             score_id = bi;
             if (mrow) a.row_state[r] = sh->c_next[(size_t)state * V + bi];
         }
         s_feed = feed < 0 ? 0 : (feed >= V ? V - 1 : feed);
+        s_pos = pos1;
     } else if (tid == 0 && col < 0) {
         const int p = prompt[(size_t)r * n_prompt + (t - sh->step0)];
         s_feed = p < 0 ? 0 : (p >= V ? V - 1 : p);
@@ -945,9 +981,12 @@
     }
     __syncthreads();
     const int feed = s_feed;
+    const int kv_pos = pRowPos ? s_pos : t + 1;
+    const u32x4 qkv0 = qkv0_load(ql, feed);
     const bf16_t* e = pEmbed + (size_t)feed * a.d;
     const bf16_t* c = a.chan_embed ? a.chan_embed + (size_t)(r % a.n_channels) * a.d : nullptr;
     embed_row(a, r, e, c, sv);
+    qkv0_store(ql, kv_pos, qkv0);
     if (logits_out && !pRowPos && col >= 0) {
         float* dst = logits_out + ((size_t)r * n_steps + col) * V;
         for (int i = tid; i < V; i += 256) dst[i] = row[i];
@@ -1004,7 +1043,10 @@
     const bf16_t* e = a.embed + (size_t)a.pad_id * a.d;
     const bf16_t* c = a.chan_embed ? a.chan_embed + (size_t)(r % a.n_channels) * a.d : nullptr;
     __shared__ float sv[4];
+    const Qkv0Lane ql = qkv0_lane(a, r);
+    const u32x4 qkv0 = qkv0_load(ql, a.pad_id);
     embed_row(a, r, e, c, sv);
+    qkv0_store(ql, step0, qkv0);
     if (tid == 0) {
         a.finished[r] = 0;
         if (a.row_state) a.row_state[r] = cv.start ? min(max(cv.start[r], 0), cv.n_states - 1) : 0;
@@ -1034,7 +1076,10 @@
     const bf16_t* e = a.embed + (size_t)a.pad_id * a.d;
     const bf16_t* c = a.chan_embed ? a.chan_embed + (size_t)(r % a.n_channels) * a.d : nullptr;
     __shared__ float sv[4];
+    const Qkv0Lane ql = qkv0_lane(a, r);
+    const u32x4 qkv0 = qkv0_load(ql, a.pad_id);
     embed_row(a, r, e, c, sv);
+    qkv0_store(ql, 0, qkv0);
     if (tid == 0) {
         a.finished[r] = 0;
         a.row_pos[r] = 0;
@@ -1042,6 +1087,11 @@
         row_prompt[r] = first_prompt + (long long)blockIdx.x * n_prompt;
         if (a.row_state) a.row_state[r] = cv.start ? min(max(cv.start[blockIdx.x], 0), cv.n_states - 1) : 0;
     }
+}
+
+__global__ __launch_bounds__(256) void qkv0_embed_kernel(ArgmaxArgs a, int v0) {
+    __shared__ float sv[4];
+    embed_row(a, blockIdx.x, a.embed + (size_t)(v0 + blockIdx.x) * a.d, nullptr, sv);
 }
 
 __global__ void slot_retire_kernel(ArgmaxArgs a, int row0, int n_steps, int n_prompt, int32_t* tokens_out, float* scores_out) {
@@ -1143,6 +1193,7 @@
     if (a.R <= 0) return 0;
     if (a.N % 16) return -1;
     const int mid_rows = a.mid_rows >= 0 ? a.mid_rows : DEC_GEMM_MID_ROWS;
+    if (a.table && (mode != DG_NORM_QKV_CACHE || a.pend_y || (mid_rows > 0 && a.R >= mid_rows))) return -1;
     if (mid_rows > 0 && a.R >= mid_rows && a.N % 64 == 0 && !a.part && !a.pend_y && (a.K == 512 || (a.K == 2048 && mode == DG_RESID)))
         return launch_dec_gemm_mid(mode, a, stream);
     if (mode == DG_RESID) {
@@ -1226,8 +1277,13 @@
     return 0;
 }
 
+static bool qkv0_args_ok(const ArgmaxArgs& a) {
+    return !a.qkv0 || (a.q0 && a.kcache0 && a.vcache0 && a.H * DKV * 3 == QKV0_COLS && a.L > 0 && !a.chan_embed && a.n_channels == 1);
+}
+
 int launch_argmax_embed(const ArgmaxArgs& a, hipStream_t stream) {
     if (a.R <= 0) return 0;
+    if (!qkv0_args_ok(a)) return -1;
     argmax_embed_kernel<<<a.R, 256, 0, stream>>>(a.logits, a.shared, a.finished, a.row_pos, a.row_out, a.embed, a.row0, a.V, a);
     return 0;
 }
@@ -1238,6 +1294,7 @@
     if (a.R <= 0) return 0;
     if (n_prompt < 0 || (n_prompt > 0 && !prompt)) return -1;
     if (cv.allowed && (!cv.next || !a.row_state || cv.n_states < 1 || cv.words * 32 < a.V)) return -1;
+    if (!qkv0_args_ok(a) || (a.qkv0 && (step0 < 0 || step0 >= a.L))) return -1;
     decode_init_kernel<<<a.R, 256, 0, stream>>>(a, n_chains, n_steps, step0, tokens_out, forced, logits_out, prompt, n_prompt, scores_out, cv);
     return 0;
 }
@@ -1246,6 +1303,7 @@
                       int n_prompt, long long* row_prompt, const ConstraintView& cv, hipStream_t stream) {
     if (!a.row_pos || !row_out || !row_prompt || a.n_channels <= 0) return -1;
     if (cv.start && cv.n_states < 1) return -1;
+    if (!qkv0_args_ok(a)) return -1;
     slot_start_kernel<<<a.n_channels, 256, 0, stream>>>(a, row0, first_out, n_steps, row_out, first_prompt, n_prompt, row_prompt, cv);
     return 0;
 }
@@ -1262,3 +1320,9 @@
     pad_tail_kernel<<<R, 256, 0, stream>>>(tokens_out, scores_out, row0, n_steps, from, pad_id);
     return 0;
 }
+
+int launch_qkv0_embed(const ArgmaxArgs& a, int v0, int n, hipStream_t stream) {
+    if (n <= 0 || v0 < 0 || v0 + n > a.V || !a.h || !a.ssq || !a.embed || a.ssq_stride < n) return -1;
+    qkv0_embed_kernel<<<n, 256, 0, stream>>>(a, v0);
+    return 0;
+}
diff --git a/yourmt3_amd/csrc/kernels.h b/yourmt3_amd/csrc/kernels.h
--- a/yourmt3_amd/csrc/kernels.h
+++ b/yourmt3_amd/csrc/kernels.h
@@ -106,6 +106,7 @@
     const float* pend_y;
     float* h_out;
     int mid_rows;
+    bf16_t* table;
 };
 constexpr int DEC_GEMM_MID_ROWS = 512;
 struct ChainArgs {
@@ -232,8 +233,15 @@
     int zero_lines;
     const long long* row_prompt;
     int* row_state;
-};
+    const bf16_t* qkv0;
+    bf16_t* q0;
+    bf16_t* kcache0;
+    bf16_t* vcache0;
+    int H, L;
+};
+constexpr int QKV0_COLS = 3 * 512;
 int launch_argmax_embed(const ArgmaxArgs& a, hipStream_t stream);
+int launch_qkv0_embed(const ArgmaxArgs& a, int v0, int n, hipStream_t stream);
 int launch_pad_tail(int32_t* tokens_out, float* scores_out, int row0, int R, int n_steps, int from, int pad_id, hipStream_t stream);
 int launch_slot_start(const ArgmaxArgs& a, int row0, long long first_out, int n_steps, long long* row_out, long long first_prompt,
                       int n_prompt, long long* row_prompt, const ConstraintView& cv, hipStream_t stream);
diff --git a/yourmt3_amd/csrc/runtime.hip b/yourmt3_amd/csrc/runtime.hip
--- a/yourmt3_amd/csrc/runtime.hip
+++ b/yourmt3_amd/csrc/runtime.hip
@@ -110,6 +110,8 @@
     bool moe_chain = false;
     int merged_max_rows = 64;
     bool step_tiles_free = false;
+    bf16_t* qkv0_table = nullptr;
+    bool qkv0_call = false;
     unsigned* ticket = nullptr;
     unsigned* step_sync = nullptr;
     bool prof_on = false;
@@ -246,6 +248,35 @@
 }
 
 extern "C" size_t ymt3_device_bytes(ymt3_handle h) { return h ? h->dev_bytes : 0; }
+extern "C" int ymt3_qkv0_table_active(ymt3_handle h) { return h && h->qkv0_call ? 1 : 0; }
+
+static int build_qkv0_table(ymt3_ctx* c) {
+    const ymt3_config& k = c->cfg;
+    const int d = k.d_model, V = k.vocab, N = 3 * c->inner, CH = 256;
+    if (dev_alloc(c, (void**)&c->qkv0_table, (size_t)V * N * 2)) return YMT3_ERR_HIP;
+    float *hs = nullptr, *ssq = nullptr;
+    struct Scratch { float** a; float** b; ~Scratch() { if (*a) (void)hipFree(*a); if (*b) (void)hipFree(*b); } } scratch{&hs, &ssq};
+    HIP_TRY(hipMalloc(reinterpret_cast<void**>(&hs), (size_t)CH * d * 4));
+    HIP_TRY(hipMalloc(reinterpret_cast<void**>(&ssq), (size_t)SSQ_TILES * CH * 4));
+    ArgmaxArgs e{};
+    e.h = hs; e.ssq = ssq; e.ssq_stride = CH; e.V = V; e.d = d; e.n_channels = 1;
+    GET(c, "dec.embed", 1u, const_cast<bf16_t**>(&e.embed), (size_t)V * d);
+    DecGemmArgs a{};
+    a.x_f32 = hs; a.ssq = ssq; a.ssq_stride = CH; a.N = N; a.K = d; a.eps = k.ln_eps; a.H = k.n_heads; a.L = k.max_decode_len;
+    a.shared = c->shared;
+    a.mid_rows = 0;
+    GET(c, "dec.0.ln1", 0u, const_cast<float**>(&a.gain), (size_t)d);
+    GET(c, "dec.0.wqkv", 1u, const_cast<bf16_t**>(&a.W), (size_t)N * d);
+    for (int v0 = 0; v0 < V; v0 += CH) {
+        const int n = std::min(CH, V - v0);
+        hipStream_t s = nullptr;
+        LAUNCH(launch_qkv0_embed(e, v0, n, s));
+        a.row0 = 0; a.R = n; a.table = c->qkv0_table + (size_t)v0 * N;
+        LAUNCH(launch_dec_gemm(DG_NORM_QKV_CACHE, a, s));
+    }
+    HIP_TRY(hipDeviceSynchronize());
+    return YMT3_OK;
+}
 
 static int create_impl(ymt3_ctx* c, const ymt3_config* cfg, const void* blob, size_t nbytes) {
     const ymt3_config& k = c->cfg;
@@ -457,6 +488,13 @@
     for (int l = 0; l < nd; ++l)
         for (const char* n : dec_names)
             if (!c->tensors.count("dec." + std::to_string(l) + "." + n)) FAIL(YMT3_ERR_BLOB, "missing dec.%d.%s", l, n);
+    {
+        const char* nt = getenv("YMT3_NO_QKV0_TABLE");
+        if (!(nt && nt[0] == '1') && k.n_channels == 1 && !c->step_kernel && !c->stamp_buf && 3 * c->inner == QKV0_COLS) {
+            rc = build_qkv0_table(c);
+            if (rc) return rc;
+        }
+    }
     HIP_TRY(hipDeviceSynchronize());
     return YMT3_OK;
 }
@@ -726,6 +764,15 @@
     return 0;
 }
 
+static void qkv0_decide(ymt3_handle h, int rows, bool beam, bool profiled) {
+    const int mid = h->mid_rows > 0 ? h->mid_rows : (h->mid_rows < 0 ? DEC_GEMM_MID_ROWS : 1 << 30);
+    h->qkv0_call = h->qkv0_table && !beam && !profiled && h->cfg.n_channels == 1 && rows < mid;
+}
+static void qkv0_wire(ymt3_handle h, ArgmaxArgs* a) {
+    if (!h->qkv0_call) return;
+    a->qkv0 = h->qkv0_table; a->q0 = h->dq; a->kcache0 = h->kcache; a->vcache0 = h->vcache; a->H = h->cfg.n_heads; a->L = h->cfg.max_decode_len;
+}
+
 static int launch_step(ymt3_handle h, int B, int row0, int R, DecodeShared* shared, hipStream_t s, bool solo = true) {
     const ymt3_config& k = h->cfg;
     const int d = k.d_model, inner = h->inner, H = k.n_heads, L = k.max_decode_len;
@@ -794,7 +841,7 @@
             a.h_out = hcur == h->h_dec ? h->h_dec2 : h->h_dec;
         }
         a.kcache = h->kcache + l * layer_cache; a.vcache = h->vcache + l * layer_cache;
-        if (!qkv_done) {
+        if (!qkv_done && !(l == 0 && h->qkv0_call && !pend)) {
             a.stamp = next_stamp(h, PC_QKV, a.N / 16 * mtiles);
             PLAUNCH(PC_QKV, launch_dec_gemm(DG_NORM_QKV_CACHE, a, s));
         }
@@ -963,6 +1010,7 @@
     if (k.n_channels > 1) GET(h, "dec.chan_embed", 1u, const_cast<bf16_t**>(&g.chan_embed), (size_t)k.n_channels * d);
     if (h->slot_mode) { g.row_pos = h->row_pos; g.row_out = h->row_out; g.row_prompt = h->row_prompt; }
     g.row_state = h->row_state;
+    qkv0_wire(h, &g);
     if (solo) g.ticket = h->ticket;
     if (stepk) { g.zero_sync = h->step_sync; g.zero_lines = k.n_dec_layers * STEP_SYNC_LINES_PER_LAYER; }
     g.stamp = next_stamp(h, PC_ARGMAX, R);
@@ -1008,6 +1056,8 @@
         n_chains = 2;
     if (n_chains > R) n_chains = R;
     h->last_chains = n_chains;
+    qkv0_decide(h, (R + n_chains - 1) / n_chains, false, prof_stride > 0);
+    qkv0_wire(h, &a);
     if (h->step_kernel && h->step_sync) HIP_TRY(hipMemsetAsync(h->step_sync, 0, (size_t)STEP_SYNC_LINES * CHAIN_LINE * sizeof(unsigned), s));
     a.row_state = h->row_state;
     LAUNCH(launch_decode_init(a, n_chains, n_steps, step0, tokens, forced, logits_out, prompt, n_prompt, scores, cv, s));
@@ -1365,6 +1415,7 @@
     BeamShared params = h->beam_trace;
     params.alpha = p->length_penalty; params.tokens_out = tokens; params.seq_out = seq_scores; params.tok_out = token_scores;
     h->last_chains = 1;
+    qkv0_decide(h, R, true, false);
     LAUNCH(launch_beam_init(b, n_steps, prompt, n_prompt, cv, params, s));
     h->last_steps = n_total;
     struct BeamGuard { ymt3_ctx* c; ~BeamGuard() { c->beam_W = 0; } } guard{h};
@@ -1587,6 +1638,8 @@
 
     struct ModeGuard { ymt3_ctx* c; ~ModeGuard() { c->slot_mode = false; } } guard{h};
     h->slot_mode = true;
+    qkv0_decide(h, R, false, false);
+    qkv0_wire(h, &a);
     if (h->step_kernel && h->step_sync) HIP_TRY(hipMemsetAsync(h->step_sync, 0, (size_t)STEP_SYNC_LINES * CHAIN_LINE * sizeof(unsigned), s));
     ConstraintView cv_init = cv;
     cv_init.start = nullptr;
@@ -1667,6 +1720,7 @@
     BeamShared bp = h->beam_trace;
     bp.alpha = params->length_penalty; bp.tokens_out = tokens_dev; bp.seq_out = seq_scores_dev; bp.tok_out = token_scores_dev;
     h->last_chains = 1;
+    qkv0_decide(h, R, true, false);
     ConstraintView cv_init = cv;
     cv_init.start = nullptr;
     LAUNCH(launch_beam_init(b, n_steps, prompt_dev, n_prompt, cv_init, bp, s));
diff --git a/yourmt3_amd/model.py b/yourmt3_amd/model.py
--- a/yourmt3_amd/model.py
+++ b/yourmt3_amd/model.py
@@ -186,6 +186,10 @@
     @property
     def last_decode_chains(self) -> int:
         return int(self._lib.ymt3_last_decode_chains(self._handle))
+
+    @property
+    def qkv0_table_active(self) -> bool:
+        return bool(self._lib.ymt3_qkv0_table_active(self._handle))
 
     def set_abort_recovery(self, mode: int) -> None:
         _lib.check(self._lib.ymt3_set_abort_recovery(self._handle, int(mode)))
```

Measured after the change: 565.9 audio_s/wall_s, median of 6. +1.7%, better.
